# shocker-0x15/GfxExp

Hardware: AMD Instinct MI355X
Metric: Mpaths/s, ReSTIR DI (original, biased) 1920x1080 1 spp, Bistro-Exterior stand-in (higher is better)
Workload: dtype f32; 1 GPU; configs[2] (0-based index into BASELINE.json): ReSTIR DI biased, procedural street stand-in for Bistro Exterior (2547728 instanced triangles, 2745 instances, 2100 emitter instances), textured materials (albedo / smoothness / normal maps with bump mapping, float emittance maps on the signs), 32 candidates, temporal + 2x5 spatial reuse, radius 20, visibility reuse; width=1920, height=1080, spp=1, parallelism=single GPU, light_inst_distribution=cached (static scene): built once, the per-frame call returns early

## Files before the change

### gfxexp_amd/csrc/capi.cpp

```cpp
#include <cstdlib>
#include <cstring>
#include <memory>
#include "internal.h"
#include "denoise/denoise.h"
#include "denoise/taa.h"
#include "bc/bc_textures.h"

using namespace gfx;

struct gfx_ctx { Context c; };
struct gfx_denoiser { Denoiser d; };
struct gfx_taa { TemporalAA t; };

static thread_local std::string g_createError;

namespace {
struct DeviceGuard {
    int prev = -1; bool switched = false;
    explicit DeviceGuard(int device) {
        GFX_HIP(hipGetDevice(&prev));
        if (prev != device) { GFX_HIP(hipSetDevice(device)); switched = true; }
    }
    ~DeviceGuard() { if (switched) (void)hipSetDevice(prev); }
};
int env_int(const char* name, int fallback, int lo, int hi) {
    const char* e = getenv(name);
    if (!e || !*e) return fallback;
    const int v = atoi(e);
    return (v < lo || v > hi) ? fallback : v;
}
}
#define GFX_TRY(ctx) if (!(ctx)) return 1; try { DeviceGuard deviceGuard__((ctx)->c.device);
#define GFX_CATCH(ctx) \
    return 0; } \
    catch (const std::exception& e) { (ctx)->c.lastError = e.what(); return 1; } \
    catch (...) { (ctx)->c.lastError = "unknown error"; return 1; }

extern "C" {

const char* gfx_version(void) { return "gfxexp_amd 0.1 gfx950"; }

int gfx_ctx_create(int device, gfx_ctx** out) {
    *out = nullptr;
    try {
        int count = 0;
        GFX_HIP(hipGetDeviceCount(&count));
        if (device < 0 || device >= count) throw HipError("gfx_ctx_create: no such HIP device");
        GFX_HIP(hipSetDevice(device));
        std::unique_ptr<gfx_ctx> ctx(new gfx_ctx());
        ctx->c.device = device;
        hipDeviceProp_t prop;
        GFX_HIP(hipGetDeviceProperties(&prop, device));
        ctx->c.numCUs = prop.multiProcessorCount;
        Tunables& t = ctx->c.tune;
        t.pixelMap = env_int("GFX_PIXEL_MAP", t.pixelMap, 0, 2);
        t.superShiftX = env_int("GFX_SUPER_X", t.superShiftX, 0, 6);
        t.superShiftY = env_int("GFX_SUPER_Y", t.superShiftY, 0, 6);
        t.traceBlocksPerCU = env_int("GFX_TRACE_BLOCKS_PER_CU", t.traceBlocksPerCU, 1, 8);
        t.traceRefill = env_int("GFX_TRACE_REFILL", t.traceRefill, 1, 64);
        t.traceBatch = env_int("GFX_TRACE_BATCH", t.traceBatch, 1, 65536);
        t.temporalHints = env_int("GFX_TEMPORAL_HINTS", t.temporalHints, 0, 1);
        t.ptOverlap = env_int("GFX_PT_OVERLAP", t.ptOverlap, 0, 1);
        t.ptRegen = env_int("GFX_PT_REGEN", t.ptRegen, 0, 8);
        t.ptRegenMin = env_int("GFX_PT_REGEN_MIN", t.ptRegenMin, 1, 64);
        t.candidateSplit = env_int("GFX_CANDIDATE_SPLIT", t.candidateSplit, 0, 4);
        t.fusePasses = env_int("GFX_FUSE_PASSES", t.fusePasses, 0, 2);
        t.blockOrder = env_int("GFX_BLOCK_ORDER", t.blockOrder, 0, 1);
        t.nrcStagedInfer = env_int("GFX_NRC_STAGED_INFER", t.nrcStagedInfer, 0, 3);
        if (t.candidateSplit == 3) t.candidateSplit = 2;
        ctx->c.dTraceCounters.reserve(64);
        GFX_HIP(hipMemset(ctx->c.dTraceCounters.p, 0, 64));
        *out = ctx.release();
        return 0;
    }
    catch (const std::exception& e) { g_createError = e.what(); return 1; }
}

void gfx_ctx_destroy(gfx_ctx* ctx) {
    if (!ctx) return;
    (void)hipDeviceSynchronize();
    bc_textures_drop(ctx->c);
    delete ctx;
}

const char* gfx_last_error(gfx_ctx* ctx) { return ctx ? ctx->c.lastError.c_str() : g_createError.c_str(); }

int gfx_material_set(gfx_ctx* ctx, uint32_t matSlot, const gfx_material* mat) {
    GFX_TRY(ctx)
    if (!mat) throw HipError("gfx_material_set: null material");
    if (matSlot >= (1u << 24)) throw HipError("gfx_material_set: material slot out of range");
    if (ctx->c.materials.size() <= matSlot) {
        gfx_material zero; std::memset(&zero, 0, sizeof(zero));
        ctx->c.materials.resize(matSlot + 1, zero);
    }
    ctx->c.materials[matSlot] = *mat;
    ctx->c.sceneDirty = true;
    GFX_CATCH(ctx)
}

int gfx_texture_set(gfx_ctx* ctx, uint32_t texSlot, uint32_t width, uint32_t height, uint32_t format, const void* texels) {
    GFX_TRY(ctx)
    if (texSlot == 0 || texSlot > (1u << 20)) throw HipError("gfx_texture_set: texture slots are 1-based");
    if (width == 0 || height == 0 || width > 16384 || height > 16384) throw HipError("gfx_texture_set: bad size");
    size_t bpp = 0;
    switch (format) {
    case GFX_TEX_RGBA8_SRGB: case GFX_TEX_RGBA8_UNORM: bpp = 4; break;
    case GFX_TEX_R8_UNORM: bpp = 1; break;
    case GFX_TEX_RG8_UNORM: bpp = 2; break;
    case GFX_TEX_RGBA32F: bpp = 16; break;
    default: throw HipError("gfx_texture_set: unknown format");
    }
    if (!texels) throw HipError("gfx_texture_set: null texels");
    if (ctx->c.textures.size() <= texSlot) ctx->c.textures.resize(texSlot + 1);
    HostTexture& t = ctx->c.textures[texSlot];
    t.width = width; t.height = height; t.format = format;
    t.texels.assign(static_cast<const uint8_t*>(texels), static_cast<const uint8_t*>(texels) + bpp * width * height);
    bc_texture_forget(ctx->c, texSlot);
    ctx->c.sceneDirty = true;
    GFX_CATCH(ctx)
}

static size_t texel_bytes(uint32_t format) {
    return format == GFX_TEX_RGBA32F ? 16 : (format == GFX_TEX_RG8_UNORM ? 2 : (format == GFX_TEX_R8_UNORM ? 1 : 4));
}

int gfx_texture_set_bc(gfx_ctx* ctx, uint32_t texSlot, uint32_t width, uint32_t height, uint32_t bcFormat, const void* blocks, uint32_t format) {
    GFX_TRY(ctx)
    if (texSlot == 0 || texSlot > (1u << 20)) throw HipError("gfx_texture_set_bc: texture slots are 1-based");
    if (width == 0 || height == 0 || width > 16384 || height > 16384) throw HipError("gfx_texture_set_bc: bad size");
    const uint32_t blockBytes = bc_block_bytes(bcFormat);
    if (blockBytes == 0) throw HipError("gfx_texture_set_bc: unknown block-compressed format");
    if (format == GFX_TEX_RGBA32F) throw HipError("gfx_texture_set_bc: blocks expand into an 8-bit format, not GFX_TEX_RGBA32F");
    if (format != GFX_TEX_RGBA8_SRGB && format != GFX_TEX_RGBA8_UNORM && format != GFX_TEX_R8_UNORM && format != GFX_TEX_RG8_UNORM)
        throw HipError("gfx_texture_set_bc: unknown format");
    if (!blocks) throw HipError("gfx_texture_set_bc: null blocks");
    bc_texture_store(ctx->c, texSlot, bcFormat, blocks, static_cast<size_t>((width + 3) / 4) * ((height + 3) / 4) * blockBytes);
    if (ctx->c.textures.size() <= texSlot) ctx->c.textures.resize(texSlot + 1);
    HostTexture& t = ctx->c.textures[texSlot];
    t.width = width; t.height = height; t.format = format;
    std::vector<uint8_t>().swap(t.texels);
    ctx->c.sceneDirty = true;
    GFX_CATCH(ctx)
}

int gfx_texture_read(gfx_ctx* ctx, void* stream, uint32_t texSlot, void* hostOut, size_t bytes) {
    GFX_TRY(ctx)
    Context& c = ctx->c;
    if (texSlot == 0 || texSlot >= c.textures.size() || c.textures[texSlot].width == 0) throw HipError("gfx_texture_read: texture slot was never set");
    const HostTexture& t = c.textures[texSlot];
    if (!hostOut || bytes != texel_bytes(t.format) * t.width * t.height) throw HipError("gfx_texture_read: the buffer must hold the slot's texels exactly");
    hipStream_t s = static_cast<hipStream_t>(stream);
    scene_upload(c, s);
    DevTexture d;
    GFX_HIP(hipMemcpyAsync(&d, c.dTextures.as<DevTexture>() + texSlot, sizeof(d), hipMemcpyDeviceToHost, s));
    GFX_HIP(hipStreamSynchronize(s));
    if (d.width != t.width || d.height != t.height || d.format != t.format) throw HipError("gfx_texture_read: the device descriptor does not match the slot");
    GFX_HIP(hipMemcpyAsync(hostOut, c.dTexelPool.as<uint32_t>() + d.offset, bytes, hipMemcpyDeviceToHost, s));
    GFX_HIP(hipStreamSynchronize(s));
    GFX_CATCH(ctx)
}

int gfx_texture_sample(gfx_ctx* ctx, void* stream, uint32_t texSlot, const void* dUv, uint32_t n, void* dOut, int gather) {
    GFX_TRY(ctx)
    texture_sample(ctx->c, static_cast<hipStream_t>(stream), texSlot, dUv, n, dOut, gather);
    GFX_CATCH(ctx)
}

int gfx_geom_create(gfx_ctx* ctx, const void* vertices, uint32_t vertexStride, uint32_t numVertices,
                    const uint32_t* triangles, uint32_t numTriangles, uint32_t matSlot, uint32_t* geomInstSlot) {
    GFX_TRY(ctx)
    if (vertexStride < sizeof(gfx_vertex)) throw HipError("gfx_geom_create: vertexStride smaller than gfx_vertex");
    HostGeom g;
    g.vertices.resize(numVertices);
    for (uint32_t i = 0; i < numVertices; ++i) {
        gfx_vertex v;
        std::memcpy(&v, static_cast<const uint8_t*>(vertices) + static_cast<size_t>(vertexStride) * i, sizeof(v));
        DevVertex& d = g.vertices[i];
        d.px = v.position[0]; d.py = v.position[1]; d.pz = v.position[2];
        d.nx = v.normal[0]; d.ny = v.normal[1]; d.nz = v.normal[2];
        d.tx = v.texCoord0Dir[0]; d.ty = v.texCoord0Dir[1]; d.tz = v.texCoord0Dir[2];
        d.u = v.texCoord[0]; d.v = v.texCoord[1]; d.pad = 0;
    }
    g.triangles.assign(triangles, triangles + 3ull * numTriangles);
    for (uint32_t idx : g.triangles) if (idx >= numVertices) throw HipError("gfx_geom_create: triangle index out of range");
    g.materialSlot = matSlot;
    *geomInstSlot = static_cast<uint32_t>(ctx->c.geoms.size());
    ctx->c.geoms.push_back(std::move(g));
    ctx->c.sceneDirty = true;
    GFX_CATCH(ctx)
}

int gfx_group_create(gfx_ctx* ctx, const uint32_t* geomInstSlots, uint32_t n, uint32_t* group) {
    GFX_TRY(ctx)
    for (uint32_t i = 0; i < n; ++i) if (geomInstSlots[i] >= ctx->c.geoms.size()) throw HipError("gfx_group_create: unknown geomInstSlot");
    *group = static_cast<uint32_t>(ctx->c.groups.size());
    ctx->c.groups.emplace_back(geomInstSlots, geomInstSlots + n);
    ctx->c.sceneDirty = true;
    GFX_CATCH(ctx)
}

int gfx_instance_create(gfx_ctx* ctx, uint32_t group, const float xfm[12], uint32_t* instSlot) {
    GFX_TRY(ctx)
    if (group >= ctx->c.groups.size()) throw HipError("gfx_instance_create: unknown group");
    HostInstance inst;
    inst.group = group;
    std::memcpy(inst.transform, xfm, sizeof(float) * 12);
    std::memcpy(inst.prevTransform, xfm, sizeof(float) * 12);
    *instSlot = static_cast<uint32_t>(ctx->c.insts.size());
    ctx->c.insts.push_back(inst);
    ctx->c.sceneDirty = true;
    GFX_CATCH(ctx)
}

static void instance_update(gfx_ctx* ctx, uint32_t instSlot, const float xfm[12], const float* normalMatrix) {
    if (instSlot >= ctx->c.insts.size()) throw HipError("gfx_instance_set_transform: unknown instSlot");
    HostInstance& inst = ctx->c.insts[instSlot];
    std::memcpy(inst.prevTransform, inst.transform, sizeof(float) * 12);
    std::memcpy(inst.transform, xfm, sizeof(float) * 12);
    instance_cur_to_prev(inst.prevTransform, inst.transform, inst.curToPrev);
    inst.animated = true;
    inst.hasNormalMatrix = normalMatrix != nullptr;
    if (normalMatrix) std::memcpy(inst.normalMatrix, normalMatrix, sizeof(float) * 9);
    if (inst.dynamic && !ctx->c.sceneDirty) {
        ctx->c.transformsDirty = true;
        ctx->c.movedInsts.push_back(instSlot);
    }
    else {
        inst.dynamic = true;
        ctx->c.sceneDirty = true;
    }
}

int gfx_instance_set_dynamic(gfx_ctx* ctx, uint32_t instSlot, int dynamic) {
    GFX_TRY(ctx)
    if (instSlot >= ctx->c.insts.size()) throw HipError("gfx_instance_set_dynamic: unknown instSlot");
    if (ctx->c.insts[instSlot].dynamic != (dynamic != 0)) {
        ctx->c.insts[instSlot].dynamic = dynamic != 0;
        ctx->c.sceneDirty = true;
    }
    GFX_CATCH(ctx)
}

int gfx_instance_set_transform(gfx_ctx* ctx, uint32_t instSlot, const float xfm[12]) {
    GFX_TRY(ctx)
    instance_update(ctx, instSlot, xfm, nullptr);
    GFX_CATCH(ctx)
}

int gfx_instance_set_transform_and_normal_matrix(gfx_ctx* ctx, uint32_t instSlot, const float xfm[12], const float normalMatrix[9]) {
    GFX_TRY(ctx)
    instance_update(ctx, instSlot, xfm, normalMatrix);
    GFX_CATCH(ctx)
}

int gfx_accel_build(gfx_ctx* ctx, void* stream, uint64_t* handle) {
    GFX_TRY(ctx)
    Accel* a = nullptr;
    if (*handle != 0 && *handle <= ctx->c.accels.size() && ctx->c.accels[*handle - 1]) a = ctx->c.accels[*handle - 1];
    else { a = new Accel(); ctx->c.accels.push_back(a); *handle = ctx->c.accels.size(); }
    if (!lbvh_update_dynamic(ctx->c, static_cast<hipStream_t>(stream), *a)) lbvh_build(ctx->c, static_cast<hipStream_t>(stream), *a);
    GFX_CATCH(ctx)
}

static Accel* find_accel(gfx_ctx* ctx, uint64_t handle) {
    if (handle == 0 || handle > ctx->c.accels.size() || !ctx->c.accels[handle - 1]) throw HipError("invalid accel handle");
    return ctx->c.accels[handle - 1];
}

int gfx_accel_stats(gfx_ctx* ctx, uint64_t handle, uint32_t stats[4]) {
    GFX_TRY(ctx)
    const Accel* a = find_accel(ctx, handle);
    stats[0] = a->numInputTris; stats[1] = a->numNodes; stats[2] = a->numTris; stats[3] = a->maxDepth;
    GFX_CATCH(ctx)
}

int gfx_accel_tri_ids(gfx_ctx* ctx, uint64_t handle, const void** dTriIds, uint32_t* count) {
    GFX_TRY(ctx)
    const Accel* a = find_accel(ctx, handle);
    *dTriIds = a->triIds.p; *count = a->numTris;
    GFX_CATCH(ctx)
}

int gfx_accel_set_max_leaf(gfx_ctx* ctx, uint32_t maxLeafTris) {
    GFX_TRY(ctx)
    ctx->c.maxLeafTris = maxLeafTris < 1 ? 1 : (maxLeafTris > 4 ? 4 : maxLeafTris);
    GFX_CATCH(ctx)
}

int gfx_lights_build_static(gfx_ctx* ctx, void* stream) {
    GFX_TRY(ctx)
    lights_build_static(ctx->c, static_cast<hipStream_t>(stream));
    GFX_CATCH(ctx)
}

int gfx_lights_build_instances(gfx_ctx* ctx, void* stream, uint32_t bufferIndex) {
    GFX_TRY(ctx)
    lights_build_instances(ctx->c, static_cast<hipStream_t>(stream), bufferIndex);
    GFX_CATCH(ctx)
}

int gfx_lights_read(gfx_ctx* ctx, uint32_t level, uint32_t index, float* weights, float* cdf,
                    uint32_t capacity, uint32_t* n, float* integral) {
    GFX_TRY(ctx)
    Context& c = ctx->c;
    GFX_HIP(hipDeviceSynchronize());
    uint32_t off = 0xFFFFFFFFu, count = 0;
    float integ = 0.0f;
    if (level == 0) {
        off = c.lightInstDistOffset; count = static_cast<uint32_t>(c.insts.size());
        GFX_HIP(hipMemcpy(&integ, c.dLightInstIntegral.p, sizeof(float), hipMemcpyDeviceToHost));
    }
    else if (level == 1) {
        if (index >= c.hInsts.size()) throw HipError("gfx_lights_read: bad instance index");
        DevInstance d;
        GFX_HIP(hipMemcpy(&d, c.dInsts.as<DevInstance>() + index, sizeof(d), hipMemcpyDeviceToHost));
        off = d.distOffset; count = off == 0xFFFFFFFFu ? 0 : d.numGeomInsts; integ = d.distIntegral;
    }
    else {
        if (index >= c.hGeomInsts.size()) throw HipError("gfx_lights_read: bad geomInst index");
        DevGeomInst d;
        GFX_HIP(hipMemcpy(&d, c.dGeomInsts.as<DevGeomInst>() + index, sizeof(d), hipMemcpyDeviceToHost));
        off = d.distOffset; count = off == 0xFFFFFFFFu ? 0 : d.distCount; integ = d.distIntegral;
    }
    *n = count; *integral = integ;
    const uint32_t m = count < capacity ? count : capacity;
    if (m && weights) GFX_HIP(hipMemcpy(weights, c.dLightW.as<float>() + off, sizeof(float) * m, hipMemcpyDeviceToHost));
    if (m && cdf) GFX_HIP(hipMemcpy(cdf, c.dLightCDF.as<float>() + off, sizeof(float) * m, hipMemcpyDeviceToHost));
    GFX_CATCH(ctx)
}

int gfx_lights_table_info(gfx_ctx* ctx, uint32_t info[8]) {
    GFX_TRY(ctx)
    Context& c = ctx->c;
    GFX_HIP(hipDeviceSynchronize());
    uint32_t header[4] = { 0, 0, 0, 0 };
    if (c.dSpanHeader.p) GFX_HIP(hipMemcpy(header, c.dSpanHeader.p, sizeof(header), hipMemcpyDeviceToHost));
    info[0] = header[0]; info[1] = header[1]; info[2] = c.numEmitterRecs; info[3] = c.spanGuideCells;
    info[4] = c.numLightMatrices; info[5] = 0; info[6] = 0; info[7] = 0;
    if (header[0] && c.spanGuideCells && c.dSpanGuide.p) {
        std::vector<SpanGuide> guide(c.spanGuideCells);
        GFX_HIP(hipMemcpy(guide.data(), c.dSpanGuide.p, sizeof(SpanGuide) * guide.size(), hipMemcpyDeviceToHost));
        for (const SpanGuide& g : guide) if (g.a & kGuideInterior) ++info[5];
    }
    GFX_CATCH(ctx)
}

int gfx_trace(gfx_ctx* ctx, void* stream, uint64_t accel, int mode, const void* dRayOrgTmin, const void* dRayDirTmax,
              uint32_t numRays, void* dOut, void* dCounters) {
    return gfx_trace_counted(ctx, stream, accel, mode, dRayOrgTmin, dRayDirTmax, numRays, dOut, dCounters, nullptr);
}

int gfx_trace_counted(gfx_ctx* ctx, void* stream, uint64_t accel, int mode, const void* dRayOrgTmin, const void* dRayDirTmax,
                      uint32_t numRays, void* dOut, void* dCounters, void* dPerRayItems) {
    GFX_TRY(ctx)
    if (dPerRayItems && !dCounters) throw HipError("gfx_trace_counted: per-ray item counts need the counter buffer (the counting kernel)");
    const Accel* a = find_accel(ctx, accel);
    TraceLaunch t;
    t.accel = a->dev();
    t.rayOrgTmin = static_cast<const float4*>(dRayOrgTmin);
    t.rayDirTmax = static_cast<const float4*>(dRayDirTmax);
    t.numRays = numRays; t.numRaysPtr = nullptr; t.out = dOut; t.mode = mode;
    t.perRayItems = static_cast<uint32_t*>(dPerRayItems);
    const bool savedEnabled = ctx->c.countersEnabled;
    DevBuf saved = ctx->c.dTraceCounters;
    if (dCounters) { ctx->c.countersEnabled = true; ctx->c.dTraceCounters.p = dCounters; ctx->c.countersSplit = false; }
    try { trace_launch(ctx->c, static_cast<hipStream_t>(stream), t); }
    catch (...) { ctx->c.dTraceCounters = saved; ctx->c.countersEnabled = savedEnabled; ctx->c.countersSplit = true; throw; }
    ctx->c.dTraceCounters = saved; ctx->c.countersEnabled = savedEnabled; ctx->c.countersSplit = true;
    GFX_CATCH(ctx)
}

int gfx_restir_copy_to_linear(gfx_ctx* ctx, void* stream, void* dLinearColor, void* dLinearAlbedo, void* dLinearNormal, void* dLinearMotionVector) {
    GFX_TRY(ctx)
    restir_copy_to_linear(ctx->c, static_cast<hipStream_t>(stream), dLinearColor, dLinearAlbedo, dLinearNormal, dLinearMotionVector);
    GFX_CATCH(ctx)
}
int gfx_visualize(gfx_ctx* ctx, void* stream, const void* dLinearBuffer, int bufferTypeToDisplay, float motionVectorOffset, float motionVectorScale,
                  uint32_t width, uint32_t height, void* dOutputFloat4) {
    GFX_TRY(ctx)
    restir_visualize(ctx->c, static_cast<hipStream_t>(stream), dLinearBuffer, bufferTypeToDisplay, motionVectorOffset, motionVectorScale, width, height, dOutputFloat4);
    GFX_CATCH(ctx)
}

int gfx_restir_copy_depth_to_linear(gfx_ctx* ctx, void* stream, void* dLinearDepth) {
    GFX_TRY(ctx)
    restir_copy_depth_to_linear(ctx->c, static_cast<hipStream_t>(stream), dLinearDepth);
    GFX_CATCH(ctx)
}

int gfx_restir_copy_emissive_to_linear(gfx_ctx* ctx, void* stream, void* dLinearEmissive) {
    GFX_TRY(ctx)
    restir_copy_emissive_to_linear(ctx->c, static_cast<hipStream_t>(stream), dLinearEmissive);
    GFX_CATCH(ctx)
}

int gfx_denoiser_default_settings(gfx_denoiser_settings* out) {
    if (!out) return 1;
    denoiser_default_settings(out);
    return 0;
}
int gfx_denoiser_create(gfx_ctx* ctx, uint32_t width, uint32_t height, const gfx_denoiser_settings* settings, gfx_denoiser** out) {
    GFX_TRY(ctx)
    if (!out) throw HipError("gfx_denoiser_create: null output handle");
    *out = nullptr;
    gfx_denoiser_settings st;
    if (settings) st = *settings;
    else denoiser_default_settings(&st);
    std::unique_ptr<gfx_denoiser> d(new gfx_denoiser());
    d->d.device = ctx->c.device;
    try { denoiser_init(d->d, width, height, st); }
    catch (...) { denoiser_release(d->d); throw; }
    *out = d.release();
    GFX_CATCH(ctx)
}
int gfx_denoiser_destroy(gfx_denoiser* den) {
    if (!den) return 1;
    int prev = -1;
    const bool switched = hipGetDevice(&prev) == hipSuccess && prev != den->d.device && hipSetDevice(den->d.device) == hipSuccess;
    (void)hipDeviceSynchronize();
    denoiser_release(den->d);
    if (switched) (void)hipSetDevice(prev);
    delete den;
    return 0;
}
int gfx_denoise(gfx_ctx* ctx, void* stream, gfx_denoiser* den, const gfx_denoiser_inputs* in, int isFirstFrame, void* dDenoisedFloat4) {
    GFX_TRY(ctx)
    if (!den || !in) throw HipError("gfx_denoise: null denoiser or inputs");
    if (!in->beauty || !in->albedo || !in->normal || !in->flow || !dDenoisedFloat4)
        throw HipError("gfx_denoise: beauty, albedo, normal, flow and the output are required");
    if (in->width != den->d.width || in->height != den->d.height)
        throw HipError("gfx_denoise: input size differs from gfx_denoiser_create's");
    if (den->d.device != ctx->c.device) throw HipError("gfx_denoise: the denoiser belongs to another device");
    denoise(den->d, static_cast<hipStream_t>(stream), *in, isFirstFrame != 0, dDenoisedFloat4);
    GFX_CATCH(ctx)
}
int gfx_denoiser_history(gfx_denoiser* den, gfx_denoiser_history_buffers* out) {
    if (!den || !out) return 1;
    const uint32_t k = den->d.cur;
    out->lighting = den->d.lighting[k].p;
    out->moments = den->d.moments[k].p;
    out->length = den->d.length[k].p;
    out->guide = den->d.guide[k].p;
    return 0;
}

int gfx_restir_copy_taa_flow_to_linear(gfx_ctx* ctx, void* stream, void* dLinearFlow) {
    GFX_TRY(ctx)
    restir_copy_taa_flow_to_linear(ctx->c, static_cast<hipStream_t>(stream), dLinearFlow);
    GFX_CATCH(ctx)
}

int gfx_taa_create(gfx_ctx* ctx, uint32_t width, uint32_t height, uint32_t historyLength, gfx_taa** out) {
    GFX_TRY(ctx)
    if (!out) throw HipError("gfx_taa_create: null output handle");
    *out = nullptr;
    std::unique_ptr<gfx_taa> t(new gfx_taa());
    t->t.device = ctx->c.device;
    try { taa_init(t->t, width, height, historyLength); }
    catch (...) { taa_release(t->t); throw; }
    *out = t.release();
    GFX_CATCH(ctx)
}
int gfx_taa_destroy(gfx_taa* taa) {
    if (!taa) return 1;
    int prev = -1;
    const bool switched = hipGetDevice(&prev) == hipSuccess && prev != taa->t.device && hipSetDevice(taa->t.device) == hipSuccess;
    (void)hipDeviceSynchronize();
    taa_release(taa->t);
    if (switched) (void)hipSetDevice(prev);
    delete taa;
    return 0;
}
int gfx_taa_set_history_length(gfx_taa* taa, uint32_t historyLength) {
    if (!taa || historyLength < 1 || historyLength > kTaaMaxHistoryLength) return 1;
    taa->t.historyLength = historyLength;
    return 0;
}
int gfx_taa_apply(gfx_ctx* ctx, void* stream, gfx_taa* taa, const gfx_taa_inputs* in, int isFirstFrame, void* dOutFloat4) {
    GFX_TRY(ctx)
    if (!taa || !in) throw HipError("gfx_taa_apply: null TAA object or inputs");
    if (!in->color || !in->flow || !dOutFloat4) throw HipError("gfx_taa_apply: color, flow and the output are required");
    if (in->width != taa->t.width || in->height != taa->t.height) throw HipError("gfx_taa_apply: input size differs from gfx_taa_create's");
    if (dOutFloat4 == in->color) throw HipError("gfx_taa_apply: the output must not be the color input (the pass reads neighbours)");
    if (dOutFloat4 == taa->t.history[0].p || dOutFloat4 == taa->t.history[1].p)
        throw HipError("gfx_taa_apply: the output must not be the object's own history");
    if (taa->t.device != ctx->c.device) throw HipError("gfx_taa_apply: the TAA object belongs to another device");
    taa_apply(taa->t, static_cast<hipStream_t>(stream), in->color, in->flow, isFirstFrame != 0, dOutFloat4);
    GFX_CATCH(ctx)
}
int gfx_taa_history(gfx_taa* taa, const void** dHistory) {
    if (!taa || !dHistory) return 1;
    *dHistory = taa->t.history[taa->t.cur].p;
    return 0;
}

int gfx_restir_set_params(gfx_ctx* ctx, void* , const gfx_restir_static_params* s, const gfx_restir_frame_params* f,
                          uint32_t currentReservoirIndex, uint32_t spatialNeighborBaseIndex) {
    GFX_TRY(ctx)
    if (s) ctx->c.restir.s = *s;
    if (f) ctx->c.restir.f = *f;
    ctx->c.restir.currentReservoirIndex = currentReservoirIndex & 1u;
    ctx->c.restir.spatialNeighborBaseIndex = spatialNeighborBaseIndex & 1023u;
    ctx->c.restir.valid = true;
    GFX_CATCH(ctx)
}

int gfx_restir_launch(gfx_ctx* ctx, void* stream, int pass, uint32_t width, uint32_t height) {
    GFX_TRY(ctx)
    restir_launch(ctx->c, static_cast<hipStream_t>(stream), pass, width, height, 0, height);
    GFX_CATCH(ctx)
}

int gfx_restir_launch_rows_gap(gfx_ctx* ctx, void* stream, int pass, uint32_t width, uint32_t height, uint32_t rowBegin, uint32_t rowEnd,
                               uint32_t gapBegin, uint32_t gapEnd) {
    GFX_TRY(ctx)
    if (rowBegin == 0 && rowEnd == 0) rowEnd = height;
    restir_launch(ctx->c, static_cast<hipStream_t>(stream), pass, width, height, rowBegin, rowEnd, gapBegin, gapEnd);
    GFX_CATCH(ctx)
}

int gfx_restir_launch_rows(gfx_ctx* ctx, void* stream, int pass, uint32_t width, uint32_t height, uint32_t rowBegin, uint32_t rowEnd) {
    GFX_TRY(ctx)
    if (rowBegin == 0 && rowEnd == 0) rowEnd = height;
    restir_launch(ctx->c, static_cast<hipStream_t>(stream), pass, width, height, rowBegin, rowEnd);
    GFX_CATCH(ctx)
}

int gfx_regir_set_params(gfx_ctx* ctx, const gfx_regir_params* p) {
    GFX_TRY(ctx)
    if (!p) throw HipError("gfx_regir_set_params: null parameters");
    if (!p->gridDimension[0] || !p->gridDimension[1] || !p->gridDimension[2]) throw HipError("gfx_regir_set_params: empty grid");
    ctx->c.regir = *p;
    ctx->c.regirValid = true;
    GFX_CATCH(ctx)
}

int gfx_nrc_set_render_params(gfx_ctx* ctx, const gfx_nrc_params* p) {
    GFX_TRY(ctx)
    if (!p) throw HipError("gfx_nrc_set_render_params: null parameters");
    ctx->c.nrcRender = *p;
    ctx->c.nrcRenderValid = true;
    GFX_CATCH(ctx)
}

int gfx_pt_launch(gfx_ctx* ctx, void* stream, int pass, uint32_t width, uint32_t height, uint32_t maxPathLength,
                  uint32_t rowBegin, uint32_t rowEnd) {
    GFX_TRY(ctx)
    if (rowEnd == 0 && rowBegin == 0) rowEnd = height;
    pathtrace_launch(ctx->c, static_cast<hipStream_t>(stream), pass, width, height, maxPathLength, rowBegin, rowEnd);
    GFX_CATCH(ctx)
}

static NrcNet* nrc_of(gfx_ctx* ctx, uint64_t handle) {
    if (handle == 0 || handle > ctx->c.nrcNets.size() || !ctx->c.nrcNets[handle - 1]) throw HipError("gfx_nrc: invalid network handle");
    return ctx->c.nrcNets[handle - 1];
}
int gfx_nrc_create(gfx_ctx* ctx, int positionEncoding, uint32_t numHiddenLayers, float learningRate, uint64_t* outHandle) {
    GFX_TRY(ctx)
    ctx->c.nrcNets.push_back(nrc_create(ctx->c, positionEncoding, numHiddenLayers, learningRate));
    *outHandle = ctx->c.nrcNets.size();
    GFX_CATCH(ctx)
}
int gfx_nrc_destroy(gfx_ctx* ctx, uint64_t handle) {
    GFX_TRY(ctx)
    NrcNet* net = nrc_of(ctx, handle);
    GFX_HIP(hipDeviceSynchronize());
    nrc_destroy(net);
    ctx->c.nrcNets[handle - 1] = nullptr;
    GFX_CATCH(ctx)
}
int gfx_nrc_infer(gfx_ctx* ctx, void* stream, uint64_t handle, const void* dInputData, uint32_t numData, void* dPredictionData) {
    GFX_TRY(ctx)
    nrc_infer(ctx->c, static_cast<hipStream_t>(stream), nrc_of(ctx, handle), static_cast<const float*>(dInputData), numData, static_cast<float*>(dPredictionData));
    GFX_CATCH(ctx)
}
int gfx_nrc_infer_indirect(gfx_ctx* ctx, void* stream, uint64_t handle, const void* dInputData, const void* dNumData, uint32_t maxNumData, void* dPredictionData) {
    GFX_TRY(ctx)
    if (!dNumData) throw HipError("gfx_nrc_infer_indirect: null batch-size pointer");
    nrc_infer(ctx->c, static_cast<hipStream_t>(stream), nrc_of(ctx, handle), static_cast<const float*>(dInputData), maxNumData, static_cast<float*>(dPredictionData),
              static_cast<const uint32_t*>(dNumData));
    GFX_CATCH(ctx)
}
int gfx_nrc_query_count_ptr(gfx_ctx* ctx, void** dNumData) {
    GFX_TRY(ctx)
    if (!ctx->c.nrcQueryCount.p) { ctx->c.nrcQueryCount.reserve(256); GFX_HIP(hipMemset(ctx->c.nrcQueryCount.p, 0, 256)); }
    *dNumData = ctx->c.nrcQueryCount.p;
    GFX_CATCH(ctx)
}
int gfx_nrc_train(gfx_ctx* ctx, void* stream, uint64_t handle, const void* dInputData, const void* dTargetData, uint32_t numData, float* lossOnCPU) {
    GFX_TRY(ctx)
    nrc_train(ctx->c, static_cast<hipStream_t>(stream), nrc_of(ctx, handle), static_cast<const float*>(dInputData), static_cast<const float*>(dTargetData), numData, lossOnCPU);
    GFX_CATCH(ctx)
}
int gfx_nrc_num_params(gfx_ctx* ctx, uint64_t handle, uint32_t* outCount) {
    GFX_TRY(ctx)
    *outCount = nrc_num_params(nrc_of(ctx, handle));
    GFX_CATCH(ctx)
}
int gfx_nrc_set_params(gfx_ctx* ctx, uint64_t handle, const float* hostParams, uint32_t count) {
    GFX_TRY(ctx)
    nrc_set_params(ctx->c, nullptr, nrc_of(ctx, handle), hostParams, count);
    GFX_CATCH(ctx)
}
int gfx_nrc_get_params(gfx_ctx* ctx, uint64_t handle, int which, float* hostOut, uint32_t count) {
    GFX_TRY(ctx)
    nrc_get_params(nrc_of(ctx, handle), which, hostOut, count);
    GFX_CATCH(ctx)
}

int gfx_nrc_inference_image(gfx_ctx* ctx, uint64_t handle, int which, void** dPtr, uint64_t* bytes) {
    GFX_TRY(ctx)
    if (!dPtr || !bytes) throw HipError("gfx_nrc_inference_image: null output");
    nrc_inference_image(ctx->c, nrc_of(ctx, handle), which, dPtr, bytes);
    GFX_CATCH(ctx)
}

int gfx_nrc_inference_image_async(gfx_ctx* ctx, void* stream, uint64_t handle, int which, void** dPtr, uint64_t* bytes) {
    GFX_TRY(ctx)
    if (!dPtr || !bytes) throw HipError("gfx_nrc_inference_image_async: null output");
    nrc_inference_image(ctx->c, nrc_of(ctx, handle), which, dPtr, bytes, static_cast<hipStream_t>(stream), true);
    GFX_CATCH(ctx)
}

int gfx_nrc_params_checksum(gfx_ctx* ctx, void* stream, uint64_t handle, void* dOutU32) {
    GFX_TRY(ctx)
    if (!dOutU32) throw HipError("gfx_nrc_params_checksum: null output");
    nrc_params_checksum(ctx->c, static_cast<hipStream_t>(stream), nrc_of(ctx, handle), static_cast<uint32_t*>(dOutU32));
    GFX_CATCH(ctx)
}

int gfx_read_device(gfx_ctx* ctx, const void* dSrc, void* hostDst, size_t bytes) {
    GFX_TRY(ctx)
    GFX_HIP(hipDeviceSynchronize());
    GFX_HIP(hipMemcpy(hostDst, dSrc, bytes, hipMemcpyDeviceToHost));
    GFX_CATCH(ctx)
}

int gfx_timing_enable(gfx_ctx* ctx, int enable) {
    GFX_TRY(ctx)
    ctx->c.timingEnabled = enable != 0;
    GFX_CATCH(ctx)
}

int gfx_timing_collect(gfx_ctx* ctx, char names[][48], float* totalMs, uint32_t* calls, uint32_t capacity, uint32_t* n) {
    GFX_TRY(ctx)
    Context& c = ctx->c;
    for (auto& e : c.pendingEvents) {
        GFX_HIP(hipEventSynchronize(e.second.second));
        float ms = 0;
        GFX_HIP(hipEventElapsedTime(&ms, e.second.first, e.second.second));
        KernelTiming& t = c.timings[e.first];
        t.ms += ms; ++t.calls;
        (void)hipEventDestroy(e.second.first); (void)hipEventDestroy(e.second.second);
    }
    c.pendingEvents.clear();
    uint32_t i = 0;
    for (const auto& kv : c.timings) {
        if (i < capacity) {
            std::memset(names[i], 0, 48);
            std::strncpy(names[i], kv.first.c_str(), 47);
            totalMs[i] = static_cast<float>(kv.second.ms); calls[i] = kv.second.calls;
        }
        ++i;
    }
    *n = i;
    c.timings.clear();
    GFX_CATCH(ctx)
}

int gfx_tunable_set(gfx_ctx* ctx, const char* name, int value) {
    GFX_TRY(ctx)
    if (!name) throw HipError("gfx_tunable_set: null name");
    Tunables& t = ctx->c.tune;
    const std::string n(name);
    auto in = [&](int lo, int hi) { if (value < lo || value > hi) throw HipError("gfx_tunable_set: value out of range for " + n); return value; };
    if (n == "pixel_map") t.pixelMap = in(0, 2);
    else if (n == "super_x") t.superShiftX = in(0, 6);
    else if (n == "super_y") t.superShiftY = in(0, 6);
    else if (n == "trace_blocks_per_cu") t.traceBlocksPerCU = in(1, 8);
    else if (n == "trace_refill") t.traceRefill = in(1, 64);
    else if (n == "temporal_hints") t.temporalHints = in(0, 1);
    else if (n == "trace_batch") t.traceBatch = in(1, 65536);
    else if (n == "pt_overlap") t.ptOverlap = in(0, 1);
    else if (n == "pt_regen") t.ptRegen = in(0, 8);
    else if (n == "pt_diag") t.ptDiag = in(0, 1);
    else if (n == "pt_regen_min") t.ptRegenMin = in(1, 64);
    else if (n == "fuse_passes") t.fusePasses = in(0, 2);
    else if (n == "block_order") t.blockOrder = in(0, 1);
    else if (n == "nrc_staged_infer") t.nrcStagedInfer = in(0, 3);
    else if (n == "candidate_split") { if (value == 3) throw HipError("gfx_tunable_set: candidate_split is 0 (automatic), 1, 2 or 4"); t.candidateSplit = in(0, 4); }
    else throw HipError("gfx_tunable_set: unknown tunable " + n);
    GFX_CATCH(ctx)
}

int gfx_stream_copy(gfx_ctx* ctx, void* dDst, const void* dSrc, size_t bytes, void* stream) {
    GFX_TRY(ctx)
    stream_copy(ctx->c, static_cast<hipStream_t>(stream), dDst, dSrc, bytes);
    GFX_CATCH(ctx)
}

int gfx_bc_expand(gfx_ctx* ctx, void* stream, uint32_t bcFormat, const void* dBlocks, uint32_t width, uint32_t height, uint32_t format, void* dTexels) {
    GFX_TRY(ctx)
    if (!dBlocks || !dTexels) throw HipError("gfx_bc_expand: null pointer");
    bc_expand_launch(static_cast<hipStream_t>(stream), bcFormat, dBlocks, width, height, format, dTexels);
    GFX_CATCH(ctx)
}

int gfx_counters_enable(gfx_ctx* ctx, int enable) {
    GFX_TRY(ctx)
    ctx->c.countersEnabled = enable != 0;
    GFX_CATCH(ctx)
}

int gfx_trace_diag_read(gfx_ctx* ctx, uint64_t diag[8], int reset) {
    GFX_TRY(ctx)
    GFX_HIP(hipDeviceSynchronize());
    for (int i = 0; i < 8; ++i) diag[i] = 0;
    if (ctx->c.dTraceDiag.p) {
        GFX_HIP(hipMemcpy(diag, ctx->c.dTraceDiag.p, 64, hipMemcpyDeviceToHost));
        if (reset) GFX_HIP(hipMemset(ctx->c.dTraceDiag.p, 0, 64));
    }
    GFX_CATCH(ctx)
}

int gfx_pt_diag_read(gfx_ctx* ctx, uint64_t diag[8], int reset) {
    GFX_TRY(ctx)
    GFX_HIP(hipDeviceSynchronize());
    for (int i = 0; i < 8; ++i) diag[i] = 0;
    if (ctx->c.ptDiag.p) {
        GFX_HIP(hipMemcpy(diag, ctx->c.ptDiag.p, 64, hipMemcpyDeviceToHost));
        if (reset) GFX_HIP(hipMemset(ctx->c.ptDiag.p, 0, 64));
    }
    GFX_CATCH(ctx)
}

int gfx_counters_read(gfx_ctx* ctx, uint64_t counters[8], int reset) {
    GFX_TRY(ctx)
    GFX_HIP(hipDeviceSynchronize());
    GFX_HIP(hipMemcpy(counters, ctx->c.dTraceCounters.p, 64, hipMemcpyDeviceToHost));
    if (reset) GFX_HIP(hipMemset(ctx->c.dTraceCounters.p, 0, 64));
    GFX_CATCH(ctx)
}

}
```

### gfxexp_amd/csrc/device_types.h

```cpp
#pragma once
#include <stdint.h>
#include "../../include/gfxexp.h"
#include "emitter_spans.h"

namespace gfx {

struct DevVertex {
    float px, py, pz, nx;
    float ny, nz, tx, ty;
    float tz, u, v, pad;
};
static_assert(sizeof(DevVertex) == 48, "DevVertex must be 48 bytes");

struct DevGeomInst {
    uint32_t vertexOffset;
    uint32_t triangleOffset;
    uint32_t numVertices;
    uint32_t numTriangles;
    uint32_t materialSlot;
    uint32_t distOffset;
    uint32_t distCount;
    float distIntegral;
};
static_assert(sizeof(DevGeomInst) == 32, "DevGeomInst must be 32 bytes");

struct DevInstance {
    float transform[12];
    float curToPrevTransform[12];
    float normalMatrix[12];
    uint32_t distOffset;
    uint32_t numGeomInsts;
    float distIntegral;
    uint32_t slotsOffset;
    float uniformScale;
    uint32_t pad[3];
};
static_assert(sizeof(DevInstance) == 176, "DevInstance must be 176 bytes");

struct LightGeomRef {
    uint32_t recBase;
    uint32_t distOffset;
    uint32_t distCount;
    float distIntegral;
};
static_assert(sizeof(LightGeomRef) == 16, "LightGeomRef must be 16 bytes");

struct EmitterRec {
    float pA[3], pB[3], pC[3];
    float nA[3];
    float emittance[3];
    uint32_t flags;
};
static_assert(sizeof(EmitterRec) == 64, "EmitterRec must be 64 bytes");
constexpr uint32_t kEmitterSmooth = 0x80000000u, kEmitterTexMask = 0x00007FFFu, kEmitterMatrixShift = 15u, kEmitterMatrixMask = 0xFFFFu;
struct EmitterRecExtra {
    float nB[3], nC[3];
    float twoOverLenNg;
    float primProb;
};
static_assert(sizeof(EmitterRecExtra) == 32, "EmitterRecExtra must be 32 bytes");

struct DevFlatGeom {
    uint32_t instSlot;
    uint32_t geomInstSlot;
    uint32_t triBegin;
    uint32_t numTriangles;
};

struct SubsetGeom {
    uint32_t instSlot;
    uint32_t geomInstSlot;
    uint32_t localBegin;
    uint32_t globalBegin;
};

struct DevTexture {
    uint32_t offset;
    uint32_t width, height;
    uint32_t format;
};
static_assert(sizeof(DevTexture) == 16, "DevTexture must be 16 bytes");

struct EmitterTexRef {
    float uvA[2], uvB[2], uvC[2];
    uint32_t texelOffset;
    uint32_t dims;
};
static_assert(sizeof(EmitterTexRef) == 32, "EmitterTexRef must be 32 bytes");

struct DevScene {
    const gfx_material* materials;
    const DevGeomInst* geomInsts;
    const DevInstance* insts;
    const DevVertex* vertices;
    const uint32_t* triangles;
    const uint32_t* geomInstSlotPool;
    const float* lightWeights;
    const float* lightProbs;
    const float* lightCDF;
    const LightGeomRef* lightGeomRefs;
    const EmitterRec* emitterRecs;
    const EmitterRecExtra* emitterRecExtras;
    const float* lightNormalMatrices;
    uint32_t numLightMatrices;
    const float* lightInstIntegral;
    const uint16_t* lightInstGuide;
    uint32_t lightInstGuideCells;
    uint32_t lightInstDistOffset;
    uint32_t numInsts;
    const EmitterSpan* spans;
    const SpanGuide* spanGuide;
    const uint32_t* spanHeader;
    uint32_t numSpans;
    uint32_t spanGuideCells;
    const DevTexture* textures;
    const uint32_t* texelPool;
    const float* srgbLut;
    const EmitterTexRef* emitterTexRefs;
};

struct Bvh8Node { uint32_t w[16]; };
struct Bvh8Link { uint32_t childBase, triBase, valid, pad; };
static_assert(sizeof(Bvh8Link) == 16, "Bvh8Link must be 16 bytes");
static_assert(sizeof(Bvh8Node) == 64, "Bvh8Node must be 64 bytes");

struct Bvh8Tri {
    float ax, ay, az, eABx;
    float eABy, eABz, eCAx, eCAy;
    float eCAz, nx, ny, nz;
    uint32_t instSlot, geomInstSlot, primIndex;
    uint32_t flatIndex;
};
static_assert(sizeof(Bvh8Tri) == 64, "Bvh8Tri must be 64 bytes");

struct BuildTri {
    float ax, ay, az, bx;
    float by, bz, cx, cy;
    float cz; uint32_t instSlot, geomInstSlot, primIndex;
};
static_assert(sizeof(BuildTri) == 48, "BuildTri must be 48 bytes");

struct DevAccel {
    const Bvh8Node* nodes;
    const Bvh8Link* links;
    const Bvh8Tri* tris;
    uint32_t numNodes;
    uint32_t numTris;
    uint32_t triItemOffset;
};

}
```

### gfxexp_amd/csrc/gm_math.hip.h

```cpp
#pragma once
#include <hip/hip_runtime.h>
#include <stdint.h>

namespace gfx {

#define GFX_DEV __device__ __forceinline__

#ifdef GFX_LANE_PROFILE
static __device__ unsigned long long g_laneProfile[64];
#define GFX_PROF(k) do { const unsigned long long m__ = __ballot(1); if ((threadIdx.x & 63) == __builtin_ctzll(m__)) { \
    atomicAdd(&g_laneProfile[2 * (k)], static_cast<unsigned long long>(__popcll(m__))); atomicAdd(&g_laneProfile[2 * (k) + 1], 1ull); } } while (0)
#define GFX_CYC_BEGIN unsigned long long cyc__[8] = { 0, 0, 0, 0, 0, 0, 0, 0 }; unsigned long long cycT__ = __builtin_amdgcn_s_memtime(); int cycK__ = 7;
#define GFX_CYC(k) do { const unsigned long long t__ = __builtin_amdgcn_s_memtime(); cyc__[cycK__] += t__ - cycT__; cycT__ = t__; cycK__ = (k); } while (0)
#define GFX_CYC_END do { GFX_CYC(7); if ((threadIdx.x & 63) == 0) for (int k__ = 0; k__ < 8; ++k__) atomicAdd(&g_laneProfile[32 + k__], cyc__[k__]); } while (0)
#else
#define GFX_PROF(k) do { } while (0)
#define GFX_CYC_BEGIN
#define GFX_CYC(k) do { } while (0)
#define GFX_CYC_END do { } while (0)
#endif

constexpr float kPi = 3.14159265358979323846f;
constexpr float kTwoPi = 2 * 3.14159265358979323846f;
constexpr float kHalfPi = 1.5707963705062866f;
constexpr float kQuarterPi = 0.7853981852531433f;

GFX_DEV uint32_t f2bits(float f) { return __float_as_uint(f); }
GFX_DEV float bits2f(uint32_t u) { return __uint_as_float(u); }
GFX_DEV float fmin2(float a, float b) { return a < b ? a : b; }
GFX_DEV float fmax2(float a, float b) { return a > b ? a : b; }
GFX_DEV float sq(float x) { return x * x; }
GFX_DEV float pow5(float x) { const float x2 = x * x; return x * (x2 * x2); }
GFX_DEV float mixf(float v0, float v1, float t) { return (1 - t) * v0 + t * v1; }
GFX_DEV bool is_finite(float x) { return (f2bits(x) & 0x7F800000u) != 0x7F800000u; }

GFX_DEV uint32_t f2u_sat(float x) {
    if (!(x > 0.0f)) return 0u;
    if (x >= 4294967296.0f) return 0xFFFFFFFFu;
    return static_cast<uint32_t>(x);
}
GFX_DEV int32_t f2i_sat(float x) {
    if (!(x == x)) return 0;
    if (x >= 2147483648.0f) return 2147483647;
    if (x <= -2147483648.0f) return -2147483647 - 1;
    return static_cast<int32_t>(x);
}

GFX_DEV void gm_sincos(float x, float& s, float& c) {
    const float q = rintf(x * 0.6366197466850281f);
    float r = fmaf(q, -1.5703125f, x);
    r = fmaf(q, -0.0004837512969970703f, r);
    r = fmaf(q, -7.549790126404332e-08f, r);
    const int32_t n = f2i_sat(q);
    const float r2 = r * r;
    float ps = fmaf(-1.9515295891e-4f, r2, 8.3321608736e-3f);
    ps = fmaf(ps, r2, -1.6666654611e-1f);
    const float sr = fmaf(ps * r2, r, r);
    float pc = fmaf(2.443315711809948e-5f, r2, -1.388731625493765e-3f);
    pc = fmaf(pc, r2, 4.166664568298827e-2f);
    const float cr = fmaf(pc * r2, r2, fmaf(-0.5f, r2, 1.0f));
    const float ss = (n & 1) ? cr : sr;
    const float cc = (n & 1) ? sr : cr;
    s = (n & 2) ? -ss : ss;
    c = ((n + 1) & 2) ? -cc : cc;
}
GFX_DEV float gm_sin(float x) { float s, c; gm_sincos(x, s, c); return s; }
GFX_DEV float gm_cos(float x) { float s, c; gm_sincos(x, s, c); return c; }
GFX_DEV float gm_tan(float x) { float s, c; gm_sincos(x, s, c); return s / c; }

GFX_DEV float gm_exp(float x) {
    const float n = floorf(x * 1.44269504088896341f + 0.5f);
    float r = fmaf(n, -0.693359375f, x);
    r = fmaf(n, 2.12194440e-4f, r);
    float p = fmaf(1.9875691500e-4f, r, 1.3981999507e-3f);
    p = fmaf(p, r, 8.3334519073e-3f);
    p = fmaf(p, r, 4.1665795894e-2f);
    p = fmaf(p, r, 1.6666665459e-1f);
    p = fmaf(p, r, 5.0000001201e-1f);
    const float y = fmaf(p, r * r, r) + 1.0f;
    return y * bits2f(static_cast<uint32_t>(static_cast<int32_t>(n) + 127) << 23);
}

GFX_DEV float gm_asin_core(float x) {
    const float z = x * x;
    float p = fmaf(4.2163199048e-2f, z, 2.4181311049e-2f);
    p = fmaf(p, z, 4.5470025998e-2f);
    p = fmaf(p, z, 7.4953002686e-2f);
    p = fmaf(p, z, 1.6666752422e-1f);
    return fmaf(p * z, x, x);
}
GFX_DEV float gm_acos(float x) {
    if (x > 0.5f) return 2.0f * gm_asin_core(sqrtf(0.5f * (1.0f - x)));
    if (x < -0.5f) return kPi - 2.0f * gm_asin_core(sqrtf(0.5f * (1.0f + x)));
    return kHalfPi - gm_asin_core(x);
}
GFX_DEV float gm_atan_nonneg(float t) {
    float y0 = 0.0f;
    if (t > 2.414213562373095f) { y0 = kHalfPi; t = -1.0f / t; }
    else if (t > 0.4142135623730950f) { y0 = kQuarterPi; t = (t - 1.0f) / (t + 1.0f); }
    const float z = t * t;
    float p = fmaf(8.05374449538e-2f, z, -1.38776856032e-1f);
    p = fmaf(p, z, 1.99777106478e-1f);
    p = fmaf(p, z, -3.33329491539e-1f);
    return y0 + fmaf(p * z, t, t);
}
GFX_DEV float gm_atan(float t) { return t < 0.0f ? -gm_atan_nonneg(-t) : gm_atan_nonneg(t); }
GFX_DEV float gm_atan2(float y, float x) {
    if (x == 0.0f && y == 0.0f) return 0.0f;
    const float ax = fabsf(x), ay = fabsf(y);
    float a = (ax == 0.0f) ? kHalfPi : gm_atan_nonneg(ay / ax);
    if (x < 0.0f) a = kPi - a;
    return y < 0.0f ? -a : a;
}

struct f3 {
    float x, y, z;
    GFX_DEV f3() {}
    GFX_DEV explicit f3(float v) : x(v), y(v), z(v) {}
    GFX_DEV f3(float a, float b, float c) : x(a), y(b), z(c) {}
};
GFX_DEV f3 operator+(f3 a, f3 b) { return f3(a.x + b.x, a.y + b.y, a.z + b.z); }
GFX_DEV f3 operator-(f3 a, f3 b) { return f3(a.x - b.x, a.y - b.y, a.z - b.z); }
GFX_DEV f3 operator-(f3 a) { return f3(-a.x, -a.y, -a.z); }
GFX_DEV f3 operator*(f3 a, float s) { return f3(a.x * s, a.y * s, a.z * s); }
GFX_DEV f3 operator*(float s, f3 a) { return f3(a.x * s, a.y * s, a.z * s); }
GFX_DEV f3 operator*(f3 a, f3 b) { return f3(a.x * b.x, a.y * b.y, a.z * b.z); }
GFX_DEV f3 operator/(f3 a, float s) { const float r = 1 / s; return f3(a.x * r, a.y * r, a.z * r); }
GFX_DEV float dot(f3 a, f3 b) { return a.x * b.x + a.y * b.y + a.z * b.z; }
GFX_DEV f3 cross(f3 a, f3 b) { return f3(a.y * b.z - a.z * b.y, a.z * b.x - a.x * b.z, a.x * b.y - a.y * b.x); }
GFX_DEV float len2(f3 a) { return a.x * a.x + a.y * a.y + a.z * a.z; }
GFX_DEV float len(f3 a) { return sqrtf(len2(a)); }
GFX_DEV f3 unit(f3 a) { return a / len(a); }
GFX_DEV bool all_finite(f3 a) { return is_finite(a.x) && is_finite(a.y) && is_finite(a.z); }
GFX_DEV f3 mix3(f3 v0, f3 v1, float t) { return (1 - t) * v0 + t * v1; }
GFX_DEV f3 min3(f3 a, f3 b) { return f3(fmin2(a.x, b.x), fmin2(a.y, b.y), fmin2(a.z, b.z)); }
GFX_DEV f3 max3(f3 a, f3 b) { return f3(fmax2(a.x, b.x), fmax2(a.y, b.y), fmax2(a.z, b.z)); }
GFX_DEV float luminance_srgb(f3 c) { return 0.2126729f * c.x + 0.7151522f * c.y + 0.0721750f * c.z; }

struct m33 { f3 r0, r1, r2; };
GFX_DEV f3 mul(const m33& m, f3 v) { return f3(dot(m.r0, v), dot(m.r1, v), dot(m.r2, v)); }
GFX_DEV m33 inverse(const m33& m) {
    const float a = m.r0.x, b = m.r0.y, c = m.r0.z, d = m.r1.x, e = m.r1.y, f = m.r1.z, g = m.r2.x, h = m.r2.y, i = m.r2.z;
    const float det = a * e * i + b * f * g + c * d * h - c * e * g - b * d * i - a * f * h;
    const float r = 1 / det;
    m33 o;
    o.r0 = f3((e * i - f * h), -(b * i - c * h), (b * f - c * e)) * r;
    o.r1 = f3(-(d * i - f * g), (a * i - c * g), -(a * f - c * d)) * r;
    o.r2 = f3((d * h - e * g), -(a * h - b * g), (a * e - b * d)) * r;
    return o;
}
struct m34 { float m[12]; };
GFX_DEV f3 xfm_point(const m34& a, f3 p) {
    return f3(a.m[0] * p.x + a.m[1] * p.y + a.m[2] * p.z + a.m[3] * 1.0f,
              a.m[4] * p.x + a.m[5] * p.y + a.m[6] * p.z + a.m[7] * 1.0f,
              a.m[8] * p.x + a.m[9] * p.y + a.m[10] * p.z + a.m[11] * 1.0f);
}
GFX_DEV f3 xfm_vector(const m34& a, f3 v) {
    return f3(a.m[0] * v.x + a.m[1] * v.y + a.m[2] * v.z + a.m[3] * 0.0f,
              a.m[4] * v.x + a.m[5] * v.y + a.m[6] * v.z + a.m[7] * 0.0f,
              a.m[8] * v.x + a.m[9] * v.y + a.m[10] * v.z + a.m[11] * 0.0f);
}

}
```

### gfxexp_amd/csrc/internal.h

```cpp
#pragma once
#include <hip/hip_runtime.h>
#include <stdint.h>
#include <map>
#include <stdexcept>
#include <string>
#include <vector>
#include "device_types.h"

namespace gfx {

struct HipError : std::runtime_error { using std::runtime_error::runtime_error; };
#define GFX_HIP(call) do { hipError_t e__ = (call); if (e__ != hipSuccess) \
    throw ::gfx::HipError(std::string(#call) + ": " + hipGetErrorString(e__)); } while (0)

struct DevBuf {
    void* p = nullptr;
    size_t bytes = 0;
    void reserve(size_t n) {
        if (n <= bytes) return;
        if (p) GFX_HIP(hipFree(p));
        p = nullptr; bytes = 0;
        GFX_HIP(hipMalloc(&p, n));
        bytes = n;
    }
    void release() { if (p) (void)hipFree(p); p = nullptr; bytes = 0; }
    template <typename T> T* as() const { return static_cast<T*>(p); }
};

struct HostTexture {
    uint32_t width = 0, height = 0, format = 0;
    std::vector<uint8_t> texels;
};
struct HostGeom {
    std::vector<DevVertex> vertices;
    std::vector<uint32_t> triangles;
    uint32_t materialSlot = 0;
};
struct HostInstance {
    uint32_t group = 0;
    float transform[12];
    float prevTransform[12];
    bool animated = false, hasNormalMatrix = false;
    bool dynamic = false;
    float curToPrev[12];
    float normalMatrix[9];
};
void instance_cur_to_prev(const float prev[12], const float cur[12], float out[12]);

struct Accel {
    DevBuf nodes, links, triIds;
    uint32_t triItemOffset = 0;
    uint32_t numNodes = 0, numTris = 0, numInputTris = 0, maxDepth = 0;
    bool split = false;
    DevBuf rootBoxes;
    uint32_t numStaticTris = 0, staticNodeEnd = 0, staticDepth = 0;
    Bvh8Tri* trisPtr() const { return reinterpret_cast<Bvh8Tri*>(nodes.as<Bvh8Node>() + triItemOffset); }
    DevAccel dev() const {
        DevAccel a; a.nodes = nodes.as<Bvh8Node>(); a.links = links.as<Bvh8Link>(); a.tris = trisPtr(); a.numNodes = numNodes; a.numTris = numTris;
        a.triItemOffset = triItemOffset;
        return a;
    }
};

struct KernelTiming { double ms = 0; uint32_t calls = 0; };

struct RestirParams {
    gfx_restir_static_params s;
    gfx_restir_frame_params f;
    uint32_t currentReservoirIndex = 0;
    uint32_t spatialNeighborBaseIndex = 0;
    bool valid = false;
};

struct NrcNet;

struct Tunables {
    int pixelMap = 2;
    int superShiftX = 2, superShiftY = 2;
    int traceBlocksPerCU = 4;
    int traceRefill = 8;
    int traceBatch = 64;
    int temporalHints = 1;
    int candidateSplit = 0;
    int blockOrder = 1;
    int fusePasses = 0;
    int nrcStagedInfer = 0;
    int ptDiag = 0;
    int ptRegen = 0;
    int ptRegenMin = 16;
    int ptOverlap = 1;
};

struct Context {
    int device = 0;
    int numCUs = 0;
    Tunables tune;
    uint32_t nrcInferPipedLds = 0;
    bool nrcInferStagedConfigured = false;
    size_t nrcTrainLdsConfigured = 0;
    std::string lastError;
    std::vector<gfx_material> materials;
    std::vector<HostTexture> textures;
    std::vector<HostGeom> geoms;
    std::vector<std::vector<uint32_t>> groups;
    std::vector<HostInstance> insts;
    bool sceneDirty = true;
    DevBuf dMaterials, dGeomInsts, dInsts, dVertices, dTriangles, dSlotPool, dFlatGeoms, dLightW, dLightP, dLightCDF, dLightRefs, dEmitterRecs, dEmitterRecExtras, dLightNormalMatrices, dInstMatrixIndex, dTextures, dTexelPool, dSrgbLut, dEmitterTexRefs;
    bool anyEmittanceTexture = false;
    std::vector<LightGeomRef> hLightRefs;
    uint32_t numEmitterRecs = 0;
    std::vector<DevGeomInst> hGeomInsts;
    std::vector<DevInstance> hInsts;
    std::vector<DevFlatGeom> hFlatGeoms;
    uint32_t totalTriangles = 0;
    std::vector<SubsetGeom> hSubset[2];
    DevBuf dSubset[2];
    uint32_t subsetTris[2] = { 0, 0 };
    bool transformsDirty = false;
    std::vector<uint32_t> movedInsts;
    bool emitterRecsDirty = false;
    bool instDistValid = false;
    uint32_t lightPoolSize = 0;
    uint32_t lightInstDistOffset = 0;
    DevBuf dLightInstIntegral;
    DevBuf dLightInstGuide;
    uint32_t lightInstGuideCells = 0;
    bool lightsStaticBuilt = false;
    DevBuf dSpans, dSpanGuide, dSpanHeader, dSpanInstBegin;
    uint32_t spanGuideCells = 0;
    struct TicketState { bool zeroed = false; uint32_t next = 0; void* buffer = nullptr; hipStream_t stream = nullptr; hipEvent_t lastLaunch = nullptr; } ticketState[3];
    uint32_t numLightMatrices = 0;
    struct PinnedStage { void* p = nullptr; size_t bytes = 0; hipEvent_t done = nullptr; } lightStage[2];
    uint32_t lightStageNext = 0;
    DevScene devScene() const;
    std::vector<Accel*> accels;
    uint32_t maxLeafTris = 4;
    DevBuf rayOrg, rayDir, rayOut, rayHits, spill, pixelRaySlot, shadeScratch, spatialScratch, smallCounters;
    DevBuf gbRayOrg, gbRayDir, gbRayHits, gbSpill, gbCounters;
    DevBuf auxSpill, auxCounters;
    struct BlockOrder { DevBuf cost, order; uint64_t key = 0; uint32_t blocks = 0; bool valid = false; hipEvent_t counted = nullptr, ordered = nullptr; } blockOrders[5];
    hipStream_t auxStream = nullptr;
    hipEvent_t auxFork = nullptr, auxJoin = nullptr;
    DevBuf ptPending, ptExtOrg, ptExtDir, ptExtOwner, ptState;
    DevBuf rearchSlots;
    DevBuf nrcState, neeTrainIdx;
    DevBuf nrcQueryCount;
    DevBuf bTris, bBoxes, bKeys, bKeysAlt, bVals, bValsAlt, bSortTemp, bNodesLR, bParents, bFlags, bNodeBoxes, bRanges, bQueueA, bQueueB, bCounters, bCosts, bDec, bFlatIdx;
    RestirParams restir;
    gfx_regir_params regir;
    std::vector<NrcNet*> nrcNets;
    gfx_nrc_params nrcRender;
    bool nrcRenderValid = false;
    bool regirValid = false;
    bool timingEnabled = false;
    std::map<std::string, KernelTiming> timings;
    std::vector<std::pair<std::string, std::pair<hipEvent_t, hipEvent_t>>> pendingEvents;
    bool countersEnabled = false;
    DevBuf dTraceCounters;
    bool countersSplit = true;
    DevBuf dTraceDiag;
    DevBuf ptDiag;
    ~Context();
};

struct ScopedKernelTimer {
    Context& ctx; hipStream_t stream; const char* name; hipEvent_t a = nullptr, b = nullptr;
    ScopedKernelTimer(Context& c, hipStream_t s, const char* n) : ctx(c), stream(s), name(n) {
        if (!ctx.timingEnabled) return;
        GFX_HIP(hipEventCreate(&a)); GFX_HIP(hipEventCreate(&b));
        GFX_HIP(hipEventRecord(a, stream));
    }
    ~ScopedKernelTimer() {
        if (!a) return;
        (void)hipEventRecord(b, stream);
        ctx.pendingEvents.push_back({ name, { a, b } });
    }
};

void scene_upload(Context& ctx, hipStream_t stream);
void transforms_upload(Context& ctx, hipStream_t stream);
void lbvh_build(Context& ctx, hipStream_t stream, Accel& out);
bool lbvh_update_dynamic(Context& ctx, hipStream_t stream, Accel& out);
constexpr size_t kSmallCountersBytes = 1024 + 2 * 4096;
constexpr size_t kSmallCountersTicketOffset = 1024;
struct TraceLaunch {
    DevAccel accel;
    const float4* rayOrgTmin; const float4* rayDirTmax;
    uint32_t numRays; const uint32_t* numRaysPtr;
    void* out;
    int mode;
    DevBuf* spill = nullptr;
    DevBuf* counters = nullptr;
    uint32_t* perRayItems = nullptr;
    uint32_t* zeroWords[2] = { nullptr, nullptr };
    bool hintFromOut = false;
};
void trace_launch(Context& ctx, hipStream_t stream, const TraceLaunch& t);
void block_order_begin(Context& ctx, hipStream_t stream, int which, uint32_t blocks, uint64_t key, uint32_t minBlocks, const uint32_t*& order, uint32_t*& cost);
void block_order_end(Context& ctx, hipStream_t stream, int which, uint32_t blocks, uint32_t* cost);
void stream_copy(Context& ctx, hipStream_t stream, void* dDst, const void* dSrc, size_t bytes);
void texture_sample(Context& ctx, hipStream_t stream, uint32_t texSlot, const void* dUv, uint32_t n, void* dOut, int gather);
void light_matrices_upload(Context& ctx, hipStream_t stream);
void lights_build_static(Context& ctx, hipStream_t stream);
void lights_build_instances(Context& ctx, hipStream_t stream, uint32_t bufferIndex);
void restir_launch(Context& ctx, hipStream_t stream, int pass, uint32_t width, uint32_t height, uint32_t rowBegin, uint32_t rowEnd, uint32_t gapBegin = 0, uint32_t gapEnd = 0);
void restir_copy_to_linear(Context& ctx, hipStream_t stream, void* color, void* albedo, void* normal, void* motion);
void restir_visualize(Context& ctx, hipStream_t stream, const void* linearBuffer, int bufferType, float mvOffset, float mvScale, uint32_t width, uint32_t height, void* out);
struct NrcNet;
NrcNet* nrc_create(Context& ctx, int posEnc, uint32_t numHiddenLayers, float learningRate);
void nrc_destroy(NrcNet* net);
uint32_t nrc_num_params(const NrcNet* net);
void nrc_set_params(Context& ctx, hipStream_t stream, NrcNet* net, const float* hostParams, uint32_t count);
void nrc_get_params(NrcNet* net, int which, float* hostOut, uint32_t count);
void nrc_inference_image(Context& ctx, NrcNet* net, int which, void** dPtr, uint64_t* bytes, hipStream_t stream = nullptr, bool onStream = false);
void nrc_params_checksum(Context& ctx, hipStream_t stream, NrcNet* net, uint32_t* dOut);
void nrc_infer(Context& ctx, hipStream_t stream, NrcNet* net, const float* dInputs, uint32_t numData, float* dPredictions, const uint32_t* dNumData = nullptr);
void nrc_train(Context& ctx, hipStream_t stream, NrcNet* net, const float* dInputs, const float* dTargets, uint32_t numData, float* lossOnCPU);
void pathtrace_launch(Context& ctx, hipStream_t stream, int pass, uint32_t width, uint32_t height,
                      uint32_t maxPathLength, uint32_t rowBegin, uint32_t rowEnd);

}
```

### gfxexp_amd/csrc/lights.hip

```cpp
#include <cstdlib>
#include "internal.h"
#include "shading.hip.h"

namespace gfx {

__global__ void k_triangle_importance(DevScene sc, uint32_t numGeomInsts, float* __restrict__ weights) {
    const uint32_t gi = blockIdx.y;
    if (gi >= numGeomInsts) return;
    const DevGeomInst g = sc.geomInsts[gi];
    if (g.distOffset == 0xFFFFFFFFu) return;
    const gfx_material& mat = sc.materials[g.materialSlot];
    const f3 e(mat.emittance[0], mat.emittance[1], mat.emittance[2]);
    for (uint32_t t = blockIdx.x * blockDim.x + threadIdx.x; t < g.numTriangles; t += gridDim.x * blockDim.x) {
        const uint32_t* tri = sc.triangles + 3ull * (g.triangleOffset + t);
        const DevVertex v0 = load_vertex(sc.vertices + g.vertexOffset + tri[0]);
        const DevVertex v1 = load_vertex(sc.vertices + g.vertexOffset + tri[1]);
        const DevVertex v2 = load_vertex(sc.vertices + g.vertexOffset + tri[2]);
        const f3 p0(v0.px, v0.py, v0.pz), p1(v1.px, v1.py, v1.pz), p2(v2.px, v2.py, v2.pz);
        const f3 n = cross(p1 - p0, p2 - p0);
        const float area = 0.5f * len(n);
        f3 e0 = e, e1 = e, e2 = e;
        if (mat.texEmittance) {
            const float4 t0 = tex2d(sc, mat.texEmittance, v0.u, v0.v), t1 = tex2d(sc, mat.texEmittance, v1.u, v1.v), t2 = tex2d(sc, mat.texEmittance, v2.u, v2.v);
            e0 = f3(t0.x, t0.y, t0.z); e1 = f3(t1.x, t1.y, t1.z); e2 = f3(t2.x, t2.y, t2.z);
        }
        f3 est = f3(0.0f) + e0;
        est = est + e1;
        est = est + e2;
        est = est / 3.0f;
        weights[g.distOffset + t] = luminance_srgb(est) * area;
    }
}

__global__ void k_scan_geom_dists(DevGeomInst* __restrict__ geomInsts, uint32_t numGeomInsts,
                                  const float* __restrict__ weights, float* __restrict__ cdf, float* __restrict__ probs) {
    const uint32_t gi = blockIdx.x * blockDim.x + threadIdx.x;
    if (gi >= numGeomInsts) return;
    DevGeomInst g = geomInsts[gi];
    if (g.distOffset == 0xFFFFFFFFu) return;
    float acc = 0.0f, last = 0.0f, lastW = 0.0f;
    for (uint32_t i = 0; i < g.distCount; ++i) {
        const float w = weights[g.distOffset + i];
        cdf[g.distOffset + i] = acc;
        last = acc; lastW = w;
        acc += w;
    }
    const float integral = g.distCount ? last + lastW : 0.0f;
    geomInsts[gi].distIntegral = integral;
    for (uint32_t i = 0; i < g.distCount; ++i) probs[g.distOffset + i] = weights[g.distOffset + i] / integral;
}

__global__ void k_inst_geom_dists(DevInstance* __restrict__ insts, uint32_t numInsts,
                                  const DevGeomInst* __restrict__ geomInsts, const uint32_t* __restrict__ slotPool,
                                  float* __restrict__ weights, float* __restrict__ cdf, float* __restrict__ probs) {
    const uint32_t ii = blockIdx.x * blockDim.x + threadIdx.x;
    if (ii >= numInsts) return;
    DevInstance* inst = insts + ii;
    if (inst->distOffset == 0xFFFFFFFFu) { inst->distIntegral = 0.0f; return; }
    float acc = 0.0f, last = 0.0f, lastW = 0.0f;
    for (uint32_t i = 0; i < inst->numGeomInsts; ++i) {
        const float w = geomInsts[slotPool[inst->slotsOffset + i]].distIntegral;
        weights[inst->distOffset + i] = w;
        cdf[inst->distOffset + i] = acc;
        last = acc; lastW = w;
        acc += w;
    }
    const float integral = inst->numGeomInsts ? last + lastW : 0.0f;
    inst->distIntegral = integral;
    for (uint32_t i = 0; i < inst->numGeomInsts; ++i) probs[inst->distOffset + i] = weights[inst->distOffset + i] / integral;
}

__global__ void k_emitter_records(DevScene sc, uint32_t numInsts, LightGeomRef* __restrict__ refs, EmitterRec* __restrict__ recs,
                                  EmitterRecExtra* __restrict__ extras, const uint32_t* __restrict__ instMatrixIndex,
                                  EmitterTexRef* __restrict__ texRefs ) {
    const uint32_t ii = blockIdx.x;
    if (ii >= numInsts) return;
    const DevInstance* inst = sc.insts + ii;
    if (inst->distOffset == 0xFFFFFFFFu) return;
    const uint32_t matrixBits = (instMatrixIndex[ii] & kEmitterMatrixMask) << kEmitterMatrixShift;
    const m34 xfm = load_m34(inst->transform);
    for (uint32_t k = 0; k < inst->numGeomInsts; ++k) {
        const DevGeomInst g = sc.geomInsts[sc.geomInstSlotPool[inst->slotsOffset + k]];
        LightGeomRef* ref = refs + inst->distOffset + k;
        if (threadIdx.x == 0) ref->distIntegral = g.distIntegral;
        const uint32_t recBase = ref->recBase;
        if (recBase == 0xFFFFFFFFu) continue;
        const gfx_material& mat = sc.materials[g.materialSlot];
        for (uint32_t t = threadIdx.x; t < g.numTriangles; t += blockDim.x) {
            const uint32_t* tri = sc.triangles + 3ull * (g.triangleOffset + t);
            const DevVertex vA = load_vertex(sc.vertices + g.vertexOffset + tri[0]);
            const DevVertex vB = load_vertex(sc.vertices + g.vertexOffset + tri[1]);
            const DevVertex vC = load_vertex(sc.vertices + g.vertexOffset + tri[2]);
            const f3 pA = xfm_point(xfm, f3(vA.px, vA.py, vA.pz));
            const f3 pB = xfm_point(xfm, f3(vB.px, vB.py, vB.pz));
            const f3 pC = xfm_point(xfm, f3(vC.px, vC.py, vC.pz));
            EmitterRec r;
            r.pA[0] = pA.x; r.pA[1] = pA.y; r.pA[2] = pA.z;
            r.pB[0] = pB.x; r.pB[1] = pB.y; r.pB[2] = pB.z;
            r.pC[0] = pC.x; r.pC[1] = pC.y; r.pC[2] = pC.z;
            r.nA[0] = vA.nx; r.nA[1] = vA.ny; r.nA[2] = vA.nz;
            EmitterRecExtra x;
            x.nB[0] = vB.nx; x.nB[1] = vB.ny; x.nB[2] = vB.nz;
            x.nC[0] = vC.nx; x.nC[1] = vC.ny; x.nC[2] = vC.nz;
            const bool smooth = f2bits(vB.nx) != f2bits(vA.nx) || f2bits(vB.ny) != f2bits(vA.ny) || f2bits(vB.nz) != f2bits(vA.nz) ||
                                f2bits(vC.nx) != f2bits(vA.nx) || f2bits(vC.ny) != f2bits(vA.ny) || f2bits(vC.nz) != f2bits(vA.nz);
            const f3 e = mat.hasEmittance ? f3(1.0f) * f3(mat.emittance[0], mat.emittance[1], mat.emittance[2]) : f3(0.0f);
            r.emittance[0] = e.x; r.emittance[1] = e.y; r.emittance[2] = e.z;
            r.flags = ((texRefs && mat.hasEmittance) ? (mat.texEmittance & kEmitterTexMask) : 0u) | matrixBits | (smooth ? kEmitterSmooth : 0u);
            x.twoOverLenNg = 2.0f / len(cross(pB - pA, pC - pA));
            x.primProb = sc.lightWeights[g.distOffset + t] / g.distIntegral;
            float4* dst = reinterpret_cast<float4*>(recs + recBase + t);
            const float4* src = reinterpret_cast<const float4*>(&r);
            for (int q = 0; q < 4; ++q) dst[q] = src[q];
            float4* dstX = reinterpret_cast<float4*>(extras + recBase + t);
            const float4* srcX = reinterpret_cast<const float4*>(&x);
            dstX[0] = srcX[0]; dstX[1] = srcX[1];
            if (texRefs) {
                EmitterTexRef tr;
                tr.uvA[0] = vA.u; tr.uvA[1] = vA.v; tr.uvB[0] = vB.u; tr.uvB[1] = vB.v; tr.uvC[0] = vC.u; tr.uvC[1] = vC.v;
                const DevTexture desc = sc.textures[mat.hasEmittance ? mat.texEmittance : 0u];
                tr.texelOffset = desc.offset;
                tr.dims = desc.width ? (((desc.width - 1u) & 0x3FFFu) | (((desc.height - 1u) & 0x3FFFu) << 14) | (desc.format << 28)) : 0u;
                texRefs[recBase + t] = tr;
            }
        }
    }
}

__global__ void k_inst_importance(const DevInstance* __restrict__ insts, uint32_t numInsts, uint32_t off, float* __restrict__ weights) {
    const uint32_t ii = blockIdx.x * blockDim.x + threadIdx.x;
    if (ii >= numInsts) return;
    const DevInstance* inst = insts + ii;
    const float sx = sqrtf(inst->transform[0] * inst->transform[0] + inst->transform[4] * inst->transform[4] +
                           inst->transform[8] * inst->transform[8]);
    weights[off + ii] = sq(sx) * inst->distIntegral;
}

constexpr int kScanChunk = 4096;
__global__ __launch_bounds__(256) void k_scan_inst_dist(uint32_t numInsts, uint32_t off, const float* __restrict__ weights,
                                                        float* __restrict__ cdf, float* __restrict__ probs,
                                                        float* __restrict__ integralOut, uint32_t guideCells) {
    __shared__ float buf[kScanChunk];
    __shared__ float carry[2];
    if (blockIdx.x != 0) return;
    if (threadIdx.x == 0) { carry[0] = 0.0f; carry[1] = 0.0f; }
    float lastCdf = 0.0f;
    for (uint32_t base = 0; base < numInsts; base += kScanChunk) {
        const uint32_t m = min(static_cast<uint32_t>(kScanChunk), numInsts - base);
        for (uint32_t i = threadIdx.x; i < m; i += blockDim.x) buf[i] = weights[off + base + i];
        __syncthreads();
        if (threadIdx.x == 0) {
            float acc = carry[0];
            for (uint32_t i = 0; i < m; ++i) {
                const float w = buf[i];
                buf[i] = acc;
                lastCdf = acc; carry[1] = w;
                acc += w;
            }
            carry[0] = acc;
        }
        __syncthreads();
        for (uint32_t i = threadIdx.x; i < m; i += blockDim.x) cdf[off + base + i] = buf[i];
        __syncthreads();
    }
    if (threadIdx.x == 0) carry[0] = numInsts ? lastCdf + carry[1] : 0.0f;
    __syncthreads();
    const float integral = carry[0];
    for (uint32_t i = threadIdx.x; i < numInsts; i += blockDim.x) probs[off + i] = weights[off + i] / integral;
    if (threadIdx.x == 0) {
        integralOut[0] = integral;
        const float scale = static_cast<float>(guideCells) / integral;
        const bool usable = numInsts > 0 && numInsts <= 65536 && integral > 0.0f && integral < INFINITY && scale > 0.0f && scale < INFINITY;
        integralOut[1] = usable ? scale : 0.0f;
        reinterpret_cast<uint32_t*>(integralOut)[2] = usable ? 1u : 0u;
    }
}

__global__ __launch_bounds__(256) void k_inst_guide(uint32_t numInsts, uint32_t off, const float* __restrict__ cdfPool,
                                                    float* __restrict__ header, uint16_t* __restrict__ guide, uint32_t cells) {
    const uint32_t t = blockIdx.x * blockDim.x + threadIdx.x;
    const float* cdf = cdfPool + off;
    if (reinterpret_cast<const uint32_t*>(header)[2] == 0u) return;
    const float scale = header[1];
    if (t + 1 < numInsts && !(cdf[t] <= cdf[t + 1])) atomicAnd(reinterpret_cast<uint32_t*>(header) + 2, 0u);
    if (t == 0 && !(cdf[0] == 0.0f)) atomicAnd(reinterpret_cast<uint32_t*>(header) + 2, 0u);
    if (t >= cells) return;
    uint32_t idx = 0;
    for (uint32_t d = next_pow2(numInsts) >> 1; d >= 1; d >>= 1) {
        if (idx + d >= numInsts) continue;
        if (guide_cell(cdf[idx + d], scale, cells) <= t) idx += d;
    }
    guide[t] = static_cast<uint16_t>(idx);
}

__global__ void k_span_init(const float* __restrict__ instHeader, uint32_t* __restrict__ spanHeader) {
    const float integral = instHeader[0];
    spanHeader[0] = (integral > 0.0f && integral < INFINITY) ? 1u : 0u;
    spanHeader[1] = 0u;
}

__global__ void k_span_inst_begin(uint32_t numInsts, const float* __restrict__ cdf1, const float* __restrict__ header,
                                  uint32_t* __restrict__ instBegin) {
    const uint32_t i = blockIdx.x * blockDim.x + threadIdx.x;
    if (i > numInsts) return;
    if (i == numInsts) { instBegin[i] = kSpanBitsEnd; return; }
    SpanInstPred pred; pred.integral = header[0]; pred.i = i; pred.cdfAtI = cdf1[i];
    instBegin[i] = span_bisect(0u, kSpanBitsEnd, pred);
}

__global__ void k_span_records(DevScene sc, uint32_t numInsts, const uint32_t* __restrict__ instBegin,
                               EmitterSpan* __restrict__ spans, uint32_t* __restrict__ spanHeader) {
    const uint32_t ii = blockIdx.x;
    if (ii >= numInsts) return;
    const DevInstance* inst = sc.insts + ii;
    if (inst->distOffset == 0xFFFFFFFFu) return;
    const float* cdf1 = sc.lightCDF + sc.lightInstDistOffset;
    SpanRecordKey key;
    key.integral1 = *sc.lightInstIntegral;
    key.lo1 = cdf1[ii];
    key.hi1 = ii + 1 < numInsts ? cdf1[ii + 1] : key.integral1;
    key.integral2 = inst->distIntegral;
    key.n2 = inst->numGeomInsts;
    const float instProb = sc.lightProbs[sc.lightInstDistOffset + ii];
    const uint32_t rangeLo = instBegin[ii], rangeHi = instBegin[ii + 1];
    bool monotone = key.lo1 <= key.hi1;
    for (uint32_t k = 0; k < key.n2; ++k) {
        const LightGeomRef ref = sc.lightGeomRefs[inst->distOffset + k];
        if (ref.recBase == 0xFFFFFFFFu) continue;
        key.k = k;
        key.lo2 = sc.lightCDF[inst->distOffset + k];
        key.hi2 = k + 1 < key.n2 ? sc.lightCDF[inst->distOffset + k + 1] : key.integral2;
        key.integral3 = ref.distIntegral;
        monotone = monotone && key.lo2 <= key.hi2;
        const float geomProb = sc.lightProbs[inst->distOffset + k];
        const bool earlyOut = instProb == 0.0f || geomProb == 0.0f;
        for (uint32_t t = threadIdx.x; t < ref.distCount; t += blockDim.x) {
            key.t = t;
            key.cdf3AtT = sc.lightCDF[ref.distOffset + t];
            if (t + 1 < ref.distCount) monotone = monotone && key.cdf3AtT <= sc.lightCDF[ref.distOffset + t + 1];
            uint32_t b, e;
            span_record_interval(key, rangeLo, rangeHi, earlyOut, t + 1 == ref.distCount, b, e);
            const EmitterRecExtra* rec = sc.emitterRecExtras + ref.recBase + t;
            EmitterSpan s;
            s.begin = span_float(b);
            s.end = span_float(e);
            s.density = ((instProb * geomProb) * rec->primProb) * rec->twoOverLenNg;
            s.instSlot = ii;
            *reinterpret_cast<SpanWords*>(spans + ref.recBase + t) = __builtin_bit_cast(SpanWords, s);
        }
    }
    if (!monotone) atomicAnd(spanHeader, 0u);
}

__global__ void k_span_finish(DevScene sc, EmitterSpan* __restrict__ spans, uint32_t* __restrict__ spanHeader) {
    const uint32_t e = blockIdx.x * blockDim.x + threadIdx.x;
    if (e >= sc.numSpans) return;
    EmitterSpan s = spans[e];
    const uint32_t nextBegin = e + 1 < sc.numSpans ? span_bits(spans[e + 1].begin) : kSpanBitsEnd;
    if (span_bits(s.end) == kSpanPending) s.end = span_float(nextBegin);
    const uint32_t b = span_bits(s.begin), en = span_bits(s.end);
    bool ok = b <= en && en <= nextBegin && en <= kSpanBitsEnd;
    const InstDist dist = inst_dist_global_unguided(sc);
    auto selects = [&](uint32_t ulBits) {
        uint32_t rec, instSlot; float partial;
        return light_locate_3level(sc, dist, span_float(ulBits), rec, instSlot, partial) && rec == e;
    };
    if (b < en) {
        ok = ok && selects(b) && selects(en - 1u);
        if (b > 0u) ok = ok && !selects(b - 1u);
        if (en < kSpanBitsEnd) ok = ok && !selects(en);
    }
    else if (b < kSpanBitsEnd) ok = ok && !selects(b);
    spans[e].end = s.end;
    if (!ok) atomicAnd(spanHeader, 0u);
    else atomicAdd(spanHeader + 1, 1u);
}

__global__ void k_span_guide(const EmitterSpan* __restrict__ spans, uint32_t numSpans, SpanGuide* __restrict__ guide, uint32_t cells) {
    const uint32_t c = blockIdx.x * blockDim.x + threadIdx.x;
    if (c >= cells) return;
    guide[c] = span_guide_entry(spans, numSpans, cells, c);
}

static void span_table_build(Context& ctx, hipStream_t stream) {
    const uint32_t ni = static_cast<uint32_t>(ctx.insts.size());
    const uint32_t ne = ctx.numEmitterRecs;
    uint32_t* header = ctx.dSpanHeader.as<uint32_t>();
    GFX_HIP(hipMemsetAsync(header, 0, 16, stream));
    static int disabled = -1;
    if (disabled < 0) { const char* e = getenv("GFX_LIGHT_TABLE"); disabled = (e && e[0] == '0') ? 1 : 0; }
    if (!ni || !ne || disabled) return;
    hipLaunchKernelGGL(k_span_init, dim3(1), dim3(1), 0, stream, ctx.dLightInstIntegral.as<float>(), header);
    hipLaunchKernelGGL(k_span_inst_begin, dim3((ni + 1 + 255) / 256), dim3(256), 0, stream, ni,
                       ctx.dLightCDF.as<float>() + ctx.lightInstDistOffset, ctx.dLightInstIntegral.as<float>(), ctx.dSpanInstBegin.as<uint32_t>());
    hipLaunchKernelGGL(k_span_records, dim3(ni), dim3(64), 0, stream, ctx.devScene(), ni, ctx.dSpanInstBegin.as<uint32_t>(),
                       ctx.dSpans.as<EmitterSpan>(), header);
    hipLaunchKernelGGL(k_span_finish, dim3((ne + 255) / 256), dim3(256), 0, stream, ctx.devScene(), ctx.dSpans.as<EmitterSpan>(), header);
    hipLaunchKernelGGL(k_span_guide, dim3((ctx.spanGuideCells + 255) / 256), dim3(256), 0, stream, ctx.dSpans.as<EmitterSpan>(), ne,
                       ctx.dSpanGuide.as<SpanGuide>(), ctx.spanGuideCells);
    GFX_HIP(hipGetLastError());
}

void lights_build_static(Context& ctx, hipStream_t stream) {
    scene_upload(ctx, stream);
    const uint32_t ng = static_cast<uint32_t>(ctx.geoms.size());
    const uint32_t ni = static_cast<uint32_t>(ctx.insts.size());
    if (ng) {
        uint32_t maxTris = 1;
        for (const DevGeomInst& g : ctx.hGeomInsts) if (g.distOffset != 0xFFFFFFFFu) maxTris = std::max(maxTris, g.numTriangles);
        const dim3 grid(std::min<uint32_t>((maxTris + 255) / 256, 64), ng);
        hipLaunchKernelGGL(k_triangle_importance, grid, dim3(256), 0, stream, ctx.devScene(), ng, ctx.dLightW.as<float>());
        hipLaunchKernelGGL(k_scan_geom_dists, dim3((ng + 63) / 64), dim3(64), 0, stream,
                           ctx.dGeomInsts.as<DevGeomInst>(), ng, ctx.dLightW.as<float>(), ctx.dLightCDF.as<float>(), ctx.dLightP.as<float>());
    }
    if (ni)
        hipLaunchKernelGGL(k_inst_geom_dists, dim3((ni + 63) / 64), dim3(64), 0, stream,
                           ctx.dInsts.as<DevInstance>(), ni, ctx.dGeomInsts.as<DevGeomInst>(), ctx.dSlotPool.as<uint32_t>(),
                           ctx.dLightW.as<float>(), ctx.dLightCDF.as<float>(), ctx.dLightP.as<float>());
    if (ni)
        hipLaunchKernelGGL(k_emitter_records, dim3(ni), dim3(64), 0, stream, ctx.devScene(), ni,
                           ctx.dLightRefs.as<LightGeomRef>(), ctx.dEmitterRecs.as<EmitterRec>(), ctx.dEmitterRecExtras.as<EmitterRecExtra>(), ctx.dInstMatrixIndex.as<uint32_t>(),
                               ctx.anyEmittanceTexture ? ctx.dEmitterTexRefs.as<EmitterTexRef>() : nullptr);
    GFX_HIP(hipGetLastError());
    GFX_HIP(hipMemcpyAsync(ctx.hGeomInsts.data(), ctx.dGeomInsts.p, sizeof(DevGeomInst) * ng, hipMemcpyDeviceToHost, stream));
    GFX_HIP(hipMemcpyAsync(ctx.hInsts.data(), ctx.dInsts.p, sizeof(DevInstance) * ni, hipMemcpyDeviceToHost, stream));
    GFX_HIP(hipStreamSynchronize(stream));
    ctx.lightsStaticBuilt = true;
}

void lights_build_instances(Context& ctx, hipStream_t stream, uint32_t ) {
    if (!ctx.lightsStaticBuilt) lights_build_static(ctx, stream);
    transforms_upload(ctx, stream);
    if (ctx.emitterRecsDirty) {
        light_matrices_upload(ctx, stream);
        const uint32_t numInsts = static_cast<uint32_t>(ctx.insts.size());
        if (numInsts)
            hipLaunchKernelGGL(k_emitter_records, dim3(numInsts), dim3(64), 0, stream, ctx.devScene(), numInsts,
                               ctx.dLightRefs.as<LightGeomRef>(), ctx.dEmitterRecs.as<EmitterRec>(), ctx.dEmitterRecExtras.as<EmitterRecExtra>(), ctx.dInstMatrixIndex.as<uint32_t>(),
                               ctx.anyEmittanceTexture ? ctx.dEmitterTexRefs.as<EmitterTexRef>() : nullptr);
        GFX_HIP(hipGetLastError());
        ctx.emitterRecsDirty = false;
    }
    if (ctx.instDistValid) return;
    ctx.instDistValid = true;
    const uint32_t ni = static_cast<uint32_t>(ctx.insts.size());
    float* dIntegral = ctx.dLightInstIntegral.as<float>();
    if (ni) {
        hipLaunchKernelGGL(k_inst_importance, dim3((ni + 63) / 64), dim3(64), 0, stream,
                           ctx.dInsts.as<DevInstance>(), ni, ctx.lightInstDistOffset, ctx.dLightW.as<float>());
        hipLaunchKernelGGL(k_scan_inst_dist, dim3(1), dim3(256), 0, stream, ni, ctx.lightInstDistOffset,
                           ctx.dLightW.as<float>(), ctx.dLightCDF.as<float>(), ctx.dLightP.as<float>(), dIntegral, ctx.lightInstGuideCells);
        const uint32_t guideThreads = std::max(ni, ctx.lightInstGuideCells);
        hipLaunchKernelGGL(k_inst_guide, dim3((guideThreads + 255) / 256), dim3(256), 0, stream, ni, ctx.lightInstDistOffset,
                           ctx.dLightCDF.as<float>(), dIntegral, ctx.dLightInstGuide.as<uint16_t>(), ctx.lightInstGuideCells);
        GFX_HIP(hipGetLastError());
    }
    else GFX_HIP(hipMemsetAsync(dIntegral, 0, 4 * sizeof(float), stream));
    span_table_build(ctx, stream);
}

}
```

### gfxexp_amd/csrc/restir.hip

```cpp
#include "internal.h"
#include "shading.hip.h"
#include "pass_common.hip.h"
#include "restir_common.hip.h"
#include "coop_fetch.hip.h"
#include "trace_local.hip.h"
#include "restir_rearch.hip.h"

namespace gfx {

struct RayPair { float4 org, dir; };
GFX_DEV RayPair primary_ray(const RestirArgs& a, const PixelId& px) {
    RayPair r;
    r.org = make_float4(0.0f, 0.0f, 0.0f, 0.0f);
    r.dir = make_float4(0.0f, 0.0f, 1.0f, -1.0f);
    if (!px.valid) return r;
    const size_t p = px.p;
    const int x = px.x, y = px.y;
    const Camera cam = load_camera(a.f.camera);
    float jx = 0.5f, jy = 0.5f;
    if (a.f.enableJittering) {
        uint64_t* rngBuf = static_cast<uint64_t*>(a.s.rngBuffer);
        Pcg32 rng; rng.state = rngBuf[p];
        jx = rng.uniform();
        jy = rng.uniform();
        rngBuf[p] = rng.state;
    }
    const float fx = (x + jx) / a.s.imageSizeX;
    const float fy = (y + jy) / a.s.imageSizeY;
    const float vh = 2 * gm_tan(cam.fovY * 0.5f);
    const float vw = cam.aspect * vh;
    const f3 dir = unit(mul(cam.ori, f3(vw * (0.5f - fx), vh * (0.5f - fy), 1)));
    r.org = make_float4(cam.pos.x, cam.pos.y, cam.pos.z, 0.0f);
    r.dir = make_float4(dir.x, dir.y, dir.z, 3.402823466e+38f);
    return r;
}
__global__ __launch_bounds__(kBlock) void k_primary_rays(RestirArgs a) {
    const PixelId px = pixel_of_thread(a.px);
    const RayPair r = primary_ray(a, px);
    a.rayOrg[px.slot] = r.org;
    a.rayDir[px.slot] = r.dir;
}

GFX_DEV void calc_screen_position(const Camera& cam, f3 pw, float& sx, float& sy) {
    const m33 invOri = inverse(cam.ori);
    const f3 pv = mul(invOri, pw - cam.pos);
    const float ax = pv.x / pv.z, ay = pv.y / pv.z;
    const float h = 2 * gm_tan(cam.fovY / 2);
    const float w = cam.aspect * h;
    sx = 1 - (ax + 0.5f * w) / w;
    sy = 1 - (ay + 0.5f * h) / h;
}

GFX_DEV void gbuffer_resolve(const RestirArgs& a, const PixelId& px, const gfx_hit& h, f3 direction) {
    const size_t p = px.p;
    const int x = px.x, y = px.y;
    const uint32_t bufIdx = a.f.bufferIndex;

    f3 albedo(0.0f);
    const float qnan = bits2f(0x7FC00000u);
    f3 positionInWorld(qnan), prevPositionInWorld(qnan), shadingNormalInWorld(qnan);
    uint32_t qGeomNormal = 0, qTangent = 0, qTexCoord = 0;
    uint32_t matSlot = 0xFFFFFFFFu, instSlot = 0xFFFFFFFFu, geomInstSlot = 0xFFFFFFFFu, primIndex = 0xFFFFFFFFu;
    uint32_t qbcB = 0, qbcC = 0;

    if (h.triIndex != GFX_INVALID_SLOT) {
        const Bvh8Tri* tr = a.tris + h.triIndex;
        instSlot = tr->instSlot; geomInstSlot = tr->geomInstSlot; primIndex = tr->primIndex;
        const DevInstance* inst = a.scene.insts + instSlot;
        const DevGeomInst g = a.scene.geomInsts[geomInstSlot];
        matSlot = g.materialSlot;
        const uint32_t* tri = a.scene.triangles + 3ull * (g.triangleOffset + primIndex);
        const DevVertex vA = load_vertex(a.scene.vertices + g.vertexOffset + tri[0]);
        const DevVertex vB = load_vertex(a.scene.vertices + g.vertexOffset + tri[1]);
        const DevVertex vC = load_vertex(a.scene.vertices + g.vertexOffset + tri[2]);
        const float bcB = h.bcB, bcC = h.bcC;
        const float bcA = 1 - (bcB + bcC);
        qbcB = encode_bc(bcB);
        qbcC = encode_bc(bcC);
        const f3 pAo(vA.px, vA.py, vA.pz), pBo(vB.px, vB.py, vB.pz), pCo(vC.px, vC.py, vC.pz);
        const f3 positionInObj = bcA * pAo + bcB * pBo + bcC * pCo;
        const f3 shadingNormalInObj = bcA * f3(vA.nx, vA.ny, vA.nz) + bcB * f3(vB.nx, vB.ny, vB.nz) + bcC * f3(vC.nx, vC.ny, vC.nz);
        const f3 tc0DirInObj = bcA * f3(vA.tx, vA.ty, vA.tz) + bcB * f3(vB.tx, vB.ty, vB.tz) + bcC * f3(vC.tx, vC.ty, vC.tz);
        const float tu = bcA * vA.u + bcB * vB.u + bcC * vC.u;
        const float tv = bcA * vA.v + bcB * vB.v + bcC * vC.v;
        const f3 geomNormalInObj = cross(pBo - pAo, pCo - pAo);
        const m34 xfm = load_m34(inst->transform);
        const m33 nrm = load_m33_rows(inst->normalMatrix);
        positionInWorld = xfm_point(xfm, positionInObj);
        prevPositionInWorld = xfm_point(load_m34(inst->curToPrevTransform), positionInWorld);
        f3 geomNormalInWorld = unit(mul(nrm, geomNormalInObj));
        shadingNormalInWorld = unit(mul(nrm, shadingNormalInObj));
        f3 tc0DirInWorld = xfm_vector(xfm, tc0DirInObj);
        tc0DirInWorld = unit(tc0DirInWorld - dot(shadingNormalInWorld, tc0DirInWorld) * shadingNormalInWorld);
        if (!all_finite(shadingNormalInWorld)) {
            geomNormalInWorld = f3(0, 0, 1);
            shadingNormalInWorld = f3(0, 0, 1);
            tc0DirInWorld = f3(1, 0, 0);
        }
        qGeomNormal = encode_dir(geomNormalInWorld);
        qTexCoord = encode_uv(tu, tv);
        const gfx_material& mat = a.scene.materials[matSlot];
        Bsdf bsdf; bsdf.setup(a.scene, mat, tu, tv);
        Frame frame(shadingNormalInWorld, tc0DirInWorld);
        if (a.f.enableBumpMapping) apply_bump_mapping(read_modified_normal(a.scene, mat, tu, tv), frame);
        const f3 vOutLocal = frame.to_local(unit(-direction));
        shadingNormalInWorld = frame.n;
        qTangent = encode_dir(frame.t);
        albedo = bsdf.dh_reflectance_estimate(vOutLocal);
    }
    else {
        const f3 vOut = -direction;
        const f3 pp = -vOut;
        float posPhi, posTheta;
        to_polar_yup(pp, posPhi, posTheta);
        const float phi = posPhi + a.f.envLightRotation;
        float u = phi / (2 * kPi);
        u -= floorf(u);
        const float v = posTheta / kPi;
        positionInWorld = pp;
        prevPositionInWorld = pp;
        qGeomNormal = encode_dir(vOut);
        shadingNormalInWorld = vOut;
        qTangent = encode_dir(f3(-gm_cos(posPhi), 0, -gm_sin(posPhi)));
        qTexCoord = encode_uv(u, v);
        qbcB = encode_bc(u);
        qbcC = encode_bc(v);
    }

    const Camera prevCam = load_camera(a.f.prevCamera);
    float sx, sy;
    calc_screen_position(prevCam, prevPositionInWorld, sx, sy);
    float mvx = (x + 0.5f) - sx * a.s.imageSizeX;
    float mvy = (y + 0.5f) - sy * a.s.imageSizeY;
    if (a.f.resetFlowBuffer || prevPositionInWorld.x != prevPositionInWorld.x) { mvx = 0.0f; mvy = 0.0f; }

    static_cast<uint4*>(a.s.gbuffer0[bufIdx])[p] = make_uint4(instSlot, geomInstSlot, primIndex, qbcB | (qbcC << 16));
    static_cast<float2*>(a.s.gbuffer1[bufIdx])[p] = make_float2(mvx, mvy);
    static_cast<float4*>(a.s.gbuffer2[bufIdx])[p] = make_float4(positionInWorld.x, positionInWorld.y, positionInWorld.z, bits2f(qGeomNormal));
    static_cast<uint4*>(a.s.gbuffer3[bufIdx])[p] = make_uint4(encode_dir(shadingNormalInWorld), qTangent, qTexCoord, matSlot);

    float4* albedoAcc = static_cast<float4*>(a.s.albedoAccumBuffer) + p;
    float4* normalAcc = static_cast<float4*>(a.s.normalAccumBuffer) + p;
    f3 prevAlbedo(0.0f), prevNormal(0.0f);
    if (a.f.numAccumFrames > 0) {
        const float4 pa = *albedoAcc, pn = *normalAcc;
        prevAlbedo = f3(pa.x, pa.y, pa.z);
        prevNormal = f3(pn.x, pn.y, pn.z);
    }
    const float curWeight = 1.0f / (1 + a.f.numAccumFrames);
    const f3 albedoResult = (1 - curWeight) * prevAlbedo + curWeight * albedo;
    const f3 normalResult = (1 - curWeight) * prevNormal + curWeight * shadingNormalInWorld;
    *albedoAcc = make_float4(albedoResult.x, albedoResult.y, albedoResult.z, 1.0f);
    *normalAcc = make_float4(normalResult.x, normalResult.y, normalResult.z, 1.0f);
}
__global__ __launch_bounds__(kBlock) void k_gbuffer_resolve(RestirArgs a) {
    const PixelId px = pixel_of_thread(a.px);
    if (!px.valid) return;
    const float4 rd = a.rayDir[px.slot];
    gbuffer_resolve(a, px, a.hits[px.slot], f3(rd.x, rd.y, rd.z));
}

#ifndef GFX_INIT_WAVES
#define GFX_INIT_WAVES 4
#endif
struct LcgJump { uint64_t mul, add; };
constexpr LcgJump lcg_jump(uint32_t n) {
    LcgJump j = { 1ull, 0ull };
    for (uint32_t k = 0; k < n; ++k) { j.add = j.add * 6364136223846793005ULL + 1ull; j.mul = j.mul * 6364136223846793005ULL; }
    return j;
}
template <int CTRL> GFX_DEV float quad_perm(float v) {
    return bits2f(static_cast<uint32_t>(__builtin_amdgcn_update_dpp(0, static_cast<int>(f2bits(v)), CTRL, 0xF, 0xF, false)));
}
template <int CTRL> GFX_DEV int quad_perm(int v) { return __builtin_amdgcn_update_dpp(0, v, CTRL, 0xF, 0xF, false); }
template <int SPLIT>
GFX_DEV PixelId pixel_of_split_thread(const PixelGrid& g, uint32_t& sub, uint32_t block) {
    if (SPLIT == 1) { sub = 0u; return pixel_of_block_thread(g, block, threadIdx.x); }
    const uint32_t launchThread = block * kBlock + threadIdx.x;
    sub = launchThread & (SPLIT - 1);
    return pixel_of_block_thread(g, (launchThread / SPLIT) / kBlock, (launchThread / SPLIT) % kBlock);
}
struct CandidateRay { bool writer, want; f3 org, dir; float tmax; };
template <bool EMITTER_TEX, int SPLIT>
GFX_DEV CandidateRay initial_candidates(const RestirArgs& a, uint4* waveBuf, int lane, const PixelId& px, uint32_t sub) {
    static_assert(SPLIT == 1 || SPLIT == 2 || SPLIT == 4, "a pixel's lanes are an aligned pair or quad");
    const size_t numPixels = static_cast<size_t>(a.s.imageSizeX) * a.s.imageSizeY;
    const size_t p = px.p;
    const uint32_t bufIdx = a.f.bufferIndex;
    bool surface = false;
    if (px.valid) surface = static_cast<const uint4*>(a.s.gbuffer0[bufIdx])[p].x != 0xFFFFFFFFu;

    bool wantRay = false;
    f3 rayO(0.0f), rayD(0.0f);
    float rayTmax = 0;
    const EnvMap env = load_env(a.s);
    const bool envEnabled = env.present() && a.f.enableEnvLight;
    ShadingPoint sp;
    uint64_t* rngBuf = static_cast<uint64_t*>(a.s.rngBuffer);
    Pcg32 rng; rng.state = 0;
    if (surface) {
        const Camera cam = load_camera(a.f.camera);
        make_shading_point(a, bufIdx, p, cam.pos, false, sp);
        rng.state = rngBuf[p];
        if (SPLIT > 1 && sub > 0) {
            constexpr LcgJump j1 = lcg_jump(4), j2 = lcg_jump(8), j3 = lcg_jump(12);
            rng.state = rng.state * (sub == 1 ? j1.mul : sub == 2 ? j2.mul : j3.mul) + (sub == 1 ? j1.add : sub == 2 ? j2.add : j3.add);
        }
    }
    Reservoir reservoir;
    reservoir.reset();
    float selectedTarget = 0.0f;
    float sumWeights = 0.0f;
    int lastAccepted = -1;
    const uint32_t numCandidates = 1u << a.f.log2NumCandidateSamples;
    GFX_CYC_BEGIN
    for (uint32_t i = sub; i < numCandidates; i += SPLIT) {
        GFX_PROF(0);
        GFX_CYC(0);
        float probCurType = 1.0f, u0 = 0.0f, u1 = 0.0f;
        bool sampleEnv = false;
        LightPick pk; pk.rec = 0; pk.instSlot = 0; pk.density = 0.0f; pk.partialProb = 0.0f; pk.ok = false; pk.table = true;
        if (surface) {
            if (SPLIT > 1 && i >= SPLIT) {
                constexpr LcgJump skip = lcg_jump(4 * (SPLIT - 1));
                rng.state = rng.state * skip.mul + skip.add;
            }
            float ul = rng.uniform();
            if (envEnabled) {
                if (*a.scene.lightInstIntegral > 0.0f) {
                    const float prob = fmin2(fmax2(0.25f * numCandidates - i, 0.0f), 1.0f);
                    if (prob == 1.0f) { probCurType = 0.25f; sampleEnv = true; }
                    else if (prob == 0.0f) probCurType = 1.0f - 0.25f;
                    else if (ul < prob) { probCurType = 0.25f; ul = ul / prob; sampleEnv = true; }
                    else { probCurType = 1.0f - 0.25f; ul = (ul - prob) / (1 - prob); }
                }
                else sampleEnv = true;
            }
            u0 = rng.uniform();
            u1 = rng.uniform();
            if (!sampleEnv) pk = light_select(a.scene, ul);
        }
        GFX_CYC(1);
        const bool fetch = surface && !sampleEnv && pk.ok;
        uint4 q0 = make_uint4(0u, 0u, 0u, 0u), q1 = q0, q2 = q0, q3 = q0;
        m33 normalMatrix;
        normalMatrix.r0 = normalMatrix.r1 = normalMatrix.r2 = f3(0.0f);
        if (__ballot(fetch) != 0ull) {
            coop_fetch64_issue(fetch ? pk.rec : kCoopNone, reinterpret_cast<const char*>(a.scene.emitterRecs), waveBuf, lane);
            coop_fetch64_wait();
            if (fetch) coop_fetch64_read(waveBuf, lane, q0, q1, q2, q3);
            if (fetch) normalMatrix = load_m33_rows(a.scene.lightNormalMatrices + 16u * emitter_matrix_index(q3.w));
        }
        GFX_CYC(2);
        if (surface) {
            LightSample ls;
            ls.emittance = f3(0.0f); ls.position = f3(0.0f); ls.normal = f3(0.0f); ls.atInfinity = 0;
            float pd = 0.0f;
            PendingEmittance pending; pending.tex = 0u; pending.rec = 0u; pending.bcA = pending.bcB = pending.bcC = 0.0f;
            if (sampleEnv) sample_env_light(env, a.f.envLightRotation, a.f.envLightPowerCoeff, u0, u1, ls, pd);
            else if (pk.ok) {
                GFX_PROF(1);
                light_from_record<EMITTER_TEX, false>(a.scene, pk, as_float4(q0), as_float4(q1), as_float4(q2), as_float4(q3), normalMatrix, u0, u1, ls, pd,
                                                      f3(0.0f), EMITTER_TEX ? &pending : nullptr);
            }
            GFX_CYC(3);
            const f3 cont = EMITTER_TEX ? direct_lighting_pending(a.scene, sp.pos, sp.vOutLocal, sp.frame, sp.bsdf, ls, pending)
                                        : direct_lighting(sp.pos, sp.vOutLocal, sp.frame, sp.bsdf, ls);
            GFX_CYC(4);
            pd *= probCurType;
            const float target = target_weight(cont);
            const float weight = target / pd;
            if (SPLIT == 1) {
                if (reservoir.update(ls, weight, rng.uniform())) { GFX_PROF(5); selectedTarget = target; }
            }
            else {
                const float u = rng.uniform();
                float s = sumWeights + weight;
#pragma unroll
                for (int j = 1; j < SPLIT; ++j) {
                    const float before = SPLIT == 2 ? quad_perm<0xA0>(s) : quad_perm<0x90>(s);
                    if (sub >= static_cast<uint32_t>(j)) s = before + weight;
                }
                if (u < weight / s) { GFX_PROF(5); reservoir.sample = ls; selectedTarget = target; lastAccepted = static_cast<int>(i); }
                sumWeights = SPLIT == 2 ? quad_perm<0xF5>(s) : quad_perm<0xFF>(s);
            }
        }
    }
    bool writer = true;
    if (SPLIT > 1) {
        int last = lastAccepted;
        last = max(last, quad_perm<0xB1>(last));
        if (SPLIT == 4) last = max(last, quad_perm<0x4E>(last));
        writer = last < 0 ? sub == 0 : lastAccepted == last;
        reservoir.sumWeights = sumWeights;
        reservoir.streamLength = numCandidates;
        if (surface && sub == SPLIT - 1) rngBuf[p] = rng.state;
    }
    GFX_CYC(5);
    if (surface && writer) {
        GFX_PROF(8);
        float recPDF = reservoir.sumWeights / (selectedTarget * reservoir.streamLength);
        if (!is_finite(recPDF)) { recPDF = 0.0f; selectedTarget = 0.0f; }

        if (a.f.reuseVisibility && selectedTarget > 0.0f) {
            const ShadowRay sr = shadow_ray(sp.pos, reservoir.sample);
            wantRay = true; rayO = sp.pos; rayD = sr.dir; rayTmax = sr.tmax;
        }
        if (SPLIT == 1) rngBuf[p] = rng.state;
        store_reservoir(a.s.reservoirBuffer[a.curRes], numPixels, p, reservoir);
        static_cast<float2*>(a.s.reservoirInfoBuffer[a.curRes])[p] = make_float2(recPDF, selectedTarget);
    }
    GFX_CYC_END;
    CandidateRay r;
    r.writer = writer; r.want = wantRay; r.org = rayO; r.dir = rayD; r.tmax = rayTmax;
    return r;
}
template <bool EMITTER_TEX, int SPLIT>
__global__ __launch_bounds__(kBlock) __attribute__((amdgpu_waves_per_eu(GFX_INIT_WAVES, GFX_INIT_WAVES))) void k_initial_candidates(RestirArgs a, uint32_t* __restrict__ blockCost) {
    __shared__ __attribute__((aligned(16))) uint4 fetchBuf[(kBlock / 64) * 256];
    const int lane = threadIdx.x & 63;
    uint4* waveBuf = fetchBuf + 256 * __builtin_amdgcn_readfirstlane(threadIdx.x >> 6);
    const uint32_t block = launch_block(a.px);
    const unsigned long long t0 = blockCost ? __builtin_amdgcn_s_memtime() : 0ull;
    uint32_t sub;
    const PixelId px = pixel_of_split_thread<SPLIT>(a.px, sub, block);
    const CandidateRay r = initial_candidates<EMITTER_TEX, SPLIT>(a, waveBuf, lane, px, sub);
    if (r.writer) {
        const uint32_t slot = emit_ray_at_slot(px, r.want, r.org, r.dir, 0.0f, r.tmax, a);
        if (px.valid) a.pixelRaySlot[px.p] = slot;
    }
    if (blockCost && lane == 0) atomicMax(blockCost + block, static_cast<uint32_t>((__builtin_amdgcn_s_memtime() - t0) >> 11));
}

template <int MODE>
GFX_DEV void temporal_reuse(const RestirArgs& a, const PixelId& px, bool occluded) {
    const size_t numPixels = static_cast<size_t>(a.s.imageSizeX) * a.s.imageSizeY;
    if (!px.valid) return;
    const size_t p = px.p;
    const uint32_t bufIdx = a.f.bufferIndex;
    if (static_cast<const uint4*>(a.s.gbuffer0[bufIdx])[p].x == 0xFFFFFFFFu) return;
    const int x = px.x, y = px.y;

    float2* infoBuf = static_cast<float2*>(a.s.reservoirInfoBuffer[a.curRes]);
    float2 info = infoBuf[p];
    float recPDF = info.x, selectedTarget = info.y;
    if (occluded) { recPDF = 0.0f; selectedTarget = 0.0f; }
    if (MODE == 0) {
        infoBuf[p] = make_float2(recPDF, selectedTarget);
        return;
    }
    constexpr bool unbiased = MODE == 2;
    const Camera cam = load_camera(a.f.camera);
    ShadingPoint sp;
    make_shading_point(a, bufIdx, p, cam.pos, false, sp);
    uint64_t* rngBuf = static_cast<uint64_t*>(a.s.rngBuffer);
    Pcg32 rng; rng.state = rngBuf[p];
    Reservoir reservoir = load_reservoir(a.s.reservoirBuffer[a.curRes], numPixels, p);

    const uint32_t prevBuf = (bufIdx + 1) % 2;
    const uint32_t prevRes = (a.curRes + 1) % 2;
    bool neighborIsSelected = false;
    const uint32_t selfStreamLength = reservoir.streamLength;
    if (recPDF == 0.0f) reservoir.reset();
    uint32_t combinedStreamLength = selfStreamLength;
    const uint32_t maxPrevStreamLength = 20 * selfStreamLength;
    const float2 mv = static_cast<const float2*>(a.s.gbuffer1[bufIdx])[p];
    const int nbx = f2i_sat(x + 0.5f - mv.x);
    const int nby = f2i_sat(y + 0.5f - mv.y);
    const bool accepted = test_neighbor(a, !unbiased, prevBuf, nbx, nby, sp.dist, sp.frame.n, cam.pos);
    size_t np = 0;
    Reservoir neighbor;
    if (accepted) {
        np = static_cast<size_t>(nby) * a.s.imageSizeX + nbx;
        neighbor = load_reservoir(a.s.reservoirBuffer[prevRes], numPixels, np);
        const float2 nbInfo = static_cast<const float2*>(a.s.reservoirInfoBuffer[prevRes])[np];
        const f3 cont = direct_lighting(sp.pos, sp.vOutLocal, sp.frame, sp.bsdf, neighbor.sample);
        const float target = target_weight(cont);
        const uint32_t nbStreamLength = min(neighbor.streamLength, maxPrevStreamLength);
        const float weight = target * nbInfo.x * nbStreamLength;
        if (reservoir.update(neighbor.sample, weight, rng.uniform())) {
            selectedTarget = target;
            if (unbiased) neighborIsSelected = true;
        }
        combinedStreamLength += nbStreamLength;
    }
    reservoir.streamLength = combinedStreamLength;

    float weightForEstimate;
    if (unbiased) {
        const LightSample selected = reservoir.sample;
        float numWeight, denomWeight;
        {
            const f3 cont = direct_lighting(sp.pos, sp.vOutLocal, sp.frame, sp.bsdf, selected);
            const float targetSelf = target_weight(cont);
            numWeight = targetSelf;
            denomWeight = targetSelf * selfStreamLength;
        }
        if (accepted) {
            const Camera prevCam = load_camera(a.f.prevCamera);
            ShadingPoint nsp;
            make_shading_point(a, prevBuf, np, prevCam.pos, true, nsp);
            const f3 cont = direct_lighting(nsp.pos, nsp.vOutLocal, nsp.frame, nsp.bsdf, selected);
            const float nbTarget = target_weight(cont);
            const uint32_t nbStreamLength = min(neighbor.streamLength, maxPrevStreamLength);
            denomWeight += nbTarget * nbStreamLength;
            if (neighborIsSelected) numWeight = nbTarget;
        }
        weightForEstimate = numWeight / denomWeight;
    }
    else weightForEstimate = 1.0f / reservoir.streamLength;

    recPDF = weightForEstimate * reservoir.sumWeights / selectedTarget;
    if (!is_finite(recPDF)) { recPDF = 0.0f; selectedTarget = 0.0f; }

    rngBuf[p] = rng.state;
    store_reservoir(a.s.reservoirBuffer[a.curRes], numPixels, p, reservoir);
    infoBuf[p] = make_float2(recPDF, selectedTarget);
}
template <int MODE>
__global__ __launch_bounds__(kBlock) void k_temporal(RestirArgs a) {
    const PixelId px = pixel_of_thread(a.px);
    if (!px.valid) return;
    const uint32_t slot = a.pixelRaySlot[px.p];
    temporal_reuse<MODE>(a, px, slot != GFX_INVALID_SLOT && a.occluded[slot] != 0u);
}

GFX_DEV void spatial_neighbor(const RestirArgs& a, Pcg32& rng, uint32_t nIdx, int x, int y, int& nbx, int& nby) {
    float radius = a.f.spatialNeighborRadius;
    float dx, dy;
    if (a.f.useLowDiscrepancyNeighbors) {
        const float2 d = static_cast<const float2*>(a.s.spatialNeighborDeltas)[(a.baseIdx + nIdx) % 1024];
        dx = radius * d.x;
        dy = radius * d.y;
    }
    else {
        radius *= sqrtf(rng.uniform());
        const float angle = 2 * kPi * rng.uniform();
        float s, c;
        gm_sincos(angle, s, c);
        dx = radius * c;
        dy = radius * s;
    }
    nbx = f2i_sat(x + 0.5f + dx);
    nby = f2i_sat(y + 0.5f + dy);
}

struct SpatialSelection {
    bool surface;
    ShadingPoint sp;
    Pcg32 rng;
    Reservoir combined;
    float selectedTarget;
    int32_t selectedNeighborIndex;
    uint32_t selfStreamLength;
};
template <bool UNBIASED>
GFX_DEV void spatial_select(const RestirArgs& a, const PixelId& px, const Camera& cam, SpatialSelection& s) {
    const size_t numPixels = static_cast<size_t>(a.s.imageSizeX) * a.s.imageSizeY;
    const size_t p = px.p;
    const uint32_t bufIdx = a.f.bufferIndex;
    const uint32_t numNb = a.f.numSpatialNeighbors;
    s.surface = false;
    if (px.valid) s.surface = static_cast<const uint4*>(a.s.gbuffer0[bufIdx])[p].x != 0xFFFFFFFFu;
    const int x = px.x, y = px.y;
    const uint32_t srcRes = a.curRes;
    s.rng.state = 0;
    s.combined.reset();
    s.selectedTarget = 0.0f;
    s.selectedNeighborIndex = -1;
    s.selfStreamLength = 0;
    const uint64_t* rngBuf = static_cast<const uint64_t*>(a.s.rngBuffer);
    if (s.surface) {
        make_shading_point(a, bufIdx, p, cam.pos, false, s.sp);
        s.rng.state = rngBuf[p];
        const Reservoir self = load_reservoir(a.s.reservoirBuffer[srcRes], numPixels, p);
        const float2 selfInfo = static_cast<const float2*>(a.s.reservoirInfoBuffer[srcRes])[p];
        if (selfInfo.x > 0.0f) { s.combined = self; s.selectedTarget = selfInfo.y; }
        s.selfStreamLength = self.streamLength;
        uint32_t combinedStreamLength = self.streamLength;
        for (uint32_t nIdx = 0; nIdx < numNb; ++nIdx) {
            int nbx, nby;
            spatial_neighbor(a, s.rng, nIdx, x, y, nbx, nby);
            const bool accepted = test_neighbor(a, !UNBIASED, bufIdx, nbx, nby, s.sp.dist, s.sp.frame.n, cam.pos) && (nbx != x || nby != y);
            if (accepted) {
                const size_t np = static_cast<size_t>(nby) * a.s.imageSizeX + nbx;
                const Reservoir neighbor = load_reservoir(a.s.reservoirBuffer[srcRes], numPixels, np);
                const float2 nbInfo = static_cast<const float2*>(a.s.reservoirInfoBuffer[srcRes])[np];
                const f3 cont = direct_lighting(s.sp.pos, s.sp.vOutLocal, s.sp.frame, s.sp.bsdf, neighbor.sample);
                const float target = target_weight(cont);
                const uint32_t nbStreamLength = neighbor.streamLength;
                const float weight = target * nbInfo.x * nbStreamLength;
                if (s.combined.update(neighbor.sample, weight, s.rng.uniform())) {
                    s.selectedTarget = target;
                    if (UNBIASED) s.selectedNeighborIndex = static_cast<int32_t>(nIdx);
                }
                combinedStreamLength += nbStreamLength;
            }
        }
        s.combined.streamLength = combinedStreamLength;
    }
}
struct MisTerm { float target; uint32_t streamLength; bool want, evaluated; f3 ro, rd; float tmax; };
GFX_DEV MisTerm spatial_mis_term(const RestirArgs& a, const PixelId& px, SpatialSelection& s, const Camera& prevCam, uint32_t k) {
    const size_t numPixels = static_cast<size_t>(a.s.imageSizeX) * a.s.imageSizeY;
    const uint32_t bufIdx = a.f.bufferIndex;
    const bool needMis = s.surface && s.selectedTarget > 0.0f;
    const LightSample selected = s.combined.sample;
    MisTerm t; t.target = 0.0f; t.streamLength = 0; t.want = false; t.evaluated = false; t.ro = f3(0.0f); t.rd = f3(0.0f); t.tmax = 0;
    if (k == 0) {
        t.streamLength = s.selfStreamLength; t.evaluated = true;
        if (needMis) {
            const f3 cont = direct_lighting(s.sp.pos, s.sp.vOutLocal, s.sp.frame, s.sp.bsdf, selected);
            t.target = target_weight(cont);
            if (a.f.reuseVisibility && t.target > 0.0f) {
                const ShadowRay sr = shadow_ray(s.sp.pos, selected);
                t.want = true; t.ro = s.sp.pos; t.rd = sr.dir; t.tmax = sr.tmax;
            }
        }
        return t;
    }
    if (needMis) {
        const int x = px.x, y = px.y;
        int nbx, nby;
        spatial_neighbor(a, s.rng, k - 1, x, y, nbx, nby);
        const bool accepted = (nbx >= 0 && nbx < a.s.imageSizeX && nby >= 0 && nby < a.s.imageSizeY) && (nbx != x || nby != y);
        if (accepted) {
            const size_t np = static_cast<size_t>(nby) * a.s.imageSizeX + nbx;
            if (static_cast<const uint4*>(a.s.gbuffer0[bufIdx])[np].x != 0xFFFFFFFFu) {
                ShadingPoint nsp;
                make_shading_point(a, bufIdx, np, prevCam.pos, true, nsp);
                const Reservoir neighbor = load_reservoir(a.s.reservoirBuffer[a.curRes], numPixels, np);
                const f3 cont = direct_lighting(nsp.pos, nsp.vOutLocal, nsp.frame, nsp.bsdf, selected);
                t.target = target_weight(cont);
                t.streamLength = neighbor.streamLength;
                t.evaluated = true;
                if (a.f.reuseVisibility && t.target > 0.0f) {
                    const ShadowRay sr = shadow_ray(nsp.pos, selected);
                    t.want = true; t.ro = nsp.pos; t.rd = sr.dir; t.tmax = sr.tmax;
                }
            }
        }
    }
    return t;
}
struct MisSum {
    float numWeight, denomWeight; bool visibility;
    GFX_DEV void begin() { numWeight = 0.0f; denomWeight = 0.0f; visibility = true; }
    GFX_DEV void add(const RestirArgs& a, uint32_t k, float target, uint32_t streamLength, bool evaluated, bool occluded, int32_t selectedNeighborIndex) {
        if (k == 0) {
            float targetSelf = target;
            if (occluded) targetSelf = 0.0f;
            if (a.f.reuseVisibility) visibility = targetSelf > 0.0f;
            numWeight = targetSelf;
            denomWeight = targetSelf * streamLength;
            return;
        }
        if (!evaluated) return;
        float nbTarget = target;
        if (occluded) nbTarget = 0.0f;
        denomWeight += nbTarget * streamLength;
        if (static_cast<int32_t>(k - 1) == selectedNeighborIndex) numWeight = nbTarget;
    }
    GFX_DEV float weight(const RestirArgs& a) const {
        float w = numWeight / denomWeight;
        if (a.f.reuseVisibility && !visibility) w = 0.0f;
        return w;
    }
};
template <bool UNBIASED>
GFX_DEV void spatial_reuse(const RestirArgs& a, const PixelId& px) {
    const size_t numPixels = static_cast<size_t>(a.s.imageSizeX) * a.s.imageSizeY;
    const size_t p = px.p;
    const uint32_t numNb = a.f.numSpatialNeighbors;
    const uint32_t dstRes = (a.curRes + 1) % 2;
    const Camera cam = load_camera(a.f.camera);
    uint64_t* rngBuf = static_cast<uint64_t*>(a.s.rngBuffer);
    SpatialSelection sel;
    spatial_select<UNBIASED>(a, px, cam, sel);
    const bool surface = sel.surface;
    Reservoir& combined = sel.combined;

    if (!UNBIASED) {
        if (!surface) return;
        const float weightForEstimate = 1.0f / combined.streamLength;
        float recPDF = weightForEstimate * combined.sumWeights / sel.selectedTarget;
        float target = sel.selectedTarget;
        if (!is_finite(recPDF)) { recPDF = 0.0f; target = 0.0f; }
        rngBuf[p] = sel.rng.state;
        store_reservoir(a.s.reservoirBuffer[dstRes], numPixels, p, combined);
        static_cast<float2*>(a.s.reservoirInfoBuffer[dstRes])[p] = make_float2(recPDF, target);
        return;
    }

    SpatialSlot* slots = a.spatialScratch + (px.valid ? p * (numNb + 1) : 0);
    const Camera prevCam = load_camera(a.f.prevCamera);
    auto store_term = [&](uint32_t k, const MisTerm& t, uint32_t slot) {
        if (!t.evaluated) slot = kSlotSkipped;
        if (px.valid) { SpatialSlot s; s.targetDensity = t.target; s.streamLength = t.streamLength; s.raySlot = slot; slots[k] = s; }
    };
    constexpr int kBatch = 4;
    if (numNb + 1 <= static_cast<uint32_t>(kBatch)) {
        MisTerm terms[kBatch];
        bool want[kBatch];
#pragma unroll
        for (int k = 0; k < kBatch; ++k) {
            if (static_cast<uint32_t>(k) <= numNb) terms[k] = spatial_mis_term(a, px, sel, prevCam, static_cast<uint32_t>(k));
            else { terms[k].want = false; terms[k].evaluated = false; }
            want[k] = terms[k].want;
        }
        uint32_t raySlots[kBatch];
        queue_reserve<kBatch>(want, a.rayCount, raySlots);
#pragma unroll
        for (int k = 0; k < kBatch; ++k) {
            if (static_cast<uint32_t>(k) > numNb) continue;
            queue_write(raySlots[k], terms[k].ro, terms[k].rd, 0.0f, terms[k].tmax, a.rayOrg, a.rayDir);
            store_term(static_cast<uint32_t>(k), terms[k], raySlots[k]);
        }
    }
    else {
        {
            const MisTerm t = spatial_mis_term(a, px, sel, prevCam, 0u);
            store_term(0, t, emit_ray(t.want, t.ro, t.rd, 0.0f, t.tmax, a));
        }
        for (uint32_t k = 1; k <= numNb; ++k) {
            const MisTerm t = spatial_mis_term(a, px, sel, prevCam, k);
            store_term(k, t, emit_ray(t.want, t.ro, t.rd, 0.0f, t.tmax, a));
        }
    }
    if (!surface) return;
    rngBuf[p] = sel.rng.state;
    store_reservoir(a.s.reservoirBuffer[dstRes], numPixels, p, combined);
    static_cast<float2*>(a.s.reservoirInfoBuffer[dstRes])[p] = make_float2(bits2f(static_cast<uint32_t>(sel.selectedNeighborIndex)), sel.selectedTarget);
}
template <bool UNBIASED>
__global__ __launch_bounds__(kBlock) __attribute__((amdgpu_waves_per_eu(4))) void k_spatial(RestirArgs a) { spatial_reuse<UNBIASED>(a, pixel_of_thread(a.px)); }

__global__ __launch_bounds__(kBlock) void k_spatial_mis_finish(RestirArgs a) {
    const size_t numPixels = static_cast<size_t>(a.s.imageSizeX) * a.s.imageSizeY;
    const PixelId px = pixel_of_thread(a.px);
    if (!px.valid) return;
    const size_t p = px.p;
    const uint32_t bufIdx = a.f.bufferIndex;
    if (static_cast<const uint4*>(a.s.gbuffer0[bufIdx])[p].x == 0xFFFFFFFFu) return;
    const uint32_t numNb = a.f.numSpatialNeighbors;
    const uint32_t dstRes = (a.curRes + 1) % 2;
    float2* infoBuf = static_cast<float2*>(a.s.reservoirInfoBuffer[dstRes]);
    const float2 stash = infoBuf[p];
    const int32_t selectedNeighborIndex = static_cast<int32_t>(f2bits(stash.x));
    const float selectedTarget = stash.y;
    const float sumWeights = static_cast<const float4*>(a.s.reservoirBuffer[dstRes])[2 * numPixels + p].z;
    const SpatialSlot* slots = a.spatialScratch + p * (numNb + 1);

    float weightForEstimate = 0.0f;
    if (selectedTarget > 0.0f) {
        MisSum sum;
        sum.begin();
        for (uint32_t k = 0; k <= numNb; ++k) {
            const SpatialSlot s = slots[k];
            const bool rayed = s.raySlot != GFX_INVALID_SLOT && s.raySlot != kSlotSkipped;
            sum.add(a, k, s.targetDensity, s.streamLength, s.raySlot != kSlotSkipped, rayed && a.occluded[s.raySlot] != 0u, selectedNeighborIndex);
        }
        weightForEstimate = sum.weight(a);
    }
    float recPDF = weightForEstimate * sumWeights / selectedTarget;
    float target = selectedTarget;
    if (!is_finite(recPDF)) { recPDF = 0.0f; target = 0.0f; }
    infoBuf[p] = make_float2(recPDF, target);
}

struct ShadeState { bool want; f3 ro, rd; float tmax; f3 contribution, direct; float recPDF; };
GFX_DEV ShadeState shade_prepare(const RestirArgs& a, const PixelId& px, uint32_t curRes) {
    const size_t numPixels = static_cast<size_t>(a.s.imageSizeX) * a.s.imageSizeY;
    const size_t p = px.p;
    const uint32_t bufIdx = a.f.bufferIndex;
    bool want = false;
    f3 ro(0.0f), rd(0.0f); float tmax = 0;
    f3 contribution(0.01f, 0.01f, 0.01f);
    f3 direct(0.0f);
    float recPDF = 0.0f;
    if (px.valid) {
        const uint32_t instSlot = static_cast<const uint4*>(a.s.gbuffer0[bufIdx])[p].x;
        const uint4 g3 = static_cast<const uint4*>(a.s.gbuffer3[bufIdx])[p];
        if (instSlot != 0xFFFFFFFFu) {
            const Camera cam = load_camera(a.f.camera);
            ShadingPoint sp;
            make_shading_point(a, bufIdx, p, cam.pos, true, sp);
            const gfx_material& mat = a.scene.materials[g3.w];
            const Reservoir reservoir = load_reservoir(a.s.reservoirBuffer[curRes], numPixels, p);
            recPDF = static_cast<const float2*>(a.s.reservoirInfoBuffer[curRes])[p].x;
            contribution = f3(0.0f);
            if (sp.vOutLocal.z > 0) {
                float tu, tv;
                decode_uv(g3.z, tu, tv);
                const f3 e = material_emittance(a.scene, mat, tu, tv);
                contribution = contribution + e / kPi;
            }
            if (recPDF > 0 && is_finite(recPDF)) {
                const bool visDone = a.f.reuseVisibility && (!a.f.enableTemporalReuse || (a.f.enableSpatialReuse && a.f.useUnbiasedEstimator));
                direct = direct_lighting(sp.pos, sp.vOutLocal, sp.frame, sp.bsdf, reservoir.sample);
                if (!visDone) {
                    if (direct.x != 0.0f || direct.y != 0.0f || direct.z != 0.0f) {
                        const ShadowRay sr = shadow_ray(sp.pos, reservoir.sample);
                        want = true; ro = sp.pos; rd = sr.dir; tmax = sr.tmax;
                    }
                }
            }
        }
        else {
            const EnvMap env = load_env(a.s);
            if (env.present() && a.f.enableEnvLight) {
                const float u = (g3.z & 0xFFFF) / 65535.0f, v = (g3.z >> 16) / 65535.0f;
                contribution = a.f.envLightPowerCoeff * env.fetch(u, v);
            }
        }
    }
    ShadeState st;
    st.want = want; st.ro = ro; st.rd = rd; st.tmax = tmax; st.contribution = contribution; st.direct = direct; st.recPDF = recPDF;
    return st;
}
__global__ __launch_bounds__(kBlock) void k_shade_prepare(RestirArgs a) {
    const PixelId px = pixel_of_thread(a.px);
    const ShadeState st = shade_prepare(a, px, a.curRes);
    const uint32_t slot = emit_ray_at_slot(px, st.want, st.ro, st.rd, 0.0f, st.tmax, a);
    if (px.valid) {
        a.shadeScratch[2 * px.p] = make_float4(st.contribution.x, st.contribution.y, st.contribution.z, bits2f(slot));
        a.shadeScratch[2 * px.p + 1] = make_float4(st.direct.x, st.direct.y, st.direct.z, st.recPDF);
    }
}

__global__ __launch_bounds__(kBlock) void k_spatial_shade_prepare(RestirArgs a) {
    const PixelId px = pixel_of_thread(a.px);
    spatial_reuse<false>(a, px);
    const ShadeState st = shade_prepare(a, px, (a.curRes + 1) % 2);
    const uint32_t slot = emit_ray_at_slot(px, st.want, st.ro, st.rd, 0.0f, st.tmax, a);
    if (px.valid) {
        a.shadeScratch[2 * px.p] = make_float4(st.contribution.x, st.contribution.y, st.contribution.z, bits2f(slot));
        a.shadeScratch[2 * px.p + 1] = make_float4(st.direct.x, st.direct.y, st.direct.z, st.recPDF);
    }
}

GFX_DEV void shade_finish(const RestirArgs& a, const PixelId& px, f3 contribution, f3 direct, float recPDF, bool occluded) {
    const size_t p = px.p;
    const uint32_t bufIdx = a.f.bufferIndex;
    if (static_cast<const uint4*>(a.s.gbuffer0[bufIdx])[p].x != 0xFFFFFFFFu) {
        if (occluded) direct = f3(0.0f);
        contribution = contribution + recPDF * direct;
    }
    float4* beauty = static_cast<float4*>(a.s.beautyAccumBuffer) + p;
    f3 prev(0.0f);
    if (a.f.numAccumFrames > 0) { const float4 b = *beauty; prev = f3(b.x, b.y, b.z); }
    const float curWeight = 1.0f / (1 + a.f.numAccumFrames);
    const f3 result = (1 - curWeight) * prev + curWeight * contribution;
    *beauty = make_float4(result.x, result.y, result.z, 1.0f);
}
__global__ __launch_bounds__(kBlock) void k_shade_finish(RestirArgs a) {
    const PixelId px = pixel_of_thread(a.px);
    if (!px.valid) return;
    const float4 c0 = a.shadeScratch[2 * px.p], c1 = a.shadeScratch[2 * px.p + 1];
    const uint32_t slot = f2bits(c0.w);
    shade_finish(a, px, f3(c0.x, c0.y, c0.z), f3(c1.x, c1.y, c1.z), c1.w, slot != GFX_INVALID_SLOT && a.occluded[slot] != 0u);
}

__global__ __launch_bounds__(kBlock) void k_gbuffer_fused(RestirArgs a, DevAccel accel, gfx_hit* hits, uint2* spill, int spillCap, int useHint, uint32_t* __restrict__ blockCost) {
    __shared__ uint2 ldsStack[kLdsStackDepth * kBlock];
    __shared__ __attribute__((aligned(16))) uint4 fetchBuf[(kBlock / 64) * 256];
    const int tid = threadIdx.x, lane = tid & 63;
    uint4* waveBuf = fetchBuf + 256 * __builtin_amdgcn_readfirstlane(tid >> 6);
    const uint32_t block = launch_block(a.px);
    const PixelId px = pixel_of_block_thread(a.px, block, threadIdx.x);
    const RayPair r = primary_ray(a, px);
    const uint32_t hint = useHint ? hits[px.slot].triIndex : 0xFFFFFFFFu;
    uint32_t steps = 0;
    const RayHit h = trace_wave_local<false>(accel, true, f3(r.org.x, r.org.y, r.org.z), f3(r.dir.x, r.dir.y, r.dir.z), r.org.w, r.dir.w, ldsStack + tid, kBlock,
                                             spill + (static_cast<size_t>(blockIdx.x) * kBlock + tid) * spillCap, spillCap, waveBuf, lane, hint, &steps);
    if (blockCost && lane == 0) atomicMax(blockCost + block, steps);
    gfx_hit gh; gh.dist = h.t; gh.bcB = h.bcB; gh.bcC = h.bcC; gh.triIndex = h.tri;
    hits[px.slot] = gh;
    if (px.valid) gbuffer_resolve(a, px, gh, f3(r.dir.x, r.dir.y, r.dir.z));
}

template <bool EMITTER_TEX, int SPLIT, int MODE>
__global__ __launch_bounds__(kBlock) __attribute__((amdgpu_waves_per_eu(GFX_INIT_WAVES, GFX_INIT_WAVES))) void k_initial_fused(RestirArgs a, DevAccel accel, uint2* spill, int spillCap, uint32_t* __restrict__ blockCost) {
    static_assert(SPLIT == 1 || SPLIT == 4, "one lane per pixel, or four with the block's rays gathered in its first wave");
    constexpr int kRays = kBlock / SPLIT;
    __shared__ __attribute__((aligned(16))) uint4 fetchBuf[(kBlock / 64) * 256];
    __shared__ uint2 ownStack[SPLIT == 1 ? kLdsStackDepth * kBlock : 1];
    static_assert(SPLIT == 1 || kLdsStackDepth * kRays * sizeof(uint2) <= 2 * 256 * sizeof(uint4), "the stack of 64 rays fits the buffers of waves 1 and 2");
    const int tid = threadIdx.x, lane = tid & 63;
    const int wave = __builtin_amdgcn_readfirstlane(tid >> 6);
    uint4* waveBuf = fetchBuf + 256 * wave;
    const uint32_t block = launch_block(a.px);
    uint32_t sub;
    PixelId px = pixel_of_split_thread<SPLIT>(a.px, sub, block);
    const CandidateRay r = initial_candidates<EMITTER_TEX, SPLIT>(a, waveBuf, lane, px, sub);
    float4 org = make_float4(r.org.x, r.org.y, r.org.z, 0.0f), dir = make_float4(r.dir.x, r.dir.y, r.dir.z, r.want ? r.tmax : -1.0f);
    uint2* stack = ownStack + tid;
    if (SPLIT > 1) {
        float4* handOver = reinterpret_cast<float4*>(fetchBuf + 256 * (tid >> 6) + 224);
        if (r.writer) { handOver[2 * ((tid & 63) / SPLIT)] = org; handOver[2 * ((tid & 63) / SPLIT) + 1] = dir; }
        __syncthreads();
        if (tid >= kRays) return;
        const float4* from = reinterpret_cast<const float4*>(fetchBuf + 256 * (tid >> 4) + 224);
        org = from[2 * (tid & 15)]; dir = from[2 * (tid & 15) + 1];
        const uint32_t t = block * kRays + tid;
        px = pixel_of_block_thread(a.px, t / kBlock, t % kBlock);
        stack = reinterpret_cast<uint2*>(fetchBuf + 256) + tid;
    }
    const bool want = dir.w > org.w;
    uint32_t steps = 0;
    const RayHit h = trace_wave_local<true>(accel, want, f3(org.x, org.y, org.z), f3(dir.x, dir.y, dir.z), org.w, dir.w, stack, kRays,
                                            spill + (static_cast<size_t>(blockIdx.x) * kRays + tid) * spillCap, spillCap, waveBuf, lane, 0xFFFFFFFFu, &steps);
    if (blockCost && lane == 0) atomicMax(blockCost + block, steps);
    temporal_reuse<MODE>(a, px, want && h.tri != GFX_INVALID_SLOT);
}

__global__ __launch_bounds__(1024) void k_order_blocks(uint32_t* __restrict__ cost, uint32_t n, uint32_t* __restrict__ order) {
    __shared__ uint32_t start[256];
    if (threadIdx.x < 256) start[threadIdx.x] = 0u;
    __syncthreads();
    for (uint32_t i = threadIdx.x; i < n; i += 1024) atomicAdd(&start[255u - min(cost[i], 255u)], 1u);
    __syncthreads();
    if (threadIdx.x == 0) {
        uint32_t sum = 0;
        for (int c = 0; c < 256; ++c) { const uint32_t k = start[c]; start[c] = sum; sum += k; }
    }
    __syncthreads();
    for (uint32_t i = threadIdx.x; i < n; i += 1024) {
        order[atomicAdd(&start[255u - min(cost[i], 255u)], 1u)] = i;
        cost[i] = 0u;
    }
}

void block_order_begin(Context& ctx, hipStream_t stream, int which, uint32_t blocks, uint64_t key, uint32_t minBlocks, const uint32_t*& order, uint32_t*& cost) {
    order = nullptr; cost = nullptr;
    if (!ctx.tune.blockOrder || blocks <= minBlocks) return;
    Context::BlockOrder& bo = ctx.blockOrders[which];
    if (bo.key != key || bo.blocks != blocks) {
        if (bo.ordered) GFX_HIP(hipStreamWaitEvent(stream, bo.ordered, 0));
        bo.cost.reserve(sizeof(uint32_t) * blocks); bo.order.reserve(sizeof(uint32_t) * blocks);
        GFX_HIP(hipMemsetAsync(bo.cost.p, 0, sizeof(uint32_t) * blocks, stream));
        bo.key = key; bo.blocks = blocks; bo.valid = false;
    }
    cost = bo.cost.as<uint32_t>();
    if (bo.valid) { GFX_HIP(hipStreamWaitEvent(stream, bo.ordered, 0)); order = bo.order.as<uint32_t>(); }
}
void block_order_end(Context& ctx, hipStream_t stream, int which, uint32_t blocks, uint32_t* cost) {
    if (!cost) return;
    Context::BlockOrder& bo = ctx.blockOrders[which];
    if (!ctx.auxStream) GFX_HIP(hipStreamCreateWithFlags(&ctx.auxStream, hipStreamNonBlocking));
    if (!bo.counted) { GFX_HIP(hipEventCreateWithFlags(&bo.counted, hipEventDisableTiming)); GFX_HIP(hipEventCreateWithFlags(&bo.ordered, hipEventDisableTiming)); }
    GFX_HIP(hipEventRecord(bo.counted, stream));
    GFX_HIP(hipStreamWaitEvent(ctx.auxStream, bo.counted, 0));
    hipLaunchKernelGGL(k_order_blocks, dim3(1), dim3(1024), 0, ctx.auxStream, cost, blocks, bo.order.as<uint32_t>());
    GFX_HIP(hipGetLastError());
    GFX_HIP(hipEventRecord(bo.ordered, ctx.auxStream));
    bo.valid = true;
}

template <bool SPATIAL_FIRST>
__global__ __launch_bounds__(kBlock) void k_shading_fused(RestirArgs a, DevAccel accel, uint2* spill, int spillCap, uint32_t* __restrict__ blockCost) {
    __shared__ uint2 ldsStack[kLdsStackDepth * kBlock];
    __shared__ __attribute__((aligned(16))) uint4 fetchBuf[(kBlock / 64) * 256];
    const int tid = threadIdx.x, lane = tid & 63;
    uint4* waveBuf = fetchBuf + 256 * __builtin_amdgcn_readfirstlane(tid >> 6);
    const uint32_t block = launch_block(a.px);
    const PixelId px = pixel_of_block_thread(a.px, block, threadIdx.x);
    if (SPATIAL_FIRST) spatial_reuse<false>(a, px);
    const ShadeState st = shade_prepare(a, px, SPATIAL_FIRST ? (a.curRes + 1) % 2 : a.curRes);
    uint32_t steps = 0;
    const RayHit h = trace_wave_local<true>(accel, st.want, st.ro, st.rd, 0.0f, st.tmax, ldsStack + tid, kBlock,
                                            spill + (static_cast<size_t>(blockIdx.x) * kBlock + tid) * spillCap, spillCap, waveBuf, lane, 0xFFFFFFFFu, &steps);
    if (blockCost && lane == 0) atomicMax(blockCost + block, steps);
    if (px.valid) shade_finish(a, px, st.contribution, st.direct, st.recPDF, st.want && h.tri != GFX_INVALID_SLOT);
}

#ifdef GFX_LANE_PROFILE
extern "C" int gfx_debug_lane_profile(unsigned long long* out64, int reset) {
    if (hipMemcpyFromSymbol(out64, HIP_SYMBOL(g_laneProfile), sizeof(g_laneProfile)) != hipSuccess) return 1;
    if (reset) { unsigned long long zero[64] = {}; if (hipMemcpyToSymbol(HIP_SYMBOL(g_laneProfile), zero, sizeof(zero)) != hipSuccess) return 1; }
    return 0;
}
#endif

static RestirArgs make_args(Context& ctx, uint32_t width, uint32_t height, uint32_t rowBegin, uint32_t rowEnd, bool rearch, uint32_t gapBegin = 0, uint32_t gapEnd = 0) {
    const RestirParams& rp = ctx.restir;
    if (!rp.valid) throw HipError("gfx_restir_launch: gfx_restir_set_params has not been called");
    if (static_cast<uint32_t>(rp.s.imageSizeX) != width || static_cast<uint32_t>(rp.s.imageSizeY) != height)
        throw HipError("gfx_restir_launch: launch size differs from imageSize in the static parameters");
    const uint64_t h = rp.f.travHandle;
    if (h == 0 || h > ctx.accels.size() || !ctx.accels[h - 1]) throw HipError("gfx_restir_launch: invalid travHandle");
    const size_t numPixels = static_cast<size_t>(width) * height;
    const size_t frameSlots = static_cast<size_t>(make_pixel_grid(ctx, width, 0, height).launchBlocks) * kBlock;
    const size_t maxRays = std::max(frameSlots, numPixels * std::max<size_t>(1 + rp.f.numSpatialNeighbors, rearch ? kRearchRayKinds : 1));
    ctx.rayOrg.reserve(16 * maxRays); ctx.rayDir.reserve(16 * maxRays);
    ctx.rayOut.reserve(4 * maxRays);
    ctx.rayHits.reserve(sizeof(gfx_hit) * numPixels);
    ctx.pixelRaySlot.reserve(4 * numPixels);
    ctx.shadeScratch.reserve(32 * numPixels);
    ctx.spatialScratch.reserve(sizeof(SpatialSlot) * maxRays);
    ctx.smallCounters.reserve(kSmallCountersBytes);
    RestirArgs a;
    a.scene = ctx.devScene();
    a.s = rp.s; a.f = rp.f;
    a.curRes = rp.currentReservoirIndex & 1u;
    a.baseIdx = rp.spatialNeighborBaseIndex & 1023u;
    a.rayOrg = ctx.rayOrg.as<float4>(); a.rayDir = ctx.rayDir.as<float4>();
    a.rayCount = ctx.smallCounters.as<uint32_t>() + 4;
    a.pixelRaySlot = ctx.pixelRaySlot.as<uint32_t>();
    a.occluded = ctx.rayOut.as<uint32_t>();
    a.hits = ctx.rayHits.as<gfx_hit>();
    a.tris = ctx.accels[h - 1]->trisPtr();
    a.shadeScratch = ctx.shadeScratch.as<float4>();
    a.spatialScratch = ctx.spatialScratch.as<SpatialSlot>();
    a.rearchSlots = nullptr;
    if (rearch) {
        ctx.rearchSlots.reserve(sizeof(uint32_t) * kRearchRayKinds * numPixels);
        a.rearchSlots = ctx.rearchSlots.as<uint32_t>();
    }
    if (rowEnd > height || rowBegin > rowEnd) throw HipError("gfx_restir_launch_rows: row range outside the image");
    if (gapEnd > gapBegin && (gapBegin < rowBegin || gapEnd > rowEnd)) throw HipError("gfx_restir_launch_rows_gap: the gap lies outside the rows");
    a.px = make_pixel_grid(ctx, width, rowBegin, rowEnd, gapBegin, gapEnd);
    return a;
}

template <typename K>
static void launch_pixels(Context& ctx, hipStream_t stream, const char* name, K kernel, const RestirArgs& a) {
    if (a.px.rowEnd == a.px.rowBegin) return;
    ScopedKernelTimer timer(ctx, stream, name);
    hipLaunchKernelGGL(kernel, dim3(a.px.launchBlocks), dim3(kBlock), 0, stream, a);
    GFX_HIP(hipGetLastError());
}

static void trace_queue(Context& ctx, hipStream_t stream, const RestirArgs& a, int mode, uint32_t fixedCount, bool useCounter, void* out) {
    TraceLaunch t;
    t.accel = ctx.accels[ctx.restir.f.travHandle - 1]->dev();
    t.rayOrgTmin = a.rayOrg; t.rayDirTmax = a.rayDir;
    t.numRays = fixedCount; t.numRaysPtr = useCounter ? a.rayCount : nullptr;
    t.out = out; t.mode = mode;
    trace_launch(ctx, stream, t);
}

__global__ __launch_bounds__(kBlock) void k_copy_to_linear(gfx_restir_static_params s, uint32_t bufferIndex, size_t numPixels,
                                                           float4* __restrict__ color, float4* __restrict__ albedo, float4* __restrict__ normal, float2* __restrict__ motion) {
    const size_t p = static_cast<size_t>(blockIdx.x) * kBlock + threadIdx.x;
    if (p >= numPixels) return;
    color[p] = static_cast<const float4*>(s.beautyAccumBuffer)[p];
    albedo[p] = static_cast<const float4*>(s.albedoAccumBuffer)[p];
    const float4 nv = static_cast<const float4*>(s.normalAccumBuffer)[p];
    f3 n(nv.x, nv.y, nv.z);
    if (n.x != 0 || n.y != 0 || n.z != 0) n = unit(n);
    normal[p] = make_float4(n.x, n.y, n.z, 1.0f);
    motion[p] = static_cast<const float2*>(s.gbuffer1[bufferIndex])[p];
}
__global__ __launch_bounds__(kBlock) void k_visualize(const void* __restrict__ linearBuffer, int bufferType, float mvOffset, float mvScale,
                                                      size_t numPixels, float4* __restrict__ out) {
    const size_t p = static_cast<size_t>(blockIdx.x) * kBlock + threadIdx.x;
    if (p >= numPixels) return;
    float4 value = make_float4(0.0f, 0.0f, 0.0f, 0.0f);
    switch (bufferType) {
    case GFX_DISPLAY_NOISY_BEAUTY: case GFX_DISPLAY_DENOISED_BEAUTY: case GFX_DISPLAY_ALBEDO:
        value = static_cast<const float4*>(linearBuffer)[p];
        break;
    case GFX_DISPLAY_NORMAL:
        value = static_cast<const float4*>(linearBuffer)[p];
        value.x = 0.5f + 0.5f * value.x; value.y = 0.5f + 0.5f * value.y; value.z = 0.5f + 0.5f * value.z;
        break;
    case GFX_DISPLAY_FLOW: {
        const float2 f = static_cast<const float2*>(linearBuffer)[p];
        value = make_float4(fminf(fmaxf(mvScale * f.x + mvOffset, 0.0f), 1.0f), fminf(fmaxf(mvScale * f.y + mvOffset, 0.0f), 1.0f), mvOffset, 1.0f);
        break;
    }
    default: break;
    }
    out[p] = value;
}
void restir_copy_to_linear(Context& ctx, hipStream_t stream, void* color, void* albedo, void* normal, void* motion) {
    if (!ctx.restir.valid) throw HipError("gfx_restir_copy_to_linear: gfx_restir_set_params first");
    const gfx_restir_static_params& s = ctx.restir.s;
    const size_t n = static_cast<size_t>(s.imageSizeX) * s.imageSizeY;
    if (!n) return;
    hipLaunchKernelGGL(k_copy_to_linear, dim3(static_cast<uint32_t>((n + kBlock - 1) / kBlock)), dim3(kBlock), 0, stream, s, ctx.restir.f.bufferIndex, n,
                       static_cast<float4*>(color), static_cast<float4*>(albedo), static_cast<float4*>(normal), static_cast<float2*>(motion));
    GFX_HIP(hipGetLastError());
}
void restir_visualize(Context& ctx, hipStream_t stream, const void* linearBuffer, int bufferType, float mvOffset, float mvScale, uint32_t width, uint32_t height, void* out) {
    (void)ctx;
    const size_t n = static_cast<size_t>(width) * height;
    if (!n) return;
    hipLaunchKernelGGL(k_visualize, dim3(static_cast<uint32_t>((n + kBlock - 1) / kBlock)), dim3(kBlock), 0, stream, linearBuffer, bufferType, mvOffset, mvScale, n,
                       static_cast<float4*>(out));
    GFX_HIP(hipGetLastError());
}

void restir_launch(Context& ctx, hipStream_t stream, int pass, uint32_t width, uint32_t height, uint32_t rowBegin, uint32_t rowEnd, uint32_t gapBegin, uint32_t gapEnd) {
    const bool rearch = pass >= GFX_RESTIR_LIGHT_PRESAMPLING && pass <= GFX_RESTIR_SHADE_AND_RESAMPLE_SPATIOTEMPORAL;
    if (gapEnd > gapBegin && pass != GFX_RESTIR_SPATIAL_BIASED) throw HipError("gfx_restir_launch_rows_gap: only GFX_RESTIR_SPATIAL_BIASED takes a gap");
    RestirArgs a = make_args(ctx, width, height, rowBegin, rowEnd, rearch, gapBegin, gapEnd);
    if (rowEnd == rowBegin || a.px.launchBlocks == 0) return;
    auto reset_queue = [&]() { GFX_HIP(hipMemsetAsync(a.rayCount, 0, sizeof(uint32_t), stream)); };
    const uint32_t launchWaves = a.px.launchBlocks * (kBlock / 64), waveSlots = static_cast<uint32_t>(ctx.numCUs) * 4u * GFX_INIT_WAVES;
    const bool smallLaunch = launchWaves <= waveSlots + waveSlots / 2;
    const bool fusableLaunch = 2u * launchWaves <= 9u * waveSlots;
    const int spillCap = static_cast<int>(local_spill_depth(ctx.accels[ctx.restir.f.travHandle - 1]->maxDepth));
    const size_t fusedSpillBytes = sizeof(uint2) * static_cast<size_t>(a.px.launchBlocks) * kBlock * spillCap;
    const bool fused = !ctx.countersEnabled && fusedSpillBytes <= (size_t(1) << 30) && (ctx.tune.fusePasses == 2 || (ctx.tune.fusePasses == 0 && fusableLaunch));
    const uint64_t orderKey = (static_cast<uint64_t>(rowBegin) << 44) ^ (static_cast<uint64_t>(rowEnd) << 24) ^ (static_cast<uint64_t>(width) << 4);
    const uint32_t orderMinBlocks = 8u * static_cast<uint32_t>(ctx.numCUs);
    auto block_order_begin = [&](int which, uint32_t blocks, uint32_t variant, const uint32_t*& order, uint32_t*& cost) {
        gfx::block_order_begin(ctx, stream, which, blocks, orderKey ^ variant, orderMinBlocks, order, cost);
        a.px.order = order;
    };
    auto block_order_end = [&](int which, uint32_t blocks, uint32_t* cost) { gfx::block_order_end(ctx, stream, which, blocks, cost); };
    switch (pass) {
    case GFX_RESTIR_SETUP_GBUFFERS: {
        const size_t frameSlots = static_cast<size_t>(make_pixel_grid(ctx, width, 0, height).launchBlocks) * kBlock;
        const uint32_t numSlots = a.px.launchBlocks * kBlock;
        ctx.gbRayOrg.reserve(16 * frameSlots); ctx.gbRayDir.reserve(16 * frameSlots);
        if (sizeof(gfx_hit) * frameSlots > ctx.gbRayHits.bytes) {
            ctx.gbRayHits.reserve(sizeof(gfx_hit) * frameSlots);
            GFX_HIP(hipMemsetAsync(ctx.gbRayHits.p, 0xFF, ctx.gbRayHits.bytes, stream));
        }
        a.rayOrg = ctx.gbRayOrg.as<float4>(); a.rayDir = ctx.gbRayDir.as<float4>();
        a.hits = ctx.gbRayHits.as<gfx_hit>();
        if (!ctx.countersEnabled && fusedSpillBytes <= (size_t(1) << 30) && ctx.tune.fusePasses != 1) {
            ctx.gbSpill.reserve(fusedSpillBytes);
            const uint32_t* order = nullptr;
            uint32_t* cost = nullptr;
            block_order_begin(2, a.px.launchBlocks, 0u, order, cost);
            {
                ScopedKernelTimer timer(ctx, stream, "gbuffer_fused");
                hipLaunchKernelGGL(k_gbuffer_fused, dim3(a.px.launchBlocks), dim3(kBlock), 0, stream, a, ctx.accels[ctx.restir.f.travHandle - 1]->dev(),
                                   ctx.gbRayHits.as<gfx_hit>(), ctx.gbSpill.as<uint2>(), spillCap, ctx.tune.temporalHints ? 1 : 0, cost);
                GFX_HIP(hipGetLastError());
            }
            block_order_end(2, a.px.launchBlocks, cost);
            break;
        }
        launch_pixels(ctx, stream, "primary_rays", k_primary_rays, a);
        TraceLaunch t;
        t.accel = ctx.accels[ctx.restir.f.travHandle - 1]->dev();
        t.rayOrgTmin = a.rayOrg; t.rayDirTmax = a.rayDir;
        t.numRays = numSlots; t.numRaysPtr = nullptr;
        t.out = ctx.gbRayHits.p; t.mode = GFX_TRACE_CLOSEST;
        t.spill = &ctx.gbSpill; t.counters = &ctx.gbCounters;
        t.hintFromOut = true;
        trace_launch(ctx, stream, t);
        launch_pixels(ctx, stream, "gbuffer_resolve", k_gbuffer_resolve, a);
        break;
    }
    case GFX_RESTIR_INITIAL_RIS:
    case GFX_RESTIR_INITIAL_AND_TEMPORAL_BIASED:
    case GFX_RESTIR_INITIAL_AND_TEMPORAL_UNBIASED:
        {
            const uint32_t numCandidates = 1u << a.f.log2NumCandidateSamples;
            uint32_t split = ctx.tune.candidateSplit > 0 ? static_cast<uint32_t>(ctx.tune.candidateSplit) : smallLaunch ? 4u : 1u;
            split = std::min(split, numCandidates);
            if (fused && split == 2) split = 1;
            const uint32_t grid = a.px.launchBlocks * split;
            if (fused) {
                ctx.spill.reserve(fusedSpillBytes);
                const DevAccel accel = ctx.accels[ctx.restir.f.travHandle - 1]->dev();
                const int mode = pass == GFX_RESTIR_INITIAL_RIS ? 0 : pass == GFX_RESTIR_INITIAL_AND_TEMPORAL_BIASED ? 1 : 2;
                const bool tex = a.scene.emitterTexRefs != nullptr;
                void (*kernel)(RestirArgs, DevAccel, uint2*, int, uint32_t*) = nullptr;
#define GFX_PICK(TEX, SPLIT) (mode == 0 ? k_initial_fused<TEX, SPLIT, 0> : mode == 1 ? k_initial_fused<TEX, SPLIT, 1> : k_initial_fused<TEX, SPLIT, 2>)
                if (tex) kernel = split == 4 ? GFX_PICK(true, 4) : GFX_PICK(true, 1);
                else kernel = split == 4 ? GFX_PICK(false, 4) : GFX_PICK(false, 1);
#undef GFX_PICK
                const uint32_t* order = nullptr;
                uint32_t* cost = nullptr;
                block_order_begin(0, grid, split, order, cost);
                {
                    ScopedKernelTimer timer(ctx, stream, "initial_fused");
                    hipLaunchKernelGGL(kernel, dim3(grid), dim3(kBlock), 0, stream, a, accel, ctx.spill.as<uint2>(), spillCap, cost);
                    GFX_HIP(hipGetLastError());
                }
                block_order_end(0, grid, cost);
                break;
            }
            void (*kernel)(RestirArgs, uint32_t*) = a.scene.emitterTexRefs
                ? (split == 4 ? k_initial_candidates<true, 4> : split == 2 ? k_initial_candidates<true, 2> : k_initial_candidates<true, 1>)
                : (split == 4 ? k_initial_candidates<false, 4> : split == 2 ? k_initial_candidates<false, 2> : k_initial_candidates<false, 1>);
            const uint32_t* order = nullptr;
            uint32_t* cost = nullptr;
            block_order_begin(3, grid, split, order, cost);
            {
                ScopedKernelTimer timer(ctx, stream, "initial_candidates");
                hipLaunchKernelGGL(kernel, dim3(grid), dim3(kBlock), 0, stream, a, cost);
                GFX_HIP(hipGetLastError());
            }
            block_order_end(3, grid, cost);
            a.px.order = nullptr;
        }
        trace_queue(ctx, stream, a, GFX_TRACE_ANY, a.px.launchBlocks * kBlock, false, ctx.rayOut.p);
        if (pass == GFX_RESTIR_INITIAL_RIS) launch_pixels(ctx, stream, "temporal_none", k_temporal<0>, a);
        else if (pass == GFX_RESTIR_INITIAL_AND_TEMPORAL_BIASED) launch_pixels(ctx, stream, "temporal_biased", k_temporal<1>, a);
        else launch_pixels(ctx, stream, "temporal_unbiased", k_temporal<2>, a);
        break;
    case GFX_RESTIR_SPATIAL_BIASED:
        launch_pixels(ctx, stream, "spatial_biased", k_spatial<false>, a);
        break;
    case GFX_RESTIR_SPATIAL_UNBIASED:
        reset_queue();
        launch_pixels(ctx, stream, "spatial_unbiased_select", k_spatial<true>, a);
        trace_queue(ctx, stream, a, GFX_TRACE_ANY, 0, true, ctx.rayOut.p);
        launch_pixels(ctx, stream, "spatial_unbiased_finish", k_spatial_mis_finish, a);
        break;
    case GFX_RESTIR_SPATIAL_BIASED_AND_SHADING:
    case GFX_RESTIR_SHADING:
        if (fused) {
            ctx.spill.reserve(fusedSpillBytes);
            const bool both = pass == GFX_RESTIR_SPATIAL_BIASED_AND_SHADING;
            const uint32_t* order = nullptr;
            uint32_t* cost = nullptr;
            block_order_begin(1, a.px.launchBlocks, both ? 1u : 0u, order, cost);
            {
                ScopedKernelTimer timer(ctx, stream, both ? "spatial_shading_fused" : "shading_fused");
                hipLaunchKernelGGL(both ? k_shading_fused<true> : k_shading_fused<false>, dim3(a.px.launchBlocks), dim3(kBlock), 0, stream, a,
                                   ctx.accels[ctx.restir.f.travHandle - 1]->dev(), ctx.spill.as<uint2>(), spillCap, cost);
                GFX_HIP(hipGetLastError());
            }
            block_order_end(1, a.px.launchBlocks, cost);
            break;
        }
        if (pass == GFX_RESTIR_SPATIAL_BIASED_AND_SHADING) launch_pixels(ctx, stream, "spatial_shade_prepare", k_spatial_shade_prepare, a);
        else launch_pixels(ctx, stream, "shade_prepare", k_shade_prepare, a);
        trace_queue(ctx, stream, a, GFX_TRACE_ANY, a.px.launchBlocks * kBlock, false, ctx.rayOut.p);
        launch_pixels(ctx, stream, "shade_finish", k_shade_finish, a);
        break;
    case GFX_RESTIR_LIGHT_PRESAMPLING: {
        if (!a.s.lightPreSamplingRngs || !a.s.preSampledLights) throw HipError("gfx_restir_launch: light pre-sampling buffers are not set");
        ScopedKernelTimer timer(ctx, stream, "light_presample");
        hipLaunchKernelGGL(k_light_presample, dim3(kNumPreSampledLights / kBlock), dim3(kBlock), 0, stream, a);
        GFX_HIP(hipGetLastError());
        break;
    }
    case GFX_RESTIR_PER_PIXEL_RIS: {
        if (rowBegin % 8 != 0) throw HipError("gfx_restir_launch_rows: per-pixel RIS bands must start on an 8-row tile boundary");
        const uint32_t tilesX = (width + 7) / 8, tileRows = (rowEnd + 7) / 8 - rowBegin / 8;
        const uint32_t numTiles = tilesX * tileRows;
        ScopedKernelTimer timer(ctx, stream, "per_pixel_ris");
        hipLaunchKernelGGL(k_per_pixel_ris, dim3((numTiles + kBlock / 64 - 1) / (kBlock / 64)), dim3(kBlock), 0, stream, a);
        GFX_HIP(hipGetLastError());
        break;
    }
    case GFX_RESTIR_TRACE_SHADOW_RAYS:
    case GFX_RESTIR_TRACE_SHADOW_RAYS_TEMPORAL_BIASED:
    case GFX_RESTIR_TRACE_SHADOW_RAYS_SPATIAL_BIASED:
    case GFX_RESTIR_TRACE_SHADOW_RAYS_SPATIOTEMPORAL_BIASED:
    case GFX_RESTIR_TRACE_SHADOW_RAYS_TEMPORAL_UNBIASED:
    case GFX_RESTIR_TRACE_SHADOW_RAYS_SPATIAL_UNBIASED:
    case GFX_RESTIR_TRACE_SHADOW_RAYS_SPATIOTEMPORAL_UNBIASED: {
        reset_queue();
        void (*emit)(RestirArgs) = nullptr; void (*finish)(RestirArgs) = nullptr;
        switch (pass) {
#define GFX_REARCH_CASE(PASS, T, S, U) case PASS: emit = k_rearch_emit<T, S, U>; finish = k_rearch_vis_finish<T, S, U>; break;
        GFX_REARCH_CASE(GFX_RESTIR_TRACE_SHADOW_RAYS, false, false, false)
        GFX_REARCH_CASE(GFX_RESTIR_TRACE_SHADOW_RAYS_TEMPORAL_BIASED, true, false, false)
        GFX_REARCH_CASE(GFX_RESTIR_TRACE_SHADOW_RAYS_SPATIAL_BIASED, false, true, false)
        GFX_REARCH_CASE(GFX_RESTIR_TRACE_SHADOW_RAYS_SPATIOTEMPORAL_BIASED, true, true, false)
        GFX_REARCH_CASE(GFX_RESTIR_TRACE_SHADOW_RAYS_TEMPORAL_UNBIASED, true, false, true)
        GFX_REARCH_CASE(GFX_RESTIR_TRACE_SHADOW_RAYS_SPATIAL_UNBIASED, false, true, true)
        GFX_REARCH_CASE(GFX_RESTIR_TRACE_SHADOW_RAYS_SPATIOTEMPORAL_UNBIASED, true, true, true)
#undef GFX_REARCH_CASE
        }
        launch_pixels(ctx, stream, "rearch_emit", emit, a);
        trace_queue(ctx, stream, a, GFX_TRACE_ANY, 0, true, ctx.rayOut.p);
        launch_pixels(ctx, stream, "rearch_vis_finish", finish, a);
        break;
    }
    case GFX_RESTIR_SHADE_AND_RESAMPLE: launch_pixels(ctx, stream, "rearch_shade", k_rearch_shade<false, false>, a); break;
    case GFX_RESTIR_SHADE_AND_RESAMPLE_TEMPORAL: launch_pixels(ctx, stream, "rearch_shade_t", k_rearch_shade<true, false>, a); break;
    case GFX_RESTIR_SHADE_AND_RESAMPLE_SPATIAL: launch_pixels(ctx, stream, "rearch_shade_s", k_rearch_shade<false, true>, a); break;
    case GFX_RESTIR_SHADE_AND_RESAMPLE_SPATIOTEMPORAL: launch_pixels(ctx, stream, "rearch_shade_st", k_rearch_shade<true, true>, a); break;
    default:
        throw HipError("gfx_restir_launch: unknown pass");
    }
}

}
```

### gfxexp_amd/csrc/scene.cpp

```cpp
#include <cmath>
#include <cstring>
#include "internal.h"
#include "bc/bc_textures.h"
#include <cstdlib>
#include <map>
#include <array>

namespace gfx {

Context::~Context() {
    for (Accel* a : accels) { if (a) { a->nodes.release(); a->links.release(); a->triIds.release(); a->rootBoxes.release(); delete a; } }
    DevBuf* all[] = { &dMaterials, &dGeomInsts, &dInsts, &dVertices, &dTriangles, &dSlotPool, &dFlatGeoms, &dSubset[0], &dSubset[1], &dLightW, &dLightP, &dLightCDF, &dLightRefs, &dEmitterRecs, &dEmitterRecExtras, &dLightNormalMatrices, &dInstMatrixIndex, &dTextures, &dTexelPool, &dSrgbLut, &dEmitterTexRefs,
                      &rayOrg, &rayDir, &rayOut, &rayHits, &spill, &gbRayOrg, &gbRayDir, &gbRayHits, &gbSpill, &gbCounters, &auxSpill, &auxCounters, &blockOrders[0].cost, &blockOrders[0].order, &blockOrders[1].cost, &blockOrders[1].order, &blockOrders[2].cost, &blockOrders[2].order, &blockOrders[3].cost, &blockOrders[3].order, &blockOrders[4].cost, &blockOrders[4].order, &pixelRaySlot, &shadeScratch, &spatialScratch, &smallCounters,
                      &bTris, &bBoxes, &bKeys, &bKeysAlt, &bVals, &bValsAlt, &bSortTemp, &bNodesLR, &bParents, &bFlags,
                      &bNodeBoxes, &bRanges, &bQueueA, &bQueueB, &bCounters, &dTraceCounters, &dLightInstIntegral, &dLightInstGuide, &dSpans, &dSpanGuide, &dSpanHeader, &dSpanInstBegin,
                      &dTraceDiag, &ptDiag, &bCosts, &bDec, &bFlatIdx, &ptPending, &ptExtOrg, &ptExtDir, &ptExtOwner, &ptState,
                      &rearchSlots, &nrcState, &neeTrainIdx };
    for (NrcNet* net : nrcNets) if (net) nrc_destroy(net);
    for (DevBuf* b : all) b->release();
    for (auto& e : pendingEvents) { (void)hipEventDestroy(e.second.first); (void)hipEventDestroy(e.second.second); }
    for (TicketState& ts : ticketState) if (ts.lastLaunch) (void)hipEventDestroy(ts.lastLaunch);
    for (PinnedStage& st : lightStage) { if (st.done) (void)hipEventDestroy(st.done); if (st.p) (void)hipHostFree(st.p); }
    for (BlockOrder& b : blockOrders) { if (b.counted) (void)hipEventDestroy(b.counted); if (b.ordered) (void)hipEventDestroy(b.ordered); }
    if (auxFork) (void)hipEventDestroy(auxFork);
    if (auxJoin) (void)hipEventDestroy(auxJoin);
    if (auxStream) (void)hipStreamDestroy(auxStream);
}

DevScene Context::devScene() const {
    DevScene s;
    s.materials = dMaterials.as<gfx_material>();
    s.geomInsts = dGeomInsts.as<DevGeomInst>();
    s.insts = dInsts.as<DevInstance>();
    s.vertices = dVertices.as<DevVertex>();
    s.triangles = dTriangles.as<uint32_t>();
    s.geomInstSlotPool = dSlotPool.as<uint32_t>();
    s.lightWeights = dLightW.as<float>();
    s.lightProbs = dLightP.as<float>();
    s.lightCDF = dLightCDF.as<float>();
    s.lightGeomRefs = dLightRefs.as<LightGeomRef>();
    s.emitterRecs = dEmitterRecs.as<EmitterRec>();
    s.emitterRecExtras = dEmitterRecExtras.as<EmitterRecExtra>();
    s.lightNormalMatrices = dLightNormalMatrices.as<float>();
    s.numLightMatrices = numLightMatrices;
    s.lightInstIntegral = dLightInstIntegral.as<float>();
    s.lightInstGuide = dLightInstGuide.as<uint16_t>();
    s.lightInstGuideCells = lightInstGuideCells;
    s.spans = dSpans.as<EmitterSpan>();
    s.spanGuide = dSpanGuide.as<SpanGuide>();
    s.spanHeader = dSpanHeader.as<uint32_t>();
    s.numSpans = numEmitterRecs;
    s.spanGuideCells = spanGuideCells;
    s.textures = dTextures.as<DevTexture>();
    s.texelPool = dTexelPool.as<uint32_t>();
    s.srgbLut = dSrgbLut.as<float>();
    s.emitterTexRefs = anyEmittanceTexture ? dEmitterTexRefs.as<EmitterTexRef>() : nullptr;
    s.lightInstDistOffset = lightInstDistOffset;
    s.numInsts = static_cast<uint32_t>(insts.size());
    return s;
}

static void normal_matrix(const float x[12], float out[12]) {
    const float a = x[0], b = x[1], c = x[2], d = x[4], e = x[5], f = x[6], g = x[8], h = x[9], i = x[10];
    const float det = a * e * i + b * f * g + c * d * h - c * e * g - b * d * i - a * f * h;
    const float r = 1 / det;
    const float inv[9] = {
        (e * i - f * h) * r, -(b * i - c * h) * r, (b * f - c * e) * r,
        -(d * i - f * g) * r, (a * i - c * g) * r, -(a * f - c * d) * r,
        (d * h - e * g) * r, -(a * h - b * g) * r, (a * e - b * d) * r };
    for (int rr = 0; rr < 3; ++rr) {
        for (int cc = 0; cc < 3; ++cc) out[rr * 4 + cc] = inv[cc * 3 + rr];
        out[rr * 4 + 3] = 0.0f;
    }
}

void instance_cur_to_prev(const float prev[12], const float cur[12], float out[12]) {
    float a[16], inv[16];
    for (int k = 0; k < 12; ++k) a[k] = cur[k];
    a[12] = 0.0f; a[13] = 0.0f; a[14] = 0.0f; a[15] = 1.0f;
    for (int i = 0; i < 4; ++i)
        for (int j = 0; j < 4; ++j) {
            int rows[3], cols[3], nr = 0, nc = 0;
            for (int k = 0; k < 4; ++k) { if (k != j) rows[nr++] = k; if (k != i) cols[nc++] = k; }
            auto e = [&](int r, int c) { return a[4 * rows[r] + cols[c]]; };
            const float minor = (e(0, 0) * e(1, 1) * e(2, 2)) - (e(2, 0) * e(1, 1) * e(0, 2)) + (e(1, 0) * e(2, 1) * e(0, 2)) -
                                (e(0, 0) * e(2, 1) * e(1, 2)) + (e(2, 0) * e(0, 1) * e(1, 2)) - (e(1, 0) * e(0, 1) * e(2, 2));
            inv[4 * i + j] = ((i + j) % 2) ? -minor : minor;
        }
    const float recDet = 1.0f / (a[0] * inv[0] + a[4] * inv[1] + a[8] * inv[2] + a[12] * inv[3]);
    for (int k = 0; k < 16; ++k) inv[k] *= recDet;
    for (int i = 0; i < 3; ++i)
        for (int j = 0; j < 4; ++j)
            out[4 * i + j] = prev[4 * i + 0] * inv[0 + j] + prev[4 * i + 1] * inv[4 + j] + prev[4 * i + 2] * inv[8 + j] + prev[4 * i + 3] * inv[12 + j];
}

static void fill_instance_transform(const HostInstance& hi, DevInstance& d) {
    std::memcpy(d.transform, hi.transform, sizeof(float) * 12);
    const float ident[12] = { 1, 0, 0, 0, 0, 1, 0, 0, 0, 0, 1, 0 };
    std::memcpy(d.curToPrevTransform, hi.animated ? hi.curToPrev : ident, sizeof(ident));
    if (hi.hasNormalMatrix)
        for (int rr = 0; rr < 3; ++rr) {
            for (int cc = 0; cc < 3; ++cc) d.normalMatrix[rr * 4 + cc] = hi.normalMatrix[rr * 3 + cc];
            d.normalMatrix[rr * 4 + 3] = 0.0f;
        }
    else normal_matrix(hi.transform, d.normalMatrix);
    d.uniformScale = std::sqrt(hi.transform[0] * hi.transform[0] + hi.transform[4] * hi.transform[4] + hi.transform[8] * hi.transform[8]);
}

void light_matrices_upload(Context& ctx, hipStream_t stream) {
    std::map<std::array<uint32_t, 9>, uint32_t> seen;
    std::vector<float> rows;
    std::vector<uint32_t> index(ctx.hInsts.size(), 0u);
    for (size_t ii = 0; ii < ctx.hInsts.size(); ++ii) {
        const DevInstance& d = ctx.hInsts[ii];
        if (d.distOffset == 0xFFFFFFFFu) continue;
        std::array<uint32_t, 9> key;
        for (int r = 0; r < 3; ++r) for (int c = 0; c < 3; ++c) std::memcpy(&key[3 * r + c], &d.normalMatrix[4 * r + c], 4);
        auto it = seen.find(key);
        if (it == seen.end()) {
            it = seen.emplace(key, static_cast<uint32_t>(seen.size())).first;
            for (int r = 0; r < 3; ++r) { for (int c = 0; c < 3; ++c) rows.push_back(d.normalMatrix[4 * r + c]); rows.push_back(0.0f); }
            rows.insert(rows.end(), 4, 0.0f);
        }
        index[ii] = it->second;
    }
    if (seen.size() > kEmitterMatrixMask + 1u)
        throw HipError("gfx: more than 65536 distinct normal matrices among the emitter instances");
    ctx.numLightMatrices = static_cast<uint32_t>(seen.size());
    ctx.dLightNormalMatrices.reserve(std::max<size_t>(rows.size() * sizeof(float) + 64 * 64, 64));
    ctx.dInstMatrixIndex.reserve(std::max<size_t>(index.size() * sizeof(uint32_t), 16));
    const size_t rowBytes = rows.size() * sizeof(float), indexBytes = index.size() * sizeof(uint32_t);
    if (rowBytes + indexBytes == 0) return;
    Context::PinnedStage& st = ctx.lightStage[ctx.lightStageNext];
    ctx.lightStageNext ^= 1u;
    if (st.done) GFX_HIP(hipEventSynchronize(st.done));
    else GFX_HIP(hipEventCreateWithFlags(&st.done, hipEventDisableTiming));
    if (st.bytes < rowBytes + indexBytes) {
        if (st.p) GFX_HIP(hipHostFree(st.p));
        st.p = nullptr; st.bytes = 0;
        GFX_HIP(hipHostMalloc(&st.p, (rowBytes + indexBytes) * 2, hipHostMallocDefault));
        st.bytes = (rowBytes + indexBytes) * 2;
    }
    char* base = static_cast<char*>(st.p);
    if (rowBytes) { std::memcpy(base, rows.data(), rowBytes); GFX_HIP(hipMemcpyAsync(ctx.dLightNormalMatrices.p, base, rowBytes, hipMemcpyHostToDevice, stream)); }
    if (indexBytes) { std::memcpy(base + rowBytes, index.data(), indexBytes); GFX_HIP(hipMemcpyAsync(ctx.dInstMatrixIndex.p, base + rowBytes, indexBytes, hipMemcpyHostToDevice, stream)); }
    GFX_HIP(hipEventRecord(st.done, stream));
}

void transforms_upload(Context& ctx, hipStream_t stream) {
    if (!ctx.transformsDirty) return;
    for (uint32_t slot : ctx.movedInsts) {
        DevInstance& d = ctx.hInsts[slot];
        fill_instance_transform(ctx.insts[slot], d);
        GFX_HIP(hipMemcpyAsync(ctx.dInsts.as<DevInstance>() + slot, &d, sizeof(DevInstance), hipMemcpyHostToDevice, stream));
    }
    ctx.movedInsts.clear();
    ctx.transformsDirty = false;
    ctx.emitterRecsDirty = true;
    ctx.instDistValid = false;
}

template <typename T>
static void upload(DevBuf& b, const std::vector<T>& v, hipStream_t stream) {
    b.reserve(std::max<size_t>(sizeof(T) * v.size(), 16));
    if (!v.empty()) GFX_HIP(hipMemcpyAsync(b.p, v.data(), sizeof(T) * v.size(), hipMemcpyHostToDevice, stream));
}

void scene_upload(Context& ctx, hipStream_t stream) {
    if (!ctx.sceneDirty) return;
    std::vector<DevVertex> vertices;
    std::vector<uint32_t> triangles;
    std::vector<uint32_t> slotPool;
    ctx.hGeomInsts.assign(ctx.geoms.size(), DevGeomInst());
    uint32_t lightPool = 0;
    for (size_t gi = 0; gi < ctx.geoms.size(); ++gi) {
        const HostGeom& g = ctx.geoms[gi];
        DevGeomInst& d = ctx.hGeomInsts[gi];
        d.vertexOffset = static_cast<uint32_t>(vertices.size());
        d.triangleOffset = static_cast<uint32_t>(triangles.size() / 3);
        d.numVertices = static_cast<uint32_t>(g.vertices.size());
        d.numTriangles = static_cast<uint32_t>(g.triangles.size() / 3);
        if (g.materialSlot >= ctx.materials.size())
            throw std::runtime_error("gfx: a geometry refers to material slot " + std::to_string(g.materialSlot) + " but only " +
                                     std::to_string(ctx.materials.size()) + " materials are set (gfx_material_set)");
        d.materialSlot = g.materialSlot;
        const bool emitter = g.materialSlot < ctx.materials.size() && ctx.materials[g.materialSlot].hasEmittance;
        d.distOffset = emitter ? lightPool : 0xFFFFFFFFu;
        d.distCount = emitter ? d.numTriangles : 0;
        d.distIntegral = 0;
        if (emitter) lightPool += d.numTriangles;
        vertices.insert(vertices.end(), g.vertices.begin(), g.vertices.end());
        triangles.insert(triangles.end(), g.triangles.begin(), g.triangles.end());
    }
    ctx.hInsts.assign(ctx.insts.size(), DevInstance());
    ctx.hFlatGeoms.clear();
    ctx.hSubset[0].clear(); ctx.hSubset[1].clear();
    ctx.subsetTris[0] = ctx.subsetTris[1] = 0;
    uint32_t triCursor = 0;
    for (size_t ii = 0; ii < ctx.insts.size(); ++ii) {
        const HostInstance& hi = ctx.insts[ii];
        DevInstance& d = ctx.hInsts[ii];
        fill_instance_transform(hi, d);
        const std::vector<uint32_t>& slots = ctx.groups[hi.group];
        d.slotsOffset = static_cast<uint32_t>(slotPool.size());
        d.numGeomInsts = static_cast<uint32_t>(slots.size());
        bool hasEmitter = false;
        for (uint32_t s : slots) {
            slotPool.push_back(s);
            if (ctx.hGeomInsts[s].distOffset != 0xFFFFFFFFu) hasEmitter = true;
            DevFlatGeom fg; fg.instSlot = static_cast<uint32_t>(ii); fg.geomInstSlot = s; fg.triBegin = triCursor;
            fg.numTriangles = ctx.hGeomInsts[s].numTriangles;
            triCursor += fg.numTriangles;
            ctx.hFlatGeoms.push_back(fg);
            const int sub = hi.dynamic ? 1 : 0;
            ctx.hSubset[sub].push_back(SubsetGeom{ fg.instSlot, fg.geomInstSlot, ctx.subsetTris[sub], fg.triBegin });
            ctx.subsetTris[sub] += fg.numTriangles;
        }
        d.distOffset = hasEmitter ? lightPool : 0xFFFFFFFFu;
        d.distIntegral = 0;
        if (hasEmitter) lightPool += d.numGeomInsts;
        d.pad[0] = d.pad[1] = d.pad[2] = 0;
    }
    ctx.totalTriangles = triCursor;
    ctx.hLightRefs.assign(lightPool + ctx.insts.size(), LightGeomRef{ 0xFFFFFFFFu, 0xFFFFFFFFu, 0u, 0.0f });
    uint32_t recCursor = 0;
    for (size_t ii = 0; ii < ctx.insts.size(); ++ii) {
        const DevInstance& d = ctx.hInsts[ii];
        if (d.distOffset == 0xFFFFFFFFu) continue;
        for (uint32_t k = 0; k < d.numGeomInsts; ++k) {
            const DevGeomInst& g = ctx.hGeomInsts[slotPool[d.slotsOffset + k]];
            LightGeomRef& r = ctx.hLightRefs[d.distOffset + k];
            r.distOffset = g.distOffset; r.distCount = g.distCount; r.distIntegral = 0.0f;
            if (g.distOffset != 0xFFFFFFFFu) { r.recBase = recCursor; recCursor += g.numTriangles; }
        }
    }
    ctx.numEmitterRecs = recCursor;
    ctx.lightInstDistOffset = lightPool;
    lightPool += static_cast<uint32_t>(ctx.insts.size());
    ctx.lightPoolSize = lightPool;
    ctx.lightsStaticBuilt = false;
    ctx.dLightInstIntegral.reserve(16);
    {
        uint32_t cells = 256;
        while (cells < ctx.insts.size() && cells < 8192) cells *= 2;
        ctx.lightInstGuideCells = cells;
        ctx.dLightInstGuide.reserve(sizeof(uint16_t) * cells);
    }
    GFX_HIP(hipMemsetAsync(ctx.dLightInstIntegral.p, 0, 16, stream));
    {
        uint32_t perRec = GFX_SPAN_CELLS_PER_REC;
        if (const char* e = std::getenv("GFX_SPAN_CELLS_PER_REC")) { const long v = std::atol(e); if (v >= 1 && v <= 64) perRec = static_cast<uint32_t>(v); }
        uint32_t cells = 256;
        while (cells < static_cast<uint64_t>(perRec) * ctx.numEmitterRecs && cells < (1u << 22)) cells *= 2;
        ctx.spanGuideCells = cells;
        ctx.dSpans.reserve(std::max<size_t>(sizeof(EmitterSpan) * ctx.numEmitterRecs, 16));
        ctx.dSpanGuide.reserve(sizeof(SpanGuide) * cells);
        ctx.dSpanHeader.reserve(16);
        ctx.dSpanInstBegin.reserve(sizeof(uint32_t) * (ctx.insts.size() + 1));
        GFX_HIP(hipMemsetAsync(ctx.dSpanHeader.p, 0, 16, stream));
    }

    {
        std::vector<DevTexture> descs(std::max<size_t>(ctx.textures.size(), 1));
        std::vector<uint32_t> pool;
        std::vector<uint32_t> bcSlots;
        for (size_t t = 0; t < ctx.textures.size(); ++t) {
            const HostTexture& ht = ctx.textures[t];
            DevTexture& d = descs[t];
            d.offset = static_cast<uint32_t>(pool.size()); d.width = ht.width; d.height = ht.height; d.format = ht.format;
            if (ht.width != 0 && bc_texture_is(ctx, static_cast<uint32_t>(t))) { bcSlots.push_back(static_cast<uint32_t>(t)); continue; }
            const size_t words = (ht.texels.size() + 3) / 4;
            const size_t at = pool.size();
            pool.resize(at + ((words + 3) & ~size_t(3)), 0u);
            if (!ht.texels.empty()) std::memcpy(pool.data() + at, ht.texels.data(), ht.texels.size());
        }
        if (pool.empty()) pool.resize(4, 0u);
        size_t poolWords = pool.size();
        for (uint32_t t : bcSlots) {
            const HostTexture& ht = ctx.textures[t];
            const size_t bpp = ht.format == GFX_TEX_R8_UNORM ? 1 : (ht.format == GFX_TEX_RG8_UNORM ? 2 : 4);
            const size_t words = (bpp * ht.width * ht.height + 3) / 4;
            if (poolWords >= (1ull << 32)) throw HipError("gfx: texel pool exceeds 16 GiB");
            descs[t].offset = static_cast<uint32_t>(poolWords);
            poolWords += (words + 3) & ~size_t(3);
        }
        if (poolWords >= (1ull << 32)) throw HipError("gfx: texel pool exceeds 16 GiB");
        float lut[256];
        for (int c = 0; c < 256; ++c) {
            const float v = static_cast<float>(c) / 255.0f;
            lut[c] = v <= 0.04045f ? v / 12.92f : std::pow((v + 0.055f) / 1.055f, 2.4f);
        }
        upload(ctx.dTextures, descs, stream);
        ctx.dTexelPool.reserve(sizeof(uint32_t) * poolWords);
        GFX_HIP(hipMemcpyAsync(ctx.dTexelPool.p, pool.data(), sizeof(uint32_t) * pool.size(), hipMemcpyHostToDevice, stream));
        for (uint32_t t : bcSlots)
            bc_texture_expand(ctx, stream, t, descs[t].width, descs[t].height, descs[t].format, ctx.dTexelPool.as<uint32_t>() + descs[t].offset);
        ctx.dSrgbLut.reserve(sizeof(lut));
        GFX_HIP(hipMemcpyAsync(ctx.dSrgbLut.p, lut, sizeof(lut), hipMemcpyHostToDevice, stream));
        GFX_HIP(hipStreamSynchronize(stream));
        for (const gfx_material& m : ctx.materials) {
            const uint32_t slots[5] = { m.texA, m.texB, m.texSmoothness, m.texNormal, m.texEmittance };
            for (uint32_t sl : slots)
                if (sl != 0 && (sl >= ctx.textures.size() || ctx.textures[sl].width == 0)) throw HipError("gfx: material references a texture slot that was never set");
            if (m.hasEmittance && m.texEmittance > kEmitterTexMask) throw HipError("gfx: an emittance texture must sit in a texture slot below 32768");
        }
        ctx.anyEmittanceTexture = false;
        for (const HostGeom& g : ctx.geoms)
            if (g.materialSlot < ctx.materials.size() && ctx.materials[g.materialSlot].hasEmittance && ctx.materials[g.materialSlot].texEmittance != 0) ctx.anyEmittanceTexture = true;
    }
    upload(ctx.dMaterials, ctx.materials, stream);
    upload(ctx.dGeomInsts, ctx.hGeomInsts, stream);
    upload(ctx.dInsts, ctx.hInsts, stream);
    upload(ctx.dVertices, vertices, stream);
    upload(ctx.dTriangles, triangles, stream);
    upload(ctx.dSlotPool, slotPool, stream);
    upload(ctx.dFlatGeoms, ctx.hFlatGeoms, stream);
    upload(ctx.dSubset[0], ctx.hSubset[0], stream);
    upload(ctx.dSubset[1], ctx.hSubset[1], stream);
    ctx.transformsDirty = false; ctx.movedInsts.clear(); ctx.emitterRecsDirty = false; ctx.instDistValid = false;
    upload(ctx.dLightRefs, ctx.hLightRefs, stream);
    ctx.dEmitterRecs.reserve(std::max<size_t>(sizeof(EmitterRec) * ctx.numEmitterRecs, 16));
    ctx.dEmitterRecExtras.reserve(std::max<size_t>(sizeof(EmitterRecExtra) * ctx.numEmitterRecs, 16));
    light_matrices_upload(ctx, stream);
    ctx.dEmitterTexRefs.reserve(std::max<size_t>(ctx.anyEmittanceTexture ? sizeof(EmitterTexRef) * ctx.numEmitterRecs : 0, 16));
    ctx.dLightW.reserve(std::max<size_t>(sizeof(float) * lightPool, 16));
    ctx.dLightCDF.reserve(std::max<size_t>(sizeof(float) * lightPool, 16));
    ctx.dLightP.reserve(std::max<size_t>(sizeof(float) * lightPool, 16));
    GFX_HIP(hipMemsetAsync(ctx.dLightW.p, 0, ctx.dLightW.bytes, stream));
    GFX_HIP(hipMemsetAsync(ctx.dLightP.p, 0, ctx.dLightP.bytes, stream));
    GFX_HIP(hipMemsetAsync(ctx.dLightCDF.p, 0, ctx.dLightCDF.bytes, stream));
    GFX_HIP(hipStreamSynchronize(stream));
    ctx.sceneDirty = false;
}

}
```

Measured before the change: 709.6 Mpaths/s.

## Prefilter ReSTIR candidates with compact per-emitter cull records

Adds a 16-byte per-emitter cull record (octahedral normal, plane offset, half-precision bounding sphere) built alongside the emitter records. The initial-candidate kernel (SPLIT=1 path, on by default) can use it to prove a candidate's contribution is zero, from back-facing or below-horizon tests, before doing the full 64-byte record fetch and shading. This avoids wasted fetches and BSDF evaluation for lights that cannot contribute. In exchange it adds an extra small load and test per candidate, uses precomputed RNG jump tables to keep the random stream consistent, and relies on conservative margins so that no lit candidate is culled.

```diff
diff --git a/gfxexp_amd/csrc/capi.cpp b/gfxexp_amd/csrc/capi.cpp
--- a/gfxexp_amd/csrc/capi.cpp
+++ b/gfxexp_amd/csrc/capi.cpp
@@ -687,6 +687,7 @@
     else if (n == "pt_regen_min") t.ptRegenMin = in(1, 64);
     else if (n == "fuse_passes") t.fusePasses = in(0, 2);
     else if (n == "block_order") t.blockOrder = in(0, 1);
+    else if (n == "candidate_prefilter") t.candidatePrefilter = in(0, 1);
     else if (n == "nrc_staged_infer") t.nrcStagedInfer = in(0, 3);
     else if (n == "candidate_split") { if (value == 3) throw HipError("gfx_tunable_set: candidate_split is 0 (automatic), 1, 2 or 4"); t.candidateSplit = in(0, 4); }
     else throw HipError("gfx_tunable_set: unknown tunable " + n);
diff --git a/gfxexp_amd/csrc/device_types.h b/gfxexp_amd/csrc/device_types.h
--- a/gfxexp_amd/csrc/device_types.h
+++ b/gfxexp_amd/csrc/device_types.h
@@ -2,6 +2,7 @@
 #include <stdint.h>
 #include "../../include/gfxexp.h"
 #include "emitter_spans.h"
+#include "emitter_cull.h"
 
 namespace gfx {
 
@@ -101,6 +102,7 @@
     const LightGeomRef* lightGeomRefs;
     const EmitterRec* emitterRecs;
     const EmitterRecExtra* emitterRecExtras;
+    const EmitterCull* emitterCull;
     const float* lightNormalMatrices;
     uint32_t numLightMatrices;
     const float* lightInstIntegral;
diff --git a/gfxexp_amd/csrc/emitter_cull.h b/gfxexp_amd/csrc/emitter_cull.h
--- /dev/null
+++ b/gfxexp_amd/csrc/emitter_cull.h
@@ -0,0 +1,150 @@
+#pragma once
+#include <stdint.h>
+
+#if defined(__HIP__)
+#define GFX_CULL_HD __attribute__((host)) __attribute__((device)) inline __attribute__((always_inline))
+#else
+#define GFX_CULL_HD inline
+#endif
+
+namespace gfx {
+
+struct alignas(16) EmitterCull {
+    uint32_t octN;
+    float hLo;
+    uint32_t cxy;
+    uint32_t czr;
+};
+static_assert(sizeof(EmitterCull) == 16, "EmitterCull must be 16 bytes");
+
+constexpr float kCullMargin = 1e-3f;
+constexpr float kCullNormalTol = 2e-4f;
+constexpr uint32_t kCullHalfInf = 0x7C00u;
+
+GFX_CULL_HD uint32_t cull_bits(float f) { return __builtin_bit_cast(uint32_t, f); }
+GFX_CULL_HD float cull_float(uint32_t u) { return __builtin_bit_cast(float, u); }
+GFX_CULL_HD float cull_abs(float x) { return cull_float(cull_bits(x) & 0x7FFFFFFFu); }
+GFX_CULL_HD float cull_neg_inf() { return cull_float(0xFF800000u); }
+
+GFX_CULL_HD float cull_half_to_float(uint32_t h) {
+#if defined(__HIP_DEVICE_COMPILE__)
+    return static_cast<float>(__builtin_bit_cast(_Float16, static_cast<uint16_t>(h)));
+#else
+    const uint32_t sign = (h & 0x8000u) << 16, e = (h >> 10) & 0x1Fu, m = h & 0x3FFu;
+    if (e == 0u) return cull_float(sign);
+    if (e == 31u) return cull_float(sign | 0x7F800000u | (m << 13));
+    return cull_float(sign | ((e + 112u) << 23) | (m << 13));
+#endif
+}
+GFX_CULL_HD uint32_t cull_float_to_half_trunc(float x, bool& ok) {
+    const uint32_t u = cull_bits(x), sign = (u >> 16) & 0x8000u;
+    const int32_t e = static_cast<int32_t>((u >> 23) & 0xFFu) - 112;
+    if (e >= 31) { ok = false; return sign; }
+    if (e <= 0) return sign;
+    return sign | (static_cast<uint32_t>(e) << 10) | ((u >> 13) & 0x3FFu);
+}
+GFX_CULL_HD uint32_t cull_float_to_half_up(float x) {
+    if (!(x <= 65504.0f)) return kCullHalfInf;
+    if (!(x >= 6.103515625e-05f)) return 0x0400u;
+    bool ok = true;
+    uint32_t h = cull_float_to_half_trunc(x, ok);
+    if (cull_half_to_float(h) < x) h += 1u;
+    return h;
+}
+
+GFX_CULL_HD void cull_oct_decode(uint32_t q, float& x, float& y, float& z) {
+    const float f = static_cast<float>(q & 0xFFFFu) * (2.0f / 65535.0f) - 1.0f;
+    const float g = static_cast<float>(q >> 16) * (2.0f / 65535.0f) - 1.0f;
+    z = 1.0f - cull_abs(f) - cull_abs(g);
+    const float t = z < 0.0f ? -z : 0.0f;
+    x = f + (f >= 0.0f ? -t : t);
+    y = g + (g >= 0.0f ? -t : t);
+}
+GFX_CULL_HD uint32_t cull_oct_encode(float x, float y, float z) {
+    const float l1 = cull_abs(x) + cull_abs(y) + cull_abs(z);
+    float f = x / l1, g = y / l1;
+    if (z < 0.0f) {
+        const float ff = (1.0f - cull_abs(g)) * (f >= 0.0f ? 1.0f : -1.0f);
+        const float gg = (1.0f - cull_abs(f)) * (g >= 0.0f ? 1.0f : -1.0f);
+        f = ff; g = gg;
+    }
+    auto q16 = [](float v) {
+        const float s = (v * 0.5f + 0.5f) * 65535.0f + 0.5f;
+        return !(s > 0.0f) ? 0u : s >= 65535.0f ? 65535u : static_cast<uint32_t>(s);
+    };
+    return q16(f) | (q16(g) << 16);
+}
+
+GFX_CULL_HD EmitterCull cull_never() {
+    EmitterCull e;
+    e.octN = 0x80008000u; e.hLo = cull_neg_inf(); e.cxy = 0u; e.czr = kCullHalfInf << 16;
+    return e;
+}
+
+GFX_CULL_HD EmitterCull cull_build(const float* m, const float* nA, bool flat, const float* pA, const float* pB, const float* pC, bool finiteEmittance) {
+    EmitterCull e = cull_never();
+    if (!finiteEmittance) return e;
+    const float inf = cull_float(0x7F800000u);
+    const float ax = pB[0] - pA[0], ay = pB[1] - pA[1], az = pB[2] - pA[2];
+    const float bx = pC[0] - pA[0], by = pC[1] - pA[1], bz = pC[2] - pA[2];
+    const float gx = ay * bz - az * by, gy = az * bx - ax * bz, gz = ax * by - ay * bx;
+    const float g2 = gx * gx + gy * gy + gz * gz;
+    if (!(g2 > 0.0f && g2 < inf)) return e;
+    bool ok = true;
+    const uint32_t hx = cull_float_to_half_trunc((pA[0] + pB[0] + pC[0]) * (1.0f / 3.0f), ok);
+    const uint32_t hy = cull_float_to_half_trunc((pA[1] + pB[1] + pC[1]) * (1.0f / 3.0f), ok);
+    const uint32_t hz = cull_float_to_half_trunc((pA[2] + pB[2] + pC[2]) * (1.0f / 3.0f), ok);
+    if (!ok) return e;
+    const float cx = cull_half_to_float(hx), cy = cull_half_to_float(hy), cz = cull_half_to_float(hz);
+    float r2 = 0.0f;
+    const float* v[3] = { pA, pB, pC };
+    for (int k = 0; k < 3; ++k) {
+        const float dx = v[k][0] - cx, dy = v[k][1] - cy, dz = v[k][2] - cz;
+        const float d2 = dx * dx + dy * dy + dz * dz;
+        if (!(d2 <= r2)) r2 = d2;
+    }
+    const uint32_t hr = cull_float_to_half_up(__builtin_sqrtf(r2) * 1.00001f);
+    if (hr >= kCullHalfInf) return e;
+    e.cxy = hx | (hy << 16);
+    e.czr = hz | (hr << 16);
+    if (!flat) return e;
+    const float wx = m[0] * nA[0] + m[1] * nA[1] + m[2] * nA[2];
+    const float wy = m[3] * nA[0] + m[4] * nA[1] + m[5] * nA[2];
+    const float wz = m[6] * nA[0] + m[7] * nA[1] + m[8] * nA[2];
+    const float len = __builtin_sqrtf(wx * wx + wy * wy + wz * wz);
+    float mag = 0.0f;
+    for (int k = 0; k < 9; ++k) mag += cull_abs(m[k] * nA[k % 3]);
+    if (!(len > 0.0f && len < inf && mag <= 64.0f * len)) return e;
+    const float ux = wx / len, uy = wy / len, uz = wz / len;
+    const uint32_t q = cull_oct_encode(ux, uy, uz);
+    float nx, ny, nz;
+    cull_oct_decode(q, nx, ny, nz);
+    const float nl = __builtin_sqrtf(nx * nx + ny * ny + nz * nz);
+    const float ex = nx / nl - ux, ey = ny / nl - uy, ez = nz / nl - uz;
+    if (!(ex * ex + ey * ey + ez * ez <= (0.5f * kCullNormalTol) * (0.5f * kCullNormalTol))) return e;
+    float hLo = inf;
+    for (int k = 0; k < 3; ++k) {
+        const float h = nx * v[k][0] + ny * v[k][1] + nz * v[k][2];
+        if (!(h >= hLo)) hLo = h;
+    }
+    if (!(hLo > -inf && hLo < inf)) return e;
+    e.octN = q;
+    e.hLo = hLo;
+    return e;
+}
+
+GFX_CULL_HD bool cull_proves_zero(const EmitterCull& e, float px, float py, float pz, float nx, float ny, float nz, float vz) {
+    const float cx = cull_half_to_float(e.cxy & 0xFFFFu), cy = cull_half_to_float(e.cxy >> 16);
+    const float cz = cull_half_to_float(e.czr & 0xFFFFu), r = cull_half_to_float(e.czr >> 16);
+    const float dx = cx - px, dy = cy - py, dz = cz - pz;
+    const float S = ((cull_abs(dx) + cull_abs(dy)) + cull_abs(dz)) + ((cull_abs(px) + cull_abs(py)) + cull_abs(pz)) + r;
+    const float margin = kCullMargin * S + kCullMargin;
+    float Nx, Ny, Nz;
+    cull_oct_decode(e.octN, Nx, Ny, Nz);
+    const bool plane = Nx * px + Ny * py + Nz * pz <= e.hLo - margin;
+    const float h = nx * dx + ny * dy + nz * dz;
+    const bool horizon = vz > 0.0f ? h + r < -margin : vz < 0.0f ? r - h < -margin : false;
+    return S < 3.0e38f && (plane || horizon);
+}
+
+}
diff --git a/gfxexp_amd/csrc/gm_math.hip.h b/gfxexp_amd/csrc/gm_math.hip.h
--- a/gfxexp_amd/csrc/gm_math.hip.h
+++ b/gfxexp_amd/csrc/gm_math.hip.h
@@ -13,11 +13,15 @@
 #define GFX_CYC_BEGIN unsigned long long cyc__[8] = { 0, 0, 0, 0, 0, 0, 0, 0 }; unsigned long long cycT__ = __builtin_amdgcn_s_memtime(); int cycK__ = 7;
 #define GFX_CYC(k) do { const unsigned long long t__ = __builtin_amdgcn_s_memtime(); cyc__[cycK__] += t__ - cycT__; cycT__ = t__; cycK__ = (k); } while (0)
 #define GFX_CYC_END do { GFX_CYC(7); if ((threadIdx.x & 63) == 0) for (int k__ = 0; k__ < 8; ++k__) atomicAdd(&g_laneProfile[32 + k__], cyc__[k__]); } while (0)
+#define GFX_CYC_PARAMS , unsigned long long (&cyc__)[8], unsigned long long& cycT__, int& cycK__
+#define GFX_CYC_ARGS , cyc__, cycT__, cycK__
 #else
 #define GFX_PROF(k) do { } while (0)
 #define GFX_CYC_BEGIN
 #define GFX_CYC(k) do { } while (0)
 #define GFX_CYC_END do { } while (0)
+#define GFX_CYC_PARAMS
+#define GFX_CYC_ARGS
 #endif
 
 constexpr float kPi = 3.14159265358979323846f;
diff --git a/gfxexp_amd/csrc/internal.h b/gfxexp_amd/csrc/internal.h
--- a/gfxexp_amd/csrc/internal.h
+++ b/gfxexp_amd/csrc/internal.h
@@ -82,6 +82,7 @@
     int traceBatch = 64;
     int temporalHints = 1;
     int candidateSplit = 0;
+    int candidatePrefilter = 1;
     int blockOrder = 1;
     int fusePasses = 0;
     int nrcStagedInfer = 0;
@@ -105,7 +106,7 @@
     std::vector<std::vector<uint32_t>> groups;
     std::vector<HostInstance> insts;
     bool sceneDirty = true;
-    DevBuf dMaterials, dGeomInsts, dInsts, dVertices, dTriangles, dSlotPool, dFlatGeoms, dLightW, dLightP, dLightCDF, dLightRefs, dEmitterRecs, dEmitterRecExtras, dLightNormalMatrices, dInstMatrixIndex, dTextures, dTexelPool, dSrgbLut, dEmitterTexRefs;
+    DevBuf dMaterials, dGeomInsts, dInsts, dVertices, dTriangles, dSlotPool, dFlatGeoms, dLightW, dLightP, dLightCDF, dLightRefs, dEmitterRecs, dEmitterRecExtras, dEmitterCull, dLightNormalMatrices, dInstMatrixIndex, dTextures, dTexelPool, dSrgbLut, dEmitterTexRefs;
     bool anyEmittanceTexture = false;
     std::vector<LightGeomRef> hLightRefs;
     uint32_t numEmitterRecs = 0;
diff --git a/gfxexp_amd/csrc/lights.hip b/gfxexp_amd/csrc/lights.hip
--- a/gfxexp_amd/csrc/lights.hip
+++ b/gfxexp_amd/csrc/lights.hip
@@ -72,13 +72,17 @@
 
 __global__ void k_emitter_records(DevScene sc, uint32_t numInsts, LightGeomRef* __restrict__ refs, EmitterRec* __restrict__ recs,
                                   EmitterRecExtra* __restrict__ extras, const uint32_t* __restrict__ instMatrixIndex,
-                                  EmitterTexRef* __restrict__ texRefs ) {
+                                  EmitterTexRef* __restrict__ texRefs ,
+                                  EmitterCull* __restrict__ cull) {
     const uint32_t ii = blockIdx.x;
     if (ii >= numInsts) return;
     const DevInstance* inst = sc.insts + ii;
     if (inst->distOffset == 0xFFFFFFFFu) return;
     const uint32_t matrixBits = (instMatrixIndex[ii] & kEmitterMatrixMask) << kEmitterMatrixShift;
     const m34 xfm = load_m34(inst->transform);
+    float normalMatrix[9];
+    for (int r = 0; r < 3; ++r)
+        for (int c = 0; c < 3; ++c) normalMatrix[3 * r + c] = sc.lightNormalMatrices[16u * (instMatrixIndex[ii] & kEmitterMatrixMask) + 4u * r + c];
     for (uint32_t k = 0; k < inst->numGeomInsts; ++k) {
         const DevGeomInst g = sc.geomInsts[sc.geomInstSlotPool[inst->slotsOffset + k]];
         LightGeomRef* ref = refs + inst->distOffset + k;
@@ -115,6 +119,9 @@
             float4* dstX = reinterpret_cast<float4*>(extras + recBase + t);
             const float4* srcX = reinterpret_cast<const float4*>(&x);
             dstX[0] = srcX[0]; dstX[1] = srcX[1];
+            const bool finiteEmittance = is_finite(e.x) && is_finite(e.y) && is_finite(e.z);
+            const EmitterCull ce = cull_build(normalMatrix, r.nA, !smooth, r.pA, r.pB, r.pC, finiteEmittance);
+            *reinterpret_cast<uint4*>(cull + recBase + t) = make_uint4(ce.octN, f2bits(ce.hLo), ce.cxy, ce.czr);
             if (texRefs) {
                 EmitterTexRef tr;
                 tr.uvA[0] = vA.u; tr.uvA[1] = vA.v; tr.uvB[0] = vB.u; tr.uvB[1] = vB.v; tr.uvC[0] = vC.u; tr.uvC[1] = vC.v;
@@ -320,7 +327,7 @@
     if (ni)
         hipLaunchKernelGGL(k_emitter_records, dim3(ni), dim3(64), 0, stream, ctx.devScene(), ni,
                            ctx.dLightRefs.as<LightGeomRef>(), ctx.dEmitterRecs.as<EmitterRec>(), ctx.dEmitterRecExtras.as<EmitterRecExtra>(), ctx.dInstMatrixIndex.as<uint32_t>(),
-                               ctx.anyEmittanceTexture ? ctx.dEmitterTexRefs.as<EmitterTexRef>() : nullptr);
+                               ctx.anyEmittanceTexture ? ctx.dEmitterTexRefs.as<EmitterTexRef>() : nullptr, ctx.dEmitterCull.as<EmitterCull>());
     GFX_HIP(hipGetLastError());
     GFX_HIP(hipMemcpyAsync(ctx.hGeomInsts.data(), ctx.dGeomInsts.p, sizeof(DevGeomInst) * ng, hipMemcpyDeviceToHost, stream));
     GFX_HIP(hipMemcpyAsync(ctx.hInsts.data(), ctx.dInsts.p, sizeof(DevInstance) * ni, hipMemcpyDeviceToHost, stream));
@@ -337,7 +344,7 @@
         if (numInsts)
             hipLaunchKernelGGL(k_emitter_records, dim3(numInsts), dim3(64), 0, stream, ctx.devScene(), numInsts,
                                ctx.dLightRefs.as<LightGeomRef>(), ctx.dEmitterRecs.as<EmitterRec>(), ctx.dEmitterRecExtras.as<EmitterRecExtra>(), ctx.dInstMatrixIndex.as<uint32_t>(),
-                               ctx.anyEmittanceTexture ? ctx.dEmitterTexRefs.as<EmitterTexRef>() : nullptr);
+                               ctx.anyEmittanceTexture ? ctx.dEmitterTexRefs.as<EmitterTexRef>() : nullptr, ctx.dEmitterCull.as<EmitterCull>());
         GFX_HIP(hipGetLastError());
         ctx.emitterRecsDirty = false;
     }
diff --git a/gfxexp_amd/csrc/restir.hip b/gfxexp_amd/csrc/restir.hip
--- a/gfxexp_amd/csrc/restir.hip
+++ b/gfxexp_amd/csrc/restir.hip
@@ -180,10 +180,94 @@
     sub = launchThread & (SPLIT - 1);
     return pixel_of_block_thread(g, (launchThread / SPLIT) / kBlock, (launchThread / SPLIT) % kBlock);
 }
+struct CandidateJumps { LcgJump j[33]; };
+constexpr CandidateJumps make_candidate_jumps() {
+    CandidateJumps t = {};
+    for (uint32_t k = 0; k <= 32u; ++k) t.j[k] = lcg_jump(4u * k);
+    return t;
+}
+__constant__ const CandidateJumps kCandidateJumps = make_candidate_jumps();
+
+GFX_DEV void candidate_light_type(const RestirArgs& a, bool envEnabled, uint32_t numCandidates, uint32_t i, float& ul, float& probCurType, bool& sampleEnv) {
+    probCurType = 1.0f; sampleEnv = false;
+    if (envEnabled) {
+        if (*a.scene.lightInstIntegral > 0.0f) {
+            const float prob = fmin2(fmax2(0.25f * numCandidates - i, 0.0f), 1.0f);
+            if (prob == 1.0f) { probCurType = 0.25f; sampleEnv = true; }
+            else if (prob == 0.0f) probCurType = 1.0f - 0.25f;
+            else if (ul < prob) { probCurType = 0.25f; ul = ul / prob; sampleEnv = true; }
+            else { probCurType = 1.0f - 0.25f; ul = (ul - prob) / (1 - prob); }
+        }
+        else sampleEnv = true;
+    }
+}
+
+template <bool EMITTER_TEX>
+GFX_DEV void candidate_eval(const RestirArgs& a, uint4* waveBuf, int lane, const EnvMap& env, bool envEnabled, const ShadingPoint& sp,
+                            bool active, uint32_t numCandidates, uint32_t i, Pcg32& rng, LightSample& ls, float& target, float& weight GFX_CYC_PARAMS) {
+    GFX_PROF(0);
+    GFX_CYC(0);
+    float probCurType = 1.0f, u0 = 0.0f, u1 = 0.0f;
+    bool sampleEnv = false;
+    LightPick pk; pk.rec = 0; pk.instSlot = 0; pk.density = 0.0f; pk.partialProb = 0.0f; pk.ok = false; pk.table = true;
+    if (active) {
+        float ul = rng.uniform();
+        candidate_light_type(a, envEnabled, numCandidates, i, ul, probCurType, sampleEnv);
+        u0 = rng.uniform();
+        u1 = rng.uniform();
+        if (!sampleEnv) pk = light_select(a.scene, ul);
+    }
+    GFX_CYC(1);
+    const bool fetch = active && !sampleEnv && pk.ok;
+    uint4 q0 = make_uint4(0u, 0u, 0u, 0u), q1 = q0, q2 = q0, q3 = q0;
+    m33 normalMatrix;
+    normalMatrix.r0 = normalMatrix.r1 = normalMatrix.r2 = f3(0.0f);
+    if (__ballot(fetch) != 0ull) {
+        coop_fetch64_issue(fetch ? pk.rec : kCoopNone, reinterpret_cast<const char*>(a.scene.emitterRecs), waveBuf, lane);
+        coop_fetch64_wait();
+        if (fetch) coop_fetch64_read(waveBuf, lane, q0, q1, q2, q3);
+        if (fetch) normalMatrix = load_m33_rows(a.scene.lightNormalMatrices + 16u * emitter_matrix_index(q3.w));
+    }
+    GFX_CYC(2);
+    if (active) {
+        ls.emittance = f3(0.0f); ls.position = f3(0.0f); ls.normal = f3(0.0f); ls.atInfinity = 0;
+        float pd = 0.0f;
+        PendingEmittance pending; pending.tex = 0u; pending.rec = 0u; pending.bcA = pending.bcB = pending.bcC = 0.0f;
+        if (sampleEnv) sample_env_light(env, a.f.envLightRotation, a.f.envLightPowerCoeff, u0, u1, ls, pd);
+        else if (pk.ok) {
+            GFX_PROF(1);
+            light_from_record<EMITTER_TEX, false>(a.scene, pk, as_float4(q0), as_float4(q1), as_float4(q2), as_float4(q3), normalMatrix, u0, u1, ls, pd,
+                                                  f3(0.0f), EMITTER_TEX ? &pending : nullptr);
+        }
+        GFX_CYC(3);
+        const f3 cont = EMITTER_TEX ? direct_lighting_pending(a.scene, sp.pos, sp.vOutLocal, sp.frame, sp.bsdf, ls, pending)
+                                    : direct_lighting(sp.pos, sp.vOutLocal, sp.frame, sp.bsdf, ls);
+        GFX_CYC(4);
+        pd *= probCurType;
+        target = target_weight(cont);
+        weight = target / pd;
+    }
+}
+
+GFX_DEV bool candidate_live(const RestirArgs& a, bool envEnabled, const ShadingPoint& sp, uint32_t numCandidates, uint32_t i, float ul) {
+    float probCurType;
+    bool sampleEnv;
+    candidate_light_type(a, envEnabled, numCandidates, i, ul, probCurType, sampleEnv);
+    if (sampleEnv) return true;
+    const LightPick pk = light_select(a.scene, ul);
+    if (!pk.table || !pk.ok) return true;
+    const float pd = pk.density * probCurType;
+    if (!(pd != 0.0f && is_finite(pd))) return true;
+    const uint4 w = *reinterpret_cast<const uint4*>(a.scene.emitterCull + pk.rec);
+    EmitterCull e; e.octN = w.x; e.hLo = bits2f(w.y); e.cxy = w.z; e.czr = w.w;
+    return !cull_proves_zero(e, sp.pos.x, sp.pos.y, sp.pos.z, sp.frame.n.x, sp.frame.n.y, sp.frame.n.z, sp.vOutLocal.z);
+}
+
 struct CandidateRay { bool writer, want; f3 org, dir; float tmax; };
-template <bool EMITTER_TEX, int SPLIT>
+template <bool EMITTER_TEX, int SPLIT, bool PREFILTER = false>
 GFX_DEV CandidateRay initial_candidates(const RestirArgs& a, uint4* waveBuf, int lane, const PixelId& px, uint32_t sub) {
     static_assert(SPLIT == 1 || SPLIT == 2 || SPLIT == 4, "a pixel's lanes are an aligned pair or quad");
+    static_assert(!PREFILTER || SPLIT == 1, "the lanes of a split pixel add their weights in lockstep");
     const size_t numPixels = static_cast<size_t>(a.s.imageSizeX) * a.s.imageSizeY;
     const size_t p = px.p;
     const uint32_t bufIdx = a.f.bufferIndex;
@@ -214,62 +298,47 @@
     int lastAccepted = -1;
     const uint32_t numCandidates = 1u << a.f.log2NumCandidateSamples;
     GFX_CYC_BEGIN
+    if (PREFILTER) {
+        for (uint32_t base = 0; base < numCandidates; base += 32u) {
+            const uint32_t chunk = numCandidates - base < 32u ? numCandidates - base : 32u;
+            const uint64_t start = rng.state;
+            uint32_t live = 0u;
+            GFX_CYC(6);
+            if (surface) {
+                Pcg32 walk; walk.state = start;
+                for (uint32_t k = 0; k < chunk; ++k) {
+                    const float ul = walk.uniform();
+                    constexpr LcgJump rest = lcg_jump(3);
+                    walk.state = walk.state * rest.mul + rest.add;
+                    if (candidate_live(a, envEnabled, sp, numCandidates, base + k, ul)) { GFX_PROF(6); live |= 1u << k; }
+                }
+            }
+            while (__ballot(live != 0u) != 0ull) {
+                const bool active = live != 0u;
+                const uint32_t k = active ? static_cast<uint32_t>(__builtin_ctz(live)) : 0u;
+                live &= live - 1u;
+                const LcgJump jump = kCandidateJumps.j[k];
+                Pcg32 at; at.state = start * jump.mul + jump.add;
+                LightSample ls;
+                float target = 0.0f, weight = 0.0f;
+                candidate_eval<EMITTER_TEX>(a, waveBuf, lane, env, envEnabled, sp, active, numCandidates, base + k, at, ls, target, weight GFX_CYC_ARGS);
+                if (active && reservoir.update(ls, weight, at.uniform())) { GFX_PROF(5); selectedTarget = target; }
+            }
+            const LcgJump past = kCandidateJumps.j[chunk];
+            rng.state = start * past.mul + past.add;
+        }
+        reservoir.streamLength = numCandidates;
+    }
+    else
     for (uint32_t i = sub; i < numCandidates; i += SPLIT) {
-        GFX_PROF(0);
-        GFX_CYC(0);
-        float probCurType = 1.0f, u0 = 0.0f, u1 = 0.0f;
-        bool sampleEnv = false;
-        LightPick pk; pk.rec = 0; pk.instSlot = 0; pk.density = 0.0f; pk.partialProb = 0.0f; pk.ok = false; pk.table = true;
+        if (surface && SPLIT > 1 && i >= SPLIT) {
+            constexpr LcgJump skip = lcg_jump(4 * (SPLIT - 1));
+            rng.state = rng.state * skip.mul + skip.add;
+        }
+        LightSample ls;
+        float target = 0.0f, weight = 0.0f;
+        candidate_eval<EMITTER_TEX>(a, waveBuf, lane, env, envEnabled, sp, surface, numCandidates, i, rng, ls, target, weight GFX_CYC_ARGS);
         if (surface) {
-            if (SPLIT > 1 && i >= SPLIT) {
-                constexpr LcgJump skip = lcg_jump(4 * (SPLIT - 1));
-                rng.state = rng.state * skip.mul + skip.add;
-            }
-            float ul = rng.uniform();
-            if (envEnabled) {
-                if (*a.scene.lightInstIntegral > 0.0f) {
-                    const float prob = fmin2(fmax2(0.25f * numCandidates - i, 0.0f), 1.0f);
-                    if (prob == 1.0f) { probCurType = 0.25f; sampleEnv = true; }
-                    else if (prob == 0.0f) probCurType = 1.0f - 0.25f;
-                    else if (ul < prob) { probCurType = 0.25f; ul = ul / prob; sampleEnv = true; }
-                    else { probCurType = 1.0f - 0.25f; ul = (ul - prob) / (1 - prob); }
-                }
-                else sampleEnv = true;
-            }
-            u0 = rng.uniform();
-            u1 = rng.uniform();
-            if (!sampleEnv) pk = light_select(a.scene, ul);
-        }
-        GFX_CYC(1);
-        const bool fetch = surface && !sampleEnv && pk.ok;
-        uint4 q0 = make_uint4(0u, 0u, 0u, 0u), q1 = q0, q2 = q0, q3 = q0;
-        m33 normalMatrix;
-        normalMatrix.r0 = normalMatrix.r1 = normalMatrix.r2 = f3(0.0f);
-        if (__ballot(fetch) != 0ull) {
-            coop_fetch64_issue(fetch ? pk.rec : kCoopNone, reinterpret_cast<const char*>(a.scene.emitterRecs), waveBuf, lane);
-            coop_fetch64_wait();
-            if (fetch) coop_fetch64_read(waveBuf, lane, q0, q1, q2, q3);
-            if (fetch) normalMatrix = load_m33_rows(a.scene.lightNormalMatrices + 16u * emitter_matrix_index(q3.w));
-        }
-        GFX_CYC(2);
-        if (surface) {
-            LightSample ls;
-            ls.emittance = f3(0.0f); ls.position = f3(0.0f); ls.normal = f3(0.0f); ls.atInfinity = 0;
-            float pd = 0.0f;
-            PendingEmittance pending; pending.tex = 0u; pending.rec = 0u; pending.bcA = pending.bcB = pending.bcC = 0.0f;
-            if (sampleEnv) sample_env_light(env, a.f.envLightRotation, a.f.envLightPowerCoeff, u0, u1, ls, pd);
-            else if (pk.ok) {
-                GFX_PROF(1);
-                light_from_record<EMITTER_TEX, false>(a.scene, pk, as_float4(q0), as_float4(q1), as_float4(q2), as_float4(q3), normalMatrix, u0, u1, ls, pd,
-                                                      f3(0.0f), EMITTER_TEX ? &pending : nullptr);
-            }
-            GFX_CYC(3);
-            const f3 cont = EMITTER_TEX ? direct_lighting_pending(a.scene, sp.pos, sp.vOutLocal, sp.frame, sp.bsdf, ls, pending)
-                                        : direct_lighting(sp.pos, sp.vOutLocal, sp.frame, sp.bsdf, ls);
-            GFX_CYC(4);
-            pd *= probCurType;
-            const float target = target_weight(cont);
-            const float weight = target / pd;
             if (SPLIT == 1) {
                 if (reservoir.update(ls, weight, rng.uniform())) { GFX_PROF(5); selectedTarget = target; }
             }
@@ -315,7 +384,7 @@
     r.writer = writer; r.want = wantRay; r.org = rayO; r.dir = rayD; r.tmax = rayTmax;
     return r;
 }
-template <bool EMITTER_TEX, int SPLIT>
+template <bool EMITTER_TEX, int SPLIT, bool PREFILTER>
 __global__ __launch_bounds__(kBlock) __attribute__((amdgpu_waves_per_eu(GFX_INIT_WAVES, GFX_INIT_WAVES))) void k_initial_candidates(RestirArgs a, uint32_t* __restrict__ blockCost) {
     __shared__ __attribute__((aligned(16))) uint4 fetchBuf[(kBlock / 64) * 256];
     const int lane = threadIdx.x & 63;
@@ -324,7 +393,7 @@
     const unsigned long long t0 = blockCost ? __builtin_amdgcn_s_memtime() : 0ull;
     uint32_t sub;
     const PixelId px = pixel_of_split_thread<SPLIT>(a.px, sub, block);
-    const CandidateRay r = initial_candidates<EMITTER_TEX, SPLIT>(a, waveBuf, lane, px, sub);
+    const CandidateRay r = initial_candidates<EMITTER_TEX, SPLIT, PREFILTER>(a, waveBuf, lane, px, sub);
     if (r.writer) {
         const uint32_t slot = emit_ray_at_slot(px, r.want, r.org, r.dir, 0.0f, r.tmax, a);
         if (px.valid) a.pixelRaySlot[px.p] = slot;
@@ -1078,9 +1147,12 @@
                 block_order_end(0, grid, cost);
                 break;
             }
+            const bool prefilter = ctx.tune.candidatePrefilter != 0;
             void (*kernel)(RestirArgs, uint32_t*) = a.scene.emitterTexRefs
-                ? (split == 4 ? k_initial_candidates<true, 4> : split == 2 ? k_initial_candidates<true, 2> : k_initial_candidates<true, 1>)
-                : (split == 4 ? k_initial_candidates<false, 4> : split == 2 ? k_initial_candidates<false, 2> : k_initial_candidates<false, 1>);
+                ? (split == 4 ? k_initial_candidates<true, 4, false> : split == 2 ? k_initial_candidates<true, 2, false>
+                   : prefilter ? k_initial_candidates<true, 1, true> : k_initial_candidates<true, 1, false>)
+                : (split == 4 ? k_initial_candidates<false, 4, false> : split == 2 ? k_initial_candidates<false, 2, false>
+                   : prefilter ? k_initial_candidates<false, 1, true> : k_initial_candidates<false, 1, false>);
             const uint32_t* order = nullptr;
             uint32_t* cost = nullptr;
             block_order_begin(3, grid, split, order, cost);
diff --git a/gfxexp_amd/csrc/scene.cpp b/gfxexp_amd/csrc/scene.cpp
--- a/gfxexp_amd/csrc/scene.cpp
+++ b/gfxexp_amd/csrc/scene.cpp
@@ -10,7 +10,7 @@
 
 Context::~Context() {
     for (Accel* a : accels) { if (a) { a->nodes.release(); a->links.release(); a->triIds.release(); a->rootBoxes.release(); delete a; } }
-    DevBuf* all[] = { &dMaterials, &dGeomInsts, &dInsts, &dVertices, &dTriangles, &dSlotPool, &dFlatGeoms, &dSubset[0], &dSubset[1], &dLightW, &dLightP, &dLightCDF, &dLightRefs, &dEmitterRecs, &dEmitterRecExtras, &dLightNormalMatrices, &dInstMatrixIndex, &dTextures, &dTexelPool, &dSrgbLut, &dEmitterTexRefs,
+    DevBuf* all[] = { &dMaterials, &dGeomInsts, &dInsts, &dVertices, &dTriangles, &dSlotPool, &dFlatGeoms, &dSubset[0], &dSubset[1], &dLightW, &dLightP, &dLightCDF, &dLightRefs, &dEmitterRecs, &dEmitterRecExtras, &dEmitterCull, &dLightNormalMatrices, &dInstMatrixIndex, &dTextures, &dTexelPool, &dSrgbLut, &dEmitterTexRefs,
                       &rayOrg, &rayDir, &rayOut, &rayHits, &spill, &gbRayOrg, &gbRayDir, &gbRayHits, &gbSpill, &gbCounters, &auxSpill, &auxCounters, &blockOrders[0].cost, &blockOrders[0].order, &blockOrders[1].cost, &blockOrders[1].order, &blockOrders[2].cost, &blockOrders[2].order, &blockOrders[3].cost, &blockOrders[3].order, &blockOrders[4].cost, &blockOrders[4].order, &pixelRaySlot, &shadeScratch, &spatialScratch, &smallCounters,
                       &bTris, &bBoxes, &bKeys, &bKeysAlt, &bVals, &bValsAlt, &bSortTemp, &bNodesLR, &bParents, &bFlags,
                       &bNodeBoxes, &bRanges, &bQueueA, &bQueueB, &bCounters, &dTraceCounters, &dLightInstIntegral, &dLightInstGuide, &dSpans, &dSpanGuide, &dSpanHeader, &dSpanInstBegin,
@@ -41,6 +41,7 @@
     s.lightGeomRefs = dLightRefs.as<LightGeomRef>();
     s.emitterRecs = dEmitterRecs.as<EmitterRec>();
     s.emitterRecExtras = dEmitterRecExtras.as<EmitterRecExtra>();
+    s.emitterCull = dEmitterCull.as<EmitterCull>();
     s.lightNormalMatrices = dLightNormalMatrices.as<float>();
     s.numLightMatrices = numLightMatrices;
     s.lightInstIntegral = dLightInstIntegral.as<float>();
@@ -321,6 +322,7 @@
     upload(ctx.dLightRefs, ctx.hLightRefs, stream);
     ctx.dEmitterRecs.reserve(std::max<size_t>(sizeof(EmitterRec) * ctx.numEmitterRecs, 16));
     ctx.dEmitterRecExtras.reserve(std::max<size_t>(sizeof(EmitterRecExtra) * ctx.numEmitterRecs, 16));
+    ctx.dEmitterCull.reserve(std::max<size_t>(sizeof(EmitterCull) * ctx.numEmitterRecs, 16));
     light_matrices_upload(ctx, stream);
     ctx.dEmitterTexRefs.reserve(std::max<size_t>(ctx.anyEmittanceTexture ? sizeof(EmitterTexRef) * ctx.numEmitterRecs : 0, 16));
     ctx.dLightW.reserve(std::max<size_t>(sizeof(float) * lightPool, 16));
```

New measurement: 753.8 Mpaths/s (median of 6 runs). +6.2%, better.
